# OpenVVC/OpenVVC

Measured on AMD Instinct MI355X. Metric: decoded frames/sec, full rcn back-end decode step (H2D of the recorded picture + MC incl. BDOF/DMVR/affine-PROF/GPM/CIIP + LMCS + inverse transform + ordered intra pass + deblocking + SAO + ALF/CC-ALF + D2H of refined MVs + wait + per-picture digest + publication to the device DPB), 4K 10-bit RA rec, higher is better.
Workload: dtype u16 samples / int16 coefficients / int32 accumulate

## Files before the change

### include/ovvc_hip.h

```cpp
#ifndef OVVC_HIP_H
#define OVVC_HIP_H

#include <stddef.h>
#include <stdint.h>

#ifdef __cplusplus
extern "C" {
#endif

#define OVHIP_ABI_VERSION 9

#define OVHIP_OK        0
#define OVHIP_ENODEV   (-1)
#define OVHIP_ENOMEM   (-2)
#define OVHIP_EINVAL   (-3)
#define OVHIP_ELAUNCH  (-4)
#define OVHIP_EUNSUP   (-5)
#define OVHIP_EREF     (-6)

enum { OVHIP_DST_VII = 0, OVHIP_DCT_VIII = 1, OVHIP_DCT_II = 2 };

typedef struct ovhip_pic {
    uint16_t *y, *cb, *cr;
    int32_t   w, h;
// ... 693 lines not shown
int  ovhip_dpb_create_ex(ovhip_dpb **out, int n_devices, const ovhip_dpb_ops *ops);
void ovhip_dpb_destroy(ovhip_dpb *d);
int  ovhip_dpb_n_devices(const ovhip_dpb *d);
int  ovhip_dpb_device(const ovhip_dpb *d, int dev);
int  ovhip_dpb_begin(ovhip_dpb *d, const void *key, int dev, int32_t w, int32_t h, ovhip_pic *pic);
int  ovhip_dpb_want(ovhip_dpb *d, const void *key, int dev);
int  ovhip_dpb_begin_tag(ovhip_dpb *d, const void *key, uint64_t tag, int dev, int32_t w, int32_t h, ovhip_pic *pic);
int  ovhip_dpb_want_tag(ovhip_dpb *d, const void *key, uint64_t tag, int dev);
int  ovhip_dpb_acquire_tag(ovhip_dpb *d, const void *key, uint64_t tag, int dev, ovhip_pic *pic, void **event);
int  ovhip_dpb_publish(ovhip_dpb *d, const void *key, int status);
void ovhip_dpb_set_unknown_key_timeout(ovhip_dpb *d, int ms);
int  ovhip_dpb_acquire(ovhip_dpb *d, const void *key, int dev, ovhip_pic *pic, void **event);
int  ovhip_dpb_poll_tag(ovhip_dpb *d, const void *key, uint64_t tag);
int  ovhip_dpb_post_rows(ovhip_dpb *d, const void *key, int32_t rows, void *event, const volatile uint32_t *abort_word);
int  ovhip_dpb_rows_tag(ovhip_dpb *d, const void *key, uint64_t tag, int dev, int32_t need_rows, int block, int pin, ovhip_pic *pic, void **event);
int  ovhip_dpb_wait_copy(ovhip_dpb *d, int dev, void *event);
int  ovhip_dpb_unpin(ovhip_dpb *d, const void *key);
int  ovhip_dpb_release(ovhip_dpb *d, const void *key);
int  ovhip_dpb_lookup(ovhip_dpb *d, const void *key, int *home_dev, ovhip_pic *pic);
void ovhip_dpb_shutdown(ovhip_dpb *d);
int  ovhip_dpb_get_stats(ovhip_dpb *d, ovhip_dpb_stats *out);

typedef struct ovhip_frame ovhip_frame;

enum { OVHIP_OUT_NONE = 0,
       OVHIP_OUT_DIGEST = 1,
       OVHIP_OUT_PLANES = 2,
       OVHIP_OUT_PACKED = 3 };
typedef struct ovhip_frame_output {
    int32_t  mode;
    ovhip_window window;
    uint16_t *y, *cb, *cr; int32_t stride_y, stride_c;
    void    *packed;
    uint8_t  digest[16];
} ovhip_frame_output;

enum { OVHIP_FE_BEGIN = 1, OVHIP_FE_REF, OVHIP_FE_DMVR_ROWS, OVHIP_FE_DMVR_BEGIN, OVHIP_FE_DMVR_COLLECT, OVHIP_FE_SUBMIT, OVHIP_FE_FAIL,
       OVHIP_FE_BAND  };
typedef struct ovhip_frame_event {
    uint32_t op; int32_t frame;
    uint64_t key, tag;
    int64_t  a, b, result;
} ovhip_frame_event;
void ovhip_frame_set_trace(void (*sink)(void *user, const ovhip_frame_event *ev), void *user);

int  ovhip_frame_create(ovhip_dpb *dpb, int dev, int32_t w, int32_t h, ovhip_frame **out);
void ovhip_frame_destroy(ovhip_frame *f);
ovhip_ctx      *ovhip_frame_ctx(ovhip_frame *f);
ovhip_job      *ovhip_frame_job(ovhip_frame *f);
ovhip_recorder *ovhip_frame_recorder(ovhip_frame *f);
int  ovhip_frame_begin(ovhip_frame *f, const void *key);
int  ovhip_frame_ref(ovhip_frame *f, const void *ref_key);
int  ovhip_frame_begin_tag(ovhip_frame *f, const void *key, uint64_t tag);
int  ovhip_frame_ref_tag(ovhip_frame *f, const void *ref_key, uint64_t tag);
int  ovhip_frame_ref_at(ovhip_frame *f, int slot, const void *ref_key);
int64_t ovhip_frame_dmvr_rows(ovhip_frame *f);
int  ovhip_frame_refs_ready(ovhip_frame *f);
int64_t ovhip_frame_dmvr_rows_begin(ovhip_frame *f, int32_t log2_ctu_s);
int64_t ovhip_frame_dmvr_rows_begin_upto(ovhip_frame *f, int32_t log2_ctu_s, size_t upto_units);
int64_t ovhip_frame_dmvr_rows_collect(ovhip_frame *f);
int  ovhip_frame_submit(ovhip_frame *f, ovhip_job *job, const ovhip_pic *intra, const ovhip_job_params *params, ovhip_frame_output *out);
int  ovhip_frame_set_band_mode(ovhip_frame *f, int on);
int  ovhip_frame_band(ovhip_frame *f, const ovhip_job_params *params, int32_t row_end, int32_t last, ovhip_frame_output *out);
int  ovhip_frame_band_upto(ovhip_frame *f, const ovhip_job_params *params, int32_t row_end, const ovhip_band_counts *upto, int32_t block);
int  ovhip_frame_band_stats(const ovhip_frame *f, int32_t *n_bands, int32_t *n_deferred);
int  ovhip_frame_set_output_scale(ovhip_frame *f, int32_t out_w, int32_t out_h, const ovhip_scale_info *info);
int  ovhip_frame_fail(ovhip_frame *f, int status);
const char *ovhip_frame_last_error(const ovhip_frame *f);

typedef struct ovhip_calllog ovhip_calllog;
ovhip_calllog *ovhip_calllog_create(void);
void   ovhip_calllog_destroy(ovhip_calllog *log);
void   ovhip_calllog_reset(ovhip_calllog *log);
const void *ovhip_calllog_data(const ovhip_calllog *log, size_t *bytes);
void   ovhip_rec_set_calllog(ovhip_recorder *rec, ovhip_calllog *log);
int64_t ovhip_calllog_replay(const void *data, size_t bytes, ovhip_recorder *rec);

#define OVHIP_STREAM_MAX_REFS 8
typedef struct ovhip_stream_content {
    const void *calllog; size_t calllog_bytes;
    ovhip_job_params params;
    uint32_t n_ref_slots;
} ovhip_stream_content;

typedef struct ovhip_stream_pic {
    uint32_t content;
    uint32_t job;
    int32_t  poc;
    uint16_t device;
    uint16_t n_refs;
    uint32_t refs[OVHIP_STREAM_MAX_REFS];
    int32_t  owner;
    uint32_t send_mask;
} ovhip_stream_pic;

typedef struct ovhip_stream_xfer {
    void *user;
    int (*send)(void *user, uint32_t idx, const ovhip_pic *pic, int dst_rank);
    int (*recv)(void *user, uint32_t idx, const ovhip_pic *pic, int src_rank);
} ovhip_stream_xfer;

typedef struct ovhip_rccl ovhip_rccl;
int  ovhip_rccl_unique_id(uint8_t out[128]);
int  ovhip_rccl_create(ovhip_rccl **out, const uint8_t unique_id[128], int rank, int world, int hip_device);
void ovhip_rccl_destroy(ovhip_rccl *r);
const ovhip_stream_xfer *ovhip_rccl_xfer(ovhip_rccl *r);
const char *ovhip_rccl_last_error(const ovhip_rccl *r);
int  ovhip_rccl_stats(const ovhip_rccl *r, uint64_t out[4]);
int  ovhip_rccl_self_exchange(ovhip_rccl *r, const ovhip_pic *src, const ovhip_pic *dst);

enum { OVHIP_STREAM_RECORD = 1,
       OVHIP_STREAM_DIGESTS = 2,
       OVHIP_STREAM_RESIDENT = 4,
       OVHIP_STREAM_KEEP = 8,
       OVHIP_STREAM_HOLD_ALL = 32,
       OVHIP_STREAM_FILE_MD5 = 16 };

typedef struct ovhip_stream_cfg {
    int32_t w, h;
    uint32_t flags;
    int32_t threads_per_device;
    int32_t output;
    ovhip_window window;
    uint32_t extra_stages;
    int32_t rank;
    const ovhip_stream_xfer *xfer;
    int32_t intra_lookahead;
    int32_t ahead_own_queue;
} ovhip_stream_cfg;

typedef struct ovhip_stream_result {
    double   seconds;
    uint64_t n_decoded, n_second_passes, n_received, n_sent;
    uint64_t out_frames, out_bytes;
    uint8_t  out_md5[16];
    double   record_seconds;
    double   host_seconds[5];
    int32_t  status;
    char     error[192];
    double  *trace;
} ovhip_stream_result;

typedef struct ovhip_stream ovhip_stream;
int  ovhip_stream_create(ovhip_stream **out, ovhip_dpb *dpb, const ovhip_stream_cfg *cfg, const ovhip_stream_content *contents,
                         uint32_t n_contents, ovhip_job *const *jobs, uint32_t n_jobs);
void ovhip_stream_destroy(ovhip_stream *s);
int  ovhip_stream_run(ovhip_stream *s, const ovhip_stream_pic *pics, uint32_t n_total, uint32_t first, uint32_t n, uint32_t flags,
                      uint8_t *digests, ovhip_stream_result *res);
ovhip_frame *ovhip_stream_frame(ovhip_stream *s, int dev, int thread);
int  ovhip_stream_queue_info(const ovhip_stream *s, int *moved, int *sharing);
int  ovhip_stream_set_output_scale(ovhip_stream *s, int32_t out_w, int32_t out_h, const ovhip_scale_info *info);
const void *ovhip_stream_key(const ovhip_stream *s, uint32_t idx);
int  ovhip_job_test_abort_next_flow(ovhip_job *job);

#ifdef __cplusplus
}
#endif
#endif
```

### openvvc_amd/capi.py

```python
from __future__ import annotations

import ctypes as C
import os
from pathlib import Path

import numpy as np

_PKG = Path(__file__).resolve().parent
LIB_PATH = _PKG / os.environ.get("OVVC_HIP_LIB_NAME", "libovvc_hip.so")

OVHIP_ABI_VERSION = 9
OVHIP_OK, OVHIP_ENODEV, OVHIP_ENOMEM, OVHIP_EINVAL, OVHIP_ELAUNCH, OVHIP_EUNSUP, OVHIP_EREF = 0, -1, -2, -3, -4, -5, -6
DST_VII, DCT_VIII, DCT_II = 0, 1, 2
TB_TR, TB_DC, TB_TS, TB_TS_RAW = 0, 1, 2, 3
TB_FLAG_RASTER = 0x80
RES_ADD, RES_SUB, RES_ADD_HALF, RES_SUB_HALF, RES_SCALE = 0, 1, 2, 3, 4
MC_HPEL_FILT, MC_FILT_4x4, MC_NO_LUMA, MC_NO_CHROMA, MC_LMCS, MC_BDOF, MC_DMVR = 1, 2, 4, 8, 16, 32, 64
PU_BDOF, PU_DMVR, PU_GPM = 1, 2, 4
MC_GPM = 128


class Pic(C.Structure):
    _fields_ = [("y", C.c_void_p), ("cb", C.c_void_p), ("cr", C.c_void_p),
                ("w", C.c_int32), ("h", C.c_int32), ("stride_y", C.c_int32), ("stride_c", C.c_int32)]
# ... 380 lines not shown
    global _lib
    if _lib is not None and path is None:
        return _lib
    p = Path(path) if path else LIB_PATH
    if not p.exists():
        raise RuntimeError(f"{p} not built: run `python -c 'import __graft_entry__ as g; g.build()'` "
                           "(the HIP engine has no CPU fallback)")
    try:
        import torch
    except Exception:
        pass
    lib = C.CDLL(str(p))
    vp, u32, i32 = C.c_void_p, C.c_uint32, C.c_int32
    P = C.POINTER
    sigs = {
        "ovhip_abi_version": (C.c_int, []),
        "ovhip_rec_create": (vp, [i32, i32]),
        "ovhip_rec_destroy": (None, [vp]),
        "ovhip_rec_reset": (None, [vp]),
        "ovhip_rec_tu": (C.c_int, [vp, P(TuState), P(TuDesc)]),
        "ovhip_rec_pu": (C.c_int, [vp, P(PuDesc)]),
        "ovhip_rec_set_ref_scale": (C.c_int, [vp, i32, P(RefScale)]),
        "ovhip_rec_refusal": (C.c_char_p, [vp]),
        "ovhip_rec_rpr_units": (vp, [vp, P(C.c_size_t)]),
        "ovhip_mc_rpr_launch": (C.c_int, [vp, P(Pic), P(Pic), u32, vp, u32, vp, P(Pic)]),
        "ovhip_rec_set_rpr_tools": (C.c_int, [vp, u32]),
        "ovhip_rec_aff_rpr_units": (vp, [vp, P(C.c_size_t)]),
        "ovhip_mca_rpr_launch": (C.c_int, [vp, P(Pic), P(Pic), u32, vp, u32, vp, vp]),
        "ovhip_rec_dbf_ctu": (C.c_int, [vp, vp]),
        "ovhip_rec_dbf_row": (C.c_int, [vp, vp, C.c_size_t]),
        "ovhip_rec_dbf_mv_prepass_view": (C.c_int, [vp, vp, vp, vp]),
        "ovhip_rec_cu_inter": (C.c_int, [vp, vp, vp]),
        "ovhip_rec_dbf_planes": (C.c_int, [vp, P(DbfPlanes)]),
        "ovhip_dbf_launch": (C.c_int, [vp, P(Pic), P(DbfPlanes)]),
        "ovhip_sao_launch": (C.c_int, [vp, P(Pic), P(Pic), vp, i32]),
        "ovhip_alf_launch": (C.c_int, [vp, P(Pic), P(Pic), P(AlfPic)]),
        "ovhip_rec_tb_cmds": (vp, [vp, P(C.c_size_t)]),
        "ovhip_rec_coefs": (vp, [vp, P(C.c_size_t)]),
        "ovhip_rec_mc_units": (vp, [vp, P(C.c_size_t)]),
        "ovhip_rec_mcx_units": (vp, [vp, P(C.c_size_t)]),
        "ovhip_rec_affine_cu": (C.c_int, [vp, P(AffineDesc)]),
        "ovhip_rec_transform_tree": (C.c_int, [vp, P(TuState), P(TtDesc)]),
        "ovhip_rec_lmcs_region": (C.c_int, [vp, C.c_int32, C.c_int32, u32, u32]),
        "ovhip_dbf_compact": (C.c_int64, [P(DbfPlanes), C.c_int, vp, C.c_size_t]),
        "ovhip_rec_dbf_mv_prepass": (C.c_int, [vp, P(DbfMvCtx)]),
        "ovhip_dbf_launch_edges": (C.c_int, [vp, P(Pic), vp, u32, vp, u32, C.c_int32, C.c_int32]),
        "ovhip_rec_ciip": (C.c_int, [vp, C.c_int32, C.c_int32, C.c_int32, C.c_int32, C.c_int32, C.c_int32]),
        "ovhip_rec_ciip_units": (vp, [vp, P(C.c_size_t)]),
        "ovhip_ciip_launch": (C.c_int, [vp, P(Pic), P(Pic), vp, u32]),
        "ovhip_rec_lmcs_regions": (vp, [vp, P(C.c_size_t)]),
        "ovhip_rec_tb_cmds_split": (vp, [vp, C.c_size_t * 4, P(C.c_size_t)]),
        "ovhip_itx_launch_classes": (C.c_int, [vp, P(Pic), vp, u32, u32, vp, vp]),
        "ovhip_itx_launch_chroma_lmcs": (C.c_int, [vp, P(Pic), vp, u32, u32, vp, vp, vp]),
        "ovhip_lmcs_build": (C.c_int, [P(LmcsData), P(LmcsLuts)]),
        "ovhip_lmcs_scale_launch": (C.c_int, [vp, P(Pic), vp, u32, P(LmcsLuts), vp]),
        "ovhip_lmcs_inverse_launch": (C.c_int, [vp, P(Pic), vp]),
        "ovhip_rec_aff_units": (vp, [vp, P(C.c_size_t)]),
        "ovhip_rec_aff_side": (vp, [vp, P(C.c_size_t)]),
        "ovhip_ctx_create": (C.c_int, [P(vp), C.c_int, vp]),
        "ovhip_ctx_destroy": (None, [vp]),
        "ovhip_ctx_sync": (C.c_int, [vp]),
        "ovhip_ctx_shares_queue": (C.c_int, [vp, vp]),
        "ovhip_ctx_new_stream": (C.c_int, [vp]),
        "ovhip_ctx_fork": (C.c_int, [vp, C.c_int]),
        "ovhip_ctx_join": (C.c_int, [vp]),
        "ovhip_last_error": (C.c_char_p, [vp]),
        "ovhip_ctx_stream": (vp, [vp]),
        "ovhip_malloc": (C.c_int, [vp, C.c_size_t, P(vp)]),
        "ovhip_free": (C.c_int, [vp, vp]),
        "ovhip_h2d": (C.c_int, [vp, vp, vp, C.c_size_t]),
        "ovhip_d2h": (C.c_int, [vp, vp, vp, C.c_size_t]),
        "ovhip_pic_alloc": (C.c_int, [vp, i32, i32, P(Pic)]),
        "ovhip_pic_free": (C.c_int, [vp, P(Pic)]),
        "ovhip_pic_upload": (C.c_int, [vp, P(Pic), vp, vp, vp, i32, i32]),
        "ovhip_pic_download": (C.c_int, [vp, P(Pic), vp, vp, vp, i32, i32]),
        "ovhip_itx_launch": (C.c_int, [vp, P(Pic), vp, u32, vp, vp]),
        "ovhip_mc_launch": (C.c_int, [vp, P(Pic), P(Pic), u32, vp, u32, vp, P(Pic)]),
        "ovhip_ciip_weight": (C.c_int, [C.c_int32, C.c_int32]),
        "ovhip_mcx_launch": (C.c_int, [vp, P(Pic), P(Pic), u32, vp, u32, vp, vp]),
        "ovhip_mca_launch": (C.c_int, [vp, P(Pic), P(Pic), u32, vp, u32, vp, vp]),
        "ovhip_mcxa_launch": (C.c_int, [vp, P(Pic), P(Pic), u32, vp, u32, vp, vp, u32, vp, vp]),
        "ovhip_rec_create_ex": (vp, [i32, i32, vp]),
        "ovhip_rec_set_dense_dbf_planes": (None, [vp, C.c_int]),
        "ovhip_rec_dbf_edges": (vp, [vp, C.c_int, P(C.c_size_t), P(DbfOffsets)]),
        "ovhip_dbf_launch_edges_ex": (C.c_int, [vp, P(Pic), vp, u32, vp, u32, P(DbfOffsets)]),
        "ovhip_dmvr_search_launch": (C.c_int, [vp, P(Pic), P(Pic), u32, vp, u32, vp]),
        "ovhip_rec_append_raw": (C.c_int, [vp, C.c_int, vp, C.c_size_t]),
        "ovhip_itx_launch_classes_res": (C.c_int, [vp, P(Pic), P(Pic), vp, u32, u32, vp, vp]),
        "ovhip_intra_level_launch": (C.c_int, [vp, P(Pic), P(Pic), vp, u32, vp, vp, vp, i32, u32]),
        "ovhip_intra_level_geom": (u32, [vp, C.c_size_t]),
        "ovhip_intra_sync_words": (C.c_size_t, [i32, i32, i32]),
        "ovhip_intra_flow_words": (C.c_size_t, [i32, i32]),
        "ovhip_intra_flow_items": (C.c_size_t, [vp, C.c_size_t, vp, C.c_size_t]),
        "ovhip_intra_flow_launch": (C.c_int, [vp, P(Pic), P(Pic), vp, u32, vp, u32, vp, vp, vp, i32, vp, u32, vp, i32, i32]),
        "ovhip_intra_ctu_launch": (C.c_int, [vp, P(Pic), P(Pic), vp, vp, u32, vp, vp, vp, i32, vp, u32, vp]),
        "ovhip_rec_itask_levels": (u32, [vp]),
        "ovhip_rec_isp_cu": (C.c_int, [vp, vp, vp]),
        "ovhip_isp_geometry": (None, [i32, i32, i32, P(i32), P(i32), P(i32), P(i32)]),
        "ovhip_job_bind": (C.c_int, [vp, vp]),
        "ovhip_rec_set_ctu_size": (C.c_int, [vp, i32]),
        "ovhip_rec_itasks_by_ctu": (vp, [vp, i32, P(C.c_size_t), P(vp), P(C.c_size_t)]),
        "ovhip_rec_tu_intra": (C.c_int, [vp, P(TuState), P(TuDesc), P(ITask), P(ITask)]),
        "ovhip_rec_itasks": (vp, [vp, P(C.c_size_t)]),
        "ovhip_rec_itasks_sorted": (vp, [vp, P(C.c_size_t), P(P(C.c_uint32)), P(C.c_uint32)]),
        "ovhip_rec_set_dbf_offsets": (C.c_int, [vp, P(DbfOffsets), C.c_int]),
        "ovhip_job_create": (C.c_int, [vp, i32, i32, P(vp)]),
        "ovhip_job_destroy": (None, [vp]),
        "ovhip_job_recorder": (vp, [vp]),
        "ovhip_job_begin": (C.c_int, [vp]),
        "ovhip_job_flush": (C.c_int, [vp, P(Pic), P(Pic), u32, P(Pic), P(JobParams)]),
        "ovhip_frame_band": (C.c_int, [vp, P(JobParams), i32, i32, P(FrameOutput)]),
        "ovhip_frame_set_band_mode": (C.c_int, [vp, C.c_int]),
        "ovhip_frame_band_upto": (C.c_int, [vp, P(JobParams), i32, P(BandCounts), i32]),
        "ovhip_frame_dmvr_rows_begin_upto": (C.c_int64, [vp, i32, C.c_size_t]),
        "ovhip_job_dmvr_rows_begin_upto": (C.c_int64, [vp, P(Pic), u32, i32, C.c_size_t]),
        "ovhip_frame_band_stats": (C.c_int, [vp, P(i32), P(i32)]),
        "ovhip_dpb_post_rows": (C.c_int, [vp, vp, i32, vp, vp]),
        "ovhip_dpb_rows_tag": (C.c_int, [vp, vp, C.c_uint64, C.c_int, i32, C.c_int, C.c_int, P(Pic), P(vp)]),
        "ovhip_job_band": (C.c_int, [vp, P(Pic), P(Pic), u32, P(JobParams), P(BandCounts), i32, i32]),
        "ovhip_job_band_active": (C.c_int, [vp]),
        "ovhip_job_band_busy": (C.c_int, [vp]),
        "ovhip_job_band_progress": (C.c_int, [vp, P(i32), P(vp), P(vp)]),
        "ovhip_rec_counts": (None, [vp, P(BandCounts)]),
        "ovhip_sao_launch_rows": (C.c_int, [vp, P(Pic), P(Pic), vp, i32, i32, i32]),
        "ovhip_alf_launch_rows": (C.c_int, [vp, P(Pic), P(Pic), P(AlfPic), i32, i32]),
        "ovhip_job_wait": (C.c_int, [vp]),
        "ovhip_job_refined_mvs": (vp, [vp, P(C.c_size_t)]),
        "ovhip_job_dmvr_rows": (C.c_int64, [vp, P(Pic), u32]),
        "ovhip_job_dmvr_rows_begin": (C.c_int64, [vp, P(Pic), u32, i32]),
        "ovhip_job_dmvr_rows_collect": (C.c_int64, [vp]),
        "ovhip_job_last_stats": (C.c_int, [vp, P(JobStats)]),
        "ovhip_job_time_stage": (C.c_int, [vp, C.c_int]),
        "ovhip_job_stage_time": (C.c_int, [vp, P(C.c_double), P(C.c_uint64)]),
        "ovhip_lmcs_scale_prepare_launch": (C.c_int, [vp, P(Pic), vp, u32, vp, vp, vp, u32, vp, u32]),
        "ovhip_lmcs_inverse_untag_launch": (C.c_int, [vp, P(Pic), vp, vp, u32]),
        "ovhip_intra_flow_untag_launch": (C.c_int, [vp, P(Pic), vp, u32, i32]),
        "ovhip_tmvp_cells_launch": (C.c_int, [vp, vp, u32, vp, i32, i32, vp]),
        "ovhip_job_tmvp_cells": (vp, [vp, P(C.c_size_t)]),
        "ovhip_output_bytes": (C.c_size_t, [i32, i32, P(Window)]),
        "ovhip_output_rows": (C.c_size_t, [i32, i32, P(Window)]),
        "ovhip_output_pack_launch": (C.c_int, [vp, P(Pic), P(Window), vp]),
        "ovhip_output_row_md5_launch": (C.c_int, [vp, P(Pic), P(Window), vp]),
        "ovhip_output_bands": (C.c_size_t, [i32, i32, P(Window)]),
        "ovhip_output_tree_md5_launch": (C.c_int, [vp, P(Pic), P(Window), vp]),
        "ovhip_pic_output": (C.c_int, [vp, P(Pic), P(Window), vp]),
        "ovhip_pic_digest": (C.c_int, [vp, P(Pic), P(Window), vp]),
        "ovhip_md5_init": (None, [P(Md5State)]),
        "ovhip_md5_update": (None, [P(Md5State), vp, C.c_size_t]),
        "ovhip_md5_final": (None, [P(Md5State), vp]),
        "ovhip_d2d": (C.c_int, [vp, vp, vp, C.c_size_t]),
        "ovhip_host_alloc": (vp, [C.c_size_t]),
        "ovhip_host_free": (None, [vp]),
        "ovhip_job_test_abort_next_flow": (C.c_int, [vp]),
        "ovhip_dpb_create": (C.c_int, [P(vp), P(C.c_int), C.c_int]),
        "ovhip_dpb_create_ex": (C.c_int, [P(vp), C.c_int, P(DpbOps)]),
        "ovhip_dpb_destroy": (None, [vp]),
        "ovhip_dpb_n_devices": (C.c_int, [vp]),
        "ovhip_dpb_device": (C.c_int, [vp, C.c_int]),
        "ovhip_dpb_begin": (C.c_int, [vp, vp, C.c_int, i32, i32, P(Pic)]),
        "ovhip_dpb_want": (C.c_int, [vp, vp, C.c_int]),
        "ovhip_dpb_begin_tag": (C.c_int, [vp, vp, C.c_uint64, C.c_int, i32, i32, P(Pic)]),
        "ovhip_dpb_want_tag": (C.c_int, [vp, vp, C.c_uint64, C.c_int]),
        "ovhip_dpb_acquire_tag": (C.c_int, [vp, vp, C.c_uint64, C.c_int, P(Pic), P(vp)]),
        "ovhip_dpb_publish": (C.c_int, [vp, vp, C.c_int]),
        "ovhip_dpb_acquire": (C.c_int, [vp, vp, C.c_int, P(Pic), P(vp)]),
        "ovhip_dpb_wait_copy": (C.c_int, [vp, C.c_int, vp]),
        "ovhip_dpb_poll_tag": (C.c_int, [vp, vp, C.c_uint64]),
        "ovhip_frame_refs_ready": (C.c_int, [vp]),
        "ovhip_dpb_set_unknown_key_timeout": (None, [vp, C.c_int]),
        "ovhip_dpb_unpin": (C.c_int, [vp, vp]),
        "ovhip_dpb_release": (C.c_int, [vp, vp]),
        "ovhip_dpb_lookup": (C.c_int, [vp, vp, P(C.c_int), P(Pic)]),
        "ovhip_dpb_shutdown": (None, [vp]),
        "ovhip_dpb_get_stats": (C.c_int, [vp, P(DpbStats)]),
        "ovhip_frame_create": (C.c_int, [vp, C.c_int, i32, i32, P(vp)]),
        "ovhip_frame_destroy": (None, [vp]),
        "ovhip_frame_ctx": (vp, [vp]),
        "ovhip_frame_job": (vp, [vp]),
        "ovhip_frame_recorder": (vp, [vp]),
        "ovhip_frame_begin": (C.c_int, [vp, vp]),
        "ovhip_frame_ref": (C.c_int, [vp, vp]),
        "ovhip_frame_set_trace": (None, [vp, vp]),
        "ovhip_rccl_unique_id": (C.c_int, [vp]),
        "ovhip_rccl_create": (C.c_int, [P(vp), vp, C.c_int, C.c_int, C.c_int]),
        "ovhip_rccl_destroy": (None, [vp]),
        "ovhip_rccl_xfer": (vp, [vp]),
        "ovhip_rccl_last_error": (C.c_char_p, [vp]),
        "ovhip_rccl_stats": (C.c_int, [vp, P(C.c_uint64)]),
        "ovhip_rccl_self_exchange": (C.c_int, [vp, P(Pic), P(Pic)]),
        "ovhip_frame_begin_tag": (C.c_int, [vp, vp, C.c_uint64]),
        "ovhip_frame_ref_tag": (C.c_int, [vp, vp, C.c_uint64]),
        "ovhip_frame_ref_at": (C.c_int, [vp, C.c_int, vp]),
        "ovhip_frame_dmvr_rows": (C.c_int64, [vp]),
        "ovhip_frame_dmvr_rows_begin": (C.c_int64, [vp, i32]),
        "ovhip_frame_dmvr_rows_collect": (C.c_int64, [vp]),
        "ovhip_frame_submit": (C.c_int, [vp, vp, P(Pic), P(JobParams), P(FrameOutput)]),
        "ovhip_frame_fail": (C.c_int, [vp, C.c_int]),
        "ovhip_frame_last_error": (C.c_char_p, [vp]),
        "ovhip_calllog_create": (vp, []),
        "ovhip_calllog_destroy": (None, [vp]),
        "ovhip_calllog_reset": (None, [vp]),
        "ovhip_calllog_data": (vp, [vp, P(C.c_size_t)]),
        "ovhip_rec_set_calllog": (None, [vp, vp]),
        "ovhip_calllog_replay": (C.c_int64, [vp, C.c_size_t, vp]),
        "ovhip_stream_create": (C.c_int, [P(vp), vp, P(StreamCfg), P(StreamContent), u32, P(vp), u32]),
        "ovhip_stream_destroy": (None, [vp]),
        "ovhip_stream_run": (C.c_int, [vp, P(StreamPic), u32, u32, u32, u32, vp, P(StreamResult)]),
        "ovhip_stream_frame": (vp, [vp, C.c_int, C.c_int]),
        "ovhip_stream_queue_info": (C.c_int, [vp, P(C.c_int), P(C.c_int)]),
        "ovhip_stream_key": (vp, [vp, u32]),
        "ovhip_output_scale_check": (C.c_int, [i32, i32, P(ScaleInfo), i32, i32, P(i32 * 4)]),
        "ovhip_output_scale_launch": (C.c_int, [vp, P(Pic), P(ScaleInfo), P(Pic)]),
        "ovhip_pic_output_scaled": (C.c_int, [vp, P(Pic), P(ScaleInfo), i32, i32, P(Window), vp]),
        "ovhip_pic_digest_scaled": (C.c_int, [vp, P(Pic), P(ScaleInfo), i32, i32, P(Window), vp]),
        "ovhip_ctx_scratch_bytes": (C.c_size_t, [vp]),
        "ovhip_frame_set_output_scale": (C.c_int, [vp, i32, i32, P(ScaleInfo)]),
        "ovhip_stream_set_output_scale": (C.c_int, [vp, i32, i32, P(ScaleInfo)]),
    }
    ab_build = "OVVC_HIP_LIB_NAME" in os.environ
    for name, (res, args) in sigs.items():
        if ab_build and not hasattr(lib, name):
            continue
        fn = getattr(lib, name)
        fn.restype, fn.argtypes = res, args
    if lib.ovhip_abi_version() != OVHIP_ABI_VERSION and not ab_build:
        raise RuntimeError("libovvc_hip.so ABI version mismatch")
    if path is None:
        _lib = lib
    return lib


EXPORTED_SYMBOLS = [
    "ovhip_abi_version", "ovhip_rec_create", "ovhip_rec_destroy", "ovhip_rec_reset", "ovhip_rec_tu",
    "ovhip_rec_pu", "ovhip_rec_cu_inter", "ovhip_rec_dbf_row", "ovhip_rec_dbf_mv_prepass_view", "ovhip_rec_dbf_ctu", "ovhip_rec_dbf_planes", "ovhip_dbf_launch", "ovhip_sao_launch", "ovhip_alf_launch", "ovhip_rec_tb_cmds", "ovhip_rec_coefs", "ovhip_rec_mc_units", "ovhip_rec_mcx_units", "ovhip_mcx_launch", "ovhip_rec_affine_cu", "ovhip_rec_transform_tree", "ovhip_rec_lmcs_region", "ovhip_dbf_compact", "ovhip_rec_dbf_mv_prepass", "ovhip_dbf_launch_edges", "ovhip_rec_ciip", "ovhip_ciip_weight", "ovhip_rec_ciip_units", "ovhip_ciip_launch", "ovhip_rec_lmcs_regions", "ovhip_rec_tb_cmds_split", "ovhip_itx_launch_classes", "ovhip_itx_launch_chroma_lmcs", "ovhip_lmcs_build", "ovhip_lmcs_scale_launch", "ovhip_lmcs_inverse_launch", "ovhip_rec_aff_units", "ovhip_rec_aff_side", "ovhip_mca_launch", "ovhip_mcxa_launch", "ovhip_ctx_create",
    "ovhip_ctx_destroy", "ovhip_ctx_sync", "ovhip_ctx_shares_queue", "ovhip_ctx_new_stream", "ovhip_ctx_fork", "ovhip_ctx_join", "ovhip_last_error", "ovhip_ctx_stream", "ovhip_malloc",
    "ovhip_free", "ovhip_h2d", "ovhip_d2h", "ovhip_pic_alloc", "ovhip_pic_free", "ovhip_pic_upload",
    "ovhip_pic_download", "ovhip_itx_launch", "ovhip_mc_launch",
    "ovhip_rec_set_ref_scale", "ovhip_rec_refusal", "ovhip_rec_rpr_units", "ovhip_mc_rpr_launch",
    "ovhip_rec_set_rpr_tools", "ovhip_rec_aff_rpr_units", "ovhip_mca_rpr_launch",
    "ovhip_rec_create_ex", "ovhip_rec_set_dense_dbf_planes", "ovhip_rec_dbf_edges", "ovhip_dbf_launch_edges_ex",
    "ovhip_dmvr_search_launch", "ovhip_rec_append_raw", "ovhip_rec_set_dbf_offsets", "ovhip_rec_tu_intra", "ovhip_rec_itasks", "ovhip_rec_itasks_sorted", "ovhip_itx_launch_classes_res", "ovhip_intra_level_launch", "ovhip_intra_level_geom", "ovhip_intra_sync_words", "ovhip_intra_ctu_launch", "ovhip_intra_flow_words", "ovhip_intra_flow_items", "ovhip_intra_flow_launch",
    "ovhip_rec_itask_levels", "ovhip_rec_isp_cu", "ovhip_isp_geometry", "ovhip_rec_itasks_by_ctu", "ovhip_rec_set_ctu_size", "ovhip_job_bind", "ovhip_job_create", "ovhip_job_destroy", "ovhip_job_recorder", "ovhip_job_begin",
    "ovhip_frame_band", "ovhip_frame_band_upto", "ovhip_frame_dmvr_rows_begin_upto", "ovhip_job_dmvr_rows_begin_upto", "ovhip_frame_set_band_mode", "ovhip_frame_band_stats", "ovhip_dpb_post_rows", "ovhip_dpb_rows_tag",
    "ovhip_job_band", "ovhip_job_band_active", "ovhip_job_band_busy", "ovhip_job_band_reserve", "ovhip_job_reserve_for_picture", "ovhip_rec_reserve_for_picture", "ovhip_job_band_progress", "ovhip_rec_counts", "ovhip_sao_launch_rows", "ovhip_alf_launch_rows",
    "ovhip_job_flush", "ovhip_job_wait", "ovhip_job_refined_mvs", "ovhip_job_dmvr_rows", "ovhip_job_dmvr_rows_begin", "ovhip_job_dmvr_rows_collect", "ovhip_job_last_stats", "ovhip_job_time_stage", "ovhip_job_stage_time",
    "ovhip_output_bytes", "ovhip_output_rows", "ovhip_output_pack_launch", "ovhip_output_row_md5_launch", "ovhip_output_bands", "ovhip_output_tree_md5_launch", "ovhip_pic_output", "ovhip_pic_digest",
    "ovhip_md5_init", "ovhip_md5_update", "ovhip_md5_final", "ovhip_tmvp_cells_launch", "ovhip_job_tmvp_cells", "ovhip_intra_flow_untag_launch", "ovhip_lmcs_inverse_untag_launch", "ovhip_lmcs_scale_prepare_launch",
    "ovhip_host_alloc", "ovhip_host_free", "ovhip_d2d", "ovhip_job_test_abort_next_flow",
    "ovhip_dpb_create", "ovhip_dpb_create_ex", "ovhip_dpb_destroy", "ovhip_dpb_n_devices", "ovhip_dpb_device", "ovhip_dpb_begin", "ovhip_dpb_want",
    "ovhip_dpb_publish", "ovhip_dpb_acquire", "ovhip_dpb_wait_copy", "ovhip_dpb_poll_tag", "ovhip_frame_refs_ready", "ovhip_dpb_set_unknown_key_timeout", "ovhip_dpb_unpin", "ovhip_dpb_release", "ovhip_dpb_lookup", "ovhip_dpb_shutdown",
    "ovhip_dpb_get_stats", "ovhip_dpb_begin_tag", "ovhip_dpb_want_tag", "ovhip_dpb_acquire_tag", "ovhip_frame_begin_tag", "ovhip_frame_ref_tag", "ovhip_frame_set_trace",
    "ovhip_rccl_unique_id", "ovhip_rccl_create", "ovhip_rccl_destroy", "ovhip_rccl_xfer", "ovhip_rccl_last_error", "ovhip_rccl_stats", "ovhip_rccl_self_exchange",
    "ovhip_frame_create", "ovhip_frame_destroy", "ovhip_frame_ctx", "ovhip_frame_job", "ovhip_frame_recorder", "ovhip_frame_begin", "ovhip_frame_ref",
    "ovhip_frame_ref_at", "ovhip_frame_dmvr_rows", "ovhip_frame_dmvr_rows_begin", "ovhip_frame_dmvr_rows_collect", "ovhip_frame_submit", "ovhip_frame_fail", "ovhip_frame_last_error",
    "ovhip_calllog_create", "ovhip_calllog_destroy", "ovhip_calllog_reset", "ovhip_calllog_data", "ovhip_rec_set_calllog", "ovhip_calllog_replay",
    "ovhip_stream_create", "ovhip_stream_destroy", "ovhip_stream_run", "ovhip_stream_frame", "ovhip_stream_key", "ovhip_stream_queue_info",
    "ovhip_output_scale_check", "ovhip_output_scale_launch", "ovhip_pic_output_scaled", "ovhip_pic_digest_scaled",
    "ovhip_frame_set_output_scale", "ovhip_stream_set_output_scale", "ovhip_ctx_scratch_bytes",
]


def rpr_units(lib, rec) -> list:
    n = C.c_size_t(0)
    ptr = lib.ovhip_rec_rpr_units(rec, C.byref(n))
    if not ptr or not n.value:
        return []
    raw = C.string_at(ptr, n.value * C.sizeof(RprUnit))
    return [RprUnit.from_buffer_copy(raw, i * C.sizeof(RprUnit)) for i in range(n.value)]


def aff_rpr_units(lib, rec) -> list:
    n = C.c_size_t(0)
    ptr = lib.ovhip_rec_aff_rpr_units(rec, C.byref(n))
    if not ptr or not n.value:
        return []
    raw = C.string_at(ptr, n.value * C.sizeof(AffRprUnit))
    return [AffRprUnit.from_buffer_copy(raw, i * C.sizeof(AffRprUnit)) for i in range(n.value)]


def set_ref_scale(lib, rec, slot: int, scale_hor: int | None = None, scale_ver: int | None = None, ref_w: int = 0, ref_h: int = 0,
                  col_hor: int = 0, col_ver: int = 0) -> int:
    if scale_hor is None:
        return lib.ovhip_rec_set_ref_scale(rec, slot, None)
    sc = RefScale(scale_hor, scale_ver if scale_ver is not None else scale_hor, ref_w, ref_h, col_hor, col_ver)
    return lib.ovhip_rec_set_ref_scale(rec, slot, C.byref(sc))


class Recorder:

    def __init__(self, pic_w: int, pic_h: int):
        self.lib = load()
        self.h = self.lib.ovhip_rec_create(pic_w, pic_h)
        if not self.h:
            raise MemoryError("ovhip_rec_create")
        self._keep = []

    def close(self):
        if self.h:
            self.lib.ovhip_rec_destroy(self.h)
            self.h = None

    def __del__(self):
        try:
            self.close()
        except Exception:
            pass

    def reset(self):
        self.lib.ovhip_rec_reset(self.h)

    def start_calllog(self):
        self._log = self.lib.ovhip_calllog_create()
        self.lib.ovhip_rec_set_calllog(self.h, self._log)

    def take_calllog(self) -> np.ndarray:
        n = C.c_size_t()
        p = self.lib.ovhip_calllog_data(self._log, C.byref(n))
        if not p and n.value:
            raise MemoryError("call log")
        out = np.frombuffer((C.c_char * n.value).from_address(p), dtype=np.uint8).copy() if n.value else np.zeros(0, np.uint8)
        self.lib.ovhip_rec_set_calllog(self.h, None)
        self.lib.ovhip_calllog_destroy(self._log)
        self._log = None
        return out

    def replay(self, log: np.ndarray) -> int:
        n = self.lib.ovhip_calllog_replay(log.ctypes.data, log.nbytes, self.h)
        if n < 0:
            raise ValueError(f"ovhip_calllog_replay -> {n}")
        return int(n)

    def tu(self, st: TuState, d: TuDesc) -> int:
        r = self.lib.ovhip_rec_tu(self.h, C.byref(st), C.byref(d))
        if r < 0:
            raise ValueError(f"ovhip_rec_tu -> {r}")
        return r

    def tu_intra(self, st: TuState, d: TuDesc, task_l: "ITask | None", task_c: "ITask | None") -> int:
        r = self.lib.ovhip_rec_tu_intra(self.h, C.byref(st), C.byref(d), C.byref(task_l) if task_l is not None else None,
                                        C.byref(task_c) if task_c is not None else None)
        if r < 0:
            raise ValueError(f"ovhip_rec_tu_intra -> {r}")
        return r

    def itasks(self) -> np.ndarray:
        return self._arr(self.lib.ovhip_rec_itasks, ITASK_DTYPE)

    def itasks_sorted(self):
        n, nl, ls = C.c_size_t(), C.c_uint32(), C.POINTER(C.c_uint32)()
        p = self.lib.ovhip_rec_itasks_sorted(self.h, C.byref(n), C.byref(ls), C.byref(nl))
        if not n.value:
            return np.zeros(0, ITASK_DTYPE), np.zeros(1, np.uint32)
        t = np.frombuffer((C.c_char * (n.value * 32)).from_address(p), dtype=ITASK_DTYPE).copy()
        return t, np.array([ls[i] for i in range(nl.value + 1)], np.uint32)

    def itasks_by_ctu(self, log2_ctu: int = 7):
        n, nc, cp = C.c_size_t(), C.c_size_t(), C.c_void_p()
        p = self.lib.ovhip_rec_itasks_by_ctu(self.h, log2_ctu, C.byref(n), C.byref(cp), C.byref(nc))
        if not n.value:
            return np.zeros(0, ITASK_DTYPE), np.zeros(0, ICTU_DTYPE)
        t = np.frombuffer((C.c_char * (n.value * 32)).from_address(p), dtype=ITASK_DTYPE).copy()
        c = np.frombuffer((C.c_char * (nc.value * 16)).from_address(cp.value), dtype=ICTU_DTYPE).copy()
        return t, c

    def transform_tree(self, st: "TuState", d: TtDesc, infos: bytes, res_cb: np.ndarray, res_cr: np.ndarray, res_y: np.ndarray) -> int:
        ib = (C.c_char * len(infos)).from_buffer_copy(infos)
        keep = [np.ascontiguousarray(a, dtype=np.int16) for a in (res_cb, res_cr, res_y)]
        d.tu_info = C.addressof(ib)
        for k in range(3):
            d.residual[k] = keep[k].ctypes.data
        r = self.lib.ovhip_rec_transform_tree(self.h, C.byref(st), C.byref(d))
        d.tu_info = None
        if r < 0:
            raise ValueError(f"ovhip_rec_transform_tree -> {r}")
        return r

    def isp_cu(self, st: TuState, d: IspDesc) -> int:
        r = self.lib.ovhip_rec_isp_cu(self.h, C.byref(st), C.byref(d))
        if r < 0:
            raise ValueError(f"ovhip_rec_isp_cu -> {r}")
        return r

    def isp_geometry(self, log2_w: int, log2_h: int, vertical: int):
        a, b, c, d = C.c_int32(), C.c_int32(), C.c_int32(), C.c_int32()
        self.lib.ovhip_isp_geometry(log2_w, log2_h, vertical, C.byref(a), C.byref(b), C.byref(c), C.byref(d))
        return a.value, b.value, c.value, d.value

    def pu(self, d: PuDesc) -> int:
        r = self.lib.ovhip_rec_pu(self.h, C.byref(d))
        if r < 0:
            raise ValueError(f"ovhip_rec_pu -> {r}")
        return r

    def affine_cu(self, d: AffineDesc, mv0: np.ndarray, mv1: np.ndarray) -> int:
        mv0 = np.ascontiguousarray(mv0, dtype=np.int32)
        mv1 = np.ascontiguousarray(mv1, dtype=np.int32)
        d.mv0, d.mv1 = mv0.ctypes.data, mv1.ctypes.data
        r = self.lib.ovhip_rec_affine_cu(self.h, C.byref(d))
        d.mv0 = d.mv1 = None
        if r < 0:
            raise ValueError(f"ovhip_rec_affine_cu -> {r}")
# ... 99 lines not shown
```

### openvvc_amd/csrc/kernels_dbf.hip

```cpp
#include "ovvc_common.hip.h"
#define OVT_ATTR __device__
#include "vvc_dbf_tables.h"

#ifndef OV_WPE_DBF
#define OV_WPE_DBF 0
#endif
#if OV_WPE_DBF > 0
#define OV_OCC_DBF __attribute__((amdgpu_waves_per_eu(OV_WPE_DBF)))
#else
#define OV_OCC_DBF
#endif

namespace {

struct Lim { int tc, beta; };

__device__ __forceinline__ Lim dbf_limits(int qp, int bs, int tc_off, int beta_off)
{
    Lim l;
    l.tc = ovt_dbf_tc[ov_clip3(qp + 2 * (bs - 1) + tc_off, 0, 66)];
    l.beta = (int)ovt_dbf_beta[ov_clip3(qp + beta_off, 0, 64)] << 2;
    return l;
}

struct Line16 { int s[16]; };

template <int NP, int NQ>
__device__ __forceinline__ void load_line(const uint16_t *pix, int step, int *s)
{
#pragma unroll
    for (int i = 0; i < NP; ++i) s[7 - i] = pix[(-1 - i) * step];
#pragma unroll
    for (int i = 0; i < NQ; ++i) s[8 + i] = pix[i * step];
}
#define P(i) s[7 - (i)]
#define Q(i) s[8 + (i)]

__device__ __forceinline__ int dp_of(const int *s, int o) { return abs(P(2 + o) - 2 * P(1 + o) + P(0 + o)); }
__device__ __forceinline__ int dq_of(const int *s, int o) { return abs(Q(0 + o) - 2 * Q(1 + o) + Q(2 + o)); }

__device__ __forceinline__ bool strong_large(const int *s, int beta, int tc, int lp, int lq)
{
    int sp3 = abs(P(3) - P(0)), sq3 = abs(Q(3) - Q(0));
    if (lp == 7)      { sp3 += abs((P(4) - P(5)) - P(6) + P(7)); sp3 += abs(P(3) - P(7)) + 1; sp3 >>= 1; }
    else if (lp == 5) { sp3 += abs(P(3) - P(5)) + 1; sp3 >>= 1; }
    if (lq == 7)      { sq3 += abs((Q(4) - Q(5)) - Q(6) + Q(7)); sq3 += abs(Q(7) - Q(3)) + 1; sq3 >>= 1; }
    else if (lq == 5) { sq3 += abs(Q(5) - Q(3)) + 1; sq3 >>= 1; }
    return ((sp3 + sq3) < (beta * 3 >> 5)) && (abs(P(0) - Q(0)) < ((tc * 5 + 1) >> 1));
}

__device__ __forceinline__ bool strong_small(const int *s, int beta, int tc)
{
    return ((abs(P(3) - P(0)) + abs(Q(3) - Q(0))) < (beta >> 3)) && (abs(P(0) - Q(0)) < ((tc * 5 + 1) >> 1));
}

__device__ __forceinline__ void long_regs(const int *s, uint16_t *pix, int step, int tc, int lp, int lq)
{
    const int f7[7] = { 59, 50, 41, 32, 23, 14, 5 }, f5[5] = { 58, 45, 32, 19, 6 }, f3[3] = { 53, 32, 11 };
    const int t7[7] = { 6, 5, 4, 3, 2, 1, 1 }, t3[3] = { 6, 4, 2 };
    const int ref_p = (P(lp - 1) + P(lp) + 1) >> 1, ref_q = (Q(lq - 1) + Q(lq) + 1) >> 1;
    int mid;
    if (lp == lq && lp == 7)
        mid = (2 * (P(0) + Q(0)) + P(1) + P(2) + P(3) + P(4) + P(5) + P(6) + Q(1) + Q(2) + Q(3) + Q(4) + Q(5) + Q(6) + 8) >> 4;
    else if (lp == lq)
        mid = (2 * (P(0) + P(1) + P(2) + Q(0) + Q(1) + Q(2)) + P(3) + P(4) + Q(3) + Q(4) + 8) >> 4;
    else if (lp + lq == 12)
        mid = (2 * (P(0) + P(1) + Q(0) + Q(1)) + P(2) + P(3) + P(4) + P(5) + Q(2) + Q(3) + Q(4) + Q(5) + 8) >> 4;
    else if (lp + lq == 8)
        mid = (P(0) + P(1) + P(2) + P(3) + Q(0) + Q(1) + Q(2) + Q(3) + 4) >> 3;
    else if (lp == 7)
        mid = (2 * (P(0) + Q(0)) + P(1) + P(2) + P(3) + P(4) + P(5) + P(6) + Q(0) + 3 * Q(1) + 2 * Q(2) + 8) >> 4;
    else
        mid = (2 * (P(0) + Q(0)) + Q(1) + Q(2) + Q(3) + Q(4) + Q(5) + Q(6) + P(0) + 3 * P(1) + 2 * P(2) + 8) >> 4;
#pragma unroll
    for (int i = 0; i < 7; ++i) {
        if (i < lp) {
            const int f = lp == 7 ? f7[i] : (lp == 5 ? f5[i < 5 ? i : 0] : f3[i < 3 ? i : 0]);
            const int cv = (tc * (lp == 3 ? t3[i < 3 ? i : 0] : t7[i])) >> 1;
            pix[(-1 - i) * step] = (uint16_t)ov_clip3((mid * f + ref_p * (64 - f) + 32) >> 6, P(i) - cv, P(i) + cv);
        }
        if (i < lq) {
            const int f = lq == 7 ? f7[i] : (lq == 5 ? f5[i < 5 ? i : 0] : f3[i < 3 ? i : 0]);
            const int cv = (tc * (lq == 3 ? t3[i < 3 ? i : 0] : t7[i])) >> 1;
            pix[i * step] = (uint16_t)ov_clip3((mid * f + ref_q * (64 - f) + 32) >> 6, Q(i) - cv, Q(i) + cv);
        }
    }
}

__device__ __forceinline__ void long_line(uint16_t *pix, int step, int tc, int lp, int lq)
{
    int s[16];
    load_line<8, 8>(pix, step, s);
    long_regs(s, pix, step, tc, lp, lq);
}

__device__ __forceinline__ void strong_regs(const int *s, uint16_t *pix, int step, int tc)
{
    const int p3 = P(3), p2 = P(2), p1 = P(1), p0 = P(0), q0 = Q(0), q1 = Q(1), q2 = Q(2), q3 = Q(3);
    pix[-3 * step] = (uint16_t)ov_clip3((2 * p3 + 3 * p2 + p1 + p0 + q0 + 4) >> 3, p2 - tc, p2 + tc);
    pix[-2 * step] = (uint16_t)ov_clip3((p2 + p1 + p0 + q0 + 2) >> 2, p1 - 2 * tc, p1 + 2 * tc);
    pix[-1 * step] = (uint16_t)ov_clip3((p2 + 2 * p1 + 2 * p0 + 2 * q0 + q1 + 4) >> 3, p0 - 3 * tc, p0 + 3 * tc);
    pix[0]         = (uint16_t)ov_clip3((p1 + 2 * p0 + 2 * q0 + 2 * q1 + q2 + 4) >> 3, q0 - 3 * tc, q0 + 3 * tc);
    pix[1 * step]  = (uint16_t)ov_clip3((p0 + q0 + q1 + q2 + 2) >> 2, q1 - 2 * tc, q1 + 2 * tc);
    pix[2 * step]  = (uint16_t)ov_clip3((p0 + q0 + q1 + 3 * q2 + 2 * q3 + 4) >> 3, q2 - tc, q2 + tc);
}

__device__ __forceinline__ void strong_line(uint16_t *pix, int step, int tc)
{
    int s[16];
    load_line<4, 4>(pix, step, s);
    strong_regs(s, pix, step, tc);
}

__device__ __forceinline__ void weak_regs(const int *s, uint16_t *pix, int step, int tc, bool ext_p, bool ext_q)
{
    const int p2 = P(2), p1 = P(1), p0 = P(0), q0 = Q(0), q1 = Q(1), q2 = Q(2);
    const int tc2p = ext_p ? tc >> 1 : 0, tc2q = ext_q ? tc >> 1 : 0;
    int delta = (9 * (q0 - p0) - 3 * (q1 - p1) + 8) >> 4;
    if (abs(delta) < tc * 10) {
        delta = ov_clip3(delta, -tc, tc);
        const int d1 = ov_clip3((((p2 + p0 + 1) >> 1) - p1 + delta) >> 1, -tc2p, tc2p);
        const int d2 = ov_clip3((((q2 + q0 + 1) >> 1) - q1 - delta) >> 1, -tc2q, tc2q);
        pix[-2 * step] = (uint16_t)ov_clip_bd(p1 + d1);
        pix[-1 * step] = (uint16_t)ov_clip_bd(p0 + delta);
        pix[0]         = (uint16_t)ov_clip_bd(q0 - delta);
        pix[1 * step]  = (uint16_t)ov_clip_bd(q1 + d2);
    }
}

__device__ __forceinline__ void weak_line(uint16_t *pix, int step, int tc, bool ext_p, bool ext_q)
{
    int s[16];
    load_line<3, 3>(pix, step, s);
    weak_regs(s, pix, step, tc, ext_p, ext_q);
}

template <int SEL> __device__ __forceinline__ int quad_bcast(int v)
{
    return __builtin_amdgcn_mov_dpp(v, SEL * 0x55, 0xf, 0xf, true);
}

template <int DIR, int NS>
__device__ __forceinline__ void load_line_q(const uint16_t *pix, int step, int *s)
{
    if (DIR == 0 && !(reinterpret_cast<uintptr_t>(pix) & 7)) {
#pragma unroll
        for (int g = 0; g < NS / 4; ++g) {
            const uint2 a = *reinterpret_cast<const uint2 *>(pix - 4 * (g + 1));
            const uint2 b = *reinterpret_cast<const uint2 *>(pix + 4 * g);
            s[7 - (4 * g + 3)] = a.x & 0xffff; s[7 - (4 * g + 2)] = a.x >> 16; s[7 - (4 * g + 1)] = a.y & 0xffff; s[7 - 4 * g] = a.y >> 16;
            s[8 + 4 * g] = b.x & 0xffff; s[8 + 4 * g + 1] = b.x >> 16; s[8 + 4 * g + 2] = b.y & 0xffff; s[8 + 4 * g + 3] = b.y >> 16;
        }
    } else {
#pragma unroll
        for (int i = 0; i < NS; ++i) { s[7 - i] = pix[(-1 - i) * step]; s[8 + i] = pix[i * step]; }
    }
}

template <int DIR>
__device__ __forceinline__ void luma_quad(uint16_t *pix, int step, Lim lim, int lp, int lq)
{
    const int beta = lim.beta, tc = lim.tc;
    const bool big = lp > 3 || lq > 3;
    int s[16];
    if (big) load_line_q<DIR, 8>(pix, step, s);
    else     load_line_q<DIR, 4>(pix, step, s);
    const int dp = dp_of(s, 0), dq = dq_of(s, 0);
    const int dp0 = quad_bcast<0>(dp), dq0 = quad_bcast<0>(dq), dp3 = quad_bcast<3>(dp), dq3 = quad_bcast<3>(dq);
    const int d0 = dp0 + dq0, d3 = dp3 + dq3;
    if (d0 + d3 >= beta) return;
    if (big) {
        int dpL = dp, dqL = dq;
        if (lp > 3) dpL = (dpL + dp_of(s, 3) + 1) >> 1;
        if (lq > 3) dqL = (dqL + dq_of(s, 3) + 1) >> 1;
        const int dL = dpL + dqL;
        const int ok = (dL < ((beta + 0x10) >> 5)) && strong_large(s, beta, tc, lp, lq);
        const int d0L = quad_bcast<0>(dL), d3L = quad_bcast<3>(dL);
        if ((d0L + d3L < beta) && quad_bcast<0>(ok) && quad_bcast<3>(ok)) { long_regs(s, pix, step, tc, lp, lq); return; }
    }
    const int oks = strong_small(s, beta, tc);
    const bool sw = lp > 2 && (d0 < ((beta + 4) >> 3)) && (d3 < ((beta + 4) >> 3)) && quad_bcast<0>(oks) && quad_bcast<3>(oks);
    if (sw) {
        strong_regs(s, pix, step, tc);
    } else {
        const int side = (beta + (beta >> 1)) >> 3;
        const bool ext_p = (dp0 + dp3) < side && lp > 1;
        const bool ext_q = (dq0 + dq3) < side && lp > 1;
        weak_regs(s, pix, step, tc, ext_p, ext_q);
    }
}

template <int DIR>
__device__ __forceinline__ void chroma_quad(uint16_t *pix, int step, Lim lim, bool large, bool ctb_b, bool store)
{
    const int tc = lim.tc, beta = lim.beta;
    if (tc == 0 || beta == 0) return;
    int s[16];
    load_line_q<DIR, 4>(pix, step, s);
    bool strong = false;
    if (large) {
        const int p3 = ctb_b ? P(1) : P(3);
        const int dpv = abs((ctb_b ? P(1) : P(2)) - 2 * P(1) + P(0));
        const int d = dpv + dq_of(s, 0);
        const int ok = ((abs(p3 - P(0)) + abs(Q(3) - Q(0))) < (beta >> 3)) && (abs(P(0) - Q(0)) < ((tc * 5 + 1) >> 1))
                       && (2 * d < (beta >> 2));
        const int da = quad_bcast<0>(d), db = quad_bcast<1>(d);
        strong = quad_bcast<0>(ok) && quad_bcast<1>(ok) && (da + db < beta);
    }
    if (!store) return;
    const int p3 = P(3), p2 = P(2), p1 = P(1), p0 = P(0), q0 = Q(0), q1 = Q(1), q2 = Q(2), q3 = Q(3);
    if (strong) {
        if (ctb_b) {
            pix[-1 * step] = (uint16_t)ov_clip3((3 * p1 + 2 * p0 + q0 + q1 + q2 + 4) >> 3, p0 - tc, p0 + tc);
            pix[0]         = (uint16_t)ov_clip3((2 * p1 + p0 + 2 * q0 + q1 + q2 + q3 + 4) >> 3, q0 - tc, q0 + tc);
        } else {
            pix[-3 * step] = (uint16_t)ov_clip3((3 * p3 + 2 * p2 + p1 + p0 + q0 + 4) >> 3, p2 - tc, p2 + tc);
            pix[-2 * step] = (uint16_t)ov_clip3((2 * p3 + p2 + 2 * p1 + p0 + q0 + q1 + 4) >> 3, p1 - tc, p1 + tc);
            pix[-1 * step] = (uint16_t)ov_clip3((p3 + p2 + p1 + 2 * p0 + q0 + q1 + q2 + 4) >> 3, p0 - tc, p0 + tc);
            pix[0]         = (uint16_t)ov_clip3((p2 + p1 + p0 + 2 * q0 + q1 + q2 + q3 + 4) >> 3, q0 - tc, q0 + tc);
        }
        pix[1 * step] = (uint16_t)ov_clip3((p1 + p0 + q0 + 2 * q1 + q2 + 2 * q3 + 4) >> 3, q1 - tc, q1 + tc);
        pix[2 * step] = (uint16_t)ov_clip3((p0 + q0 + q1 + 2 * q2 + 3 * q3 + 4) >> 3, q2 - tc, q2 + tc);
    } else {
        const int delta = ov_clip3(((q0 << 2) - (p0 << 2) + p1 - q1 + 4) >> 3, -tc, tc);
        pix[-1 * step] = (uint16_t)ov_clip_bd(p0 + delta);
        pix[0]         = (uint16_t)ov_clip_bd(q0 - delta);
    }
}

__device__ __forceinline__ void luma_segment(uint16_t *pix0, int step, int lstep, Lim lim, int lp, int lq)
{
    const int beta = lim.beta, tc = lim.tc;
    int a[16], b[16];
    if (lp > 3 || lq > 3) { load_line<8, 8>(pix0, step, a); load_line<8, 8>(pix0 + 3 * lstep, step, b); }
    else                  { load_line<4, 4>(pix0, step, a); load_line<4, 4>(pix0 + 3 * lstep, step, b); }
    const int dp0 = dp_of(a, 0), dq0 = dq_of(a, 0), dp3 = dp_of(b, 0), dq3 = dq_of(b, 0);
    const int d0 = dp0 + dq0, d3 = dp3 + dq3;
    if (d0 + d3 >= beta) return;
    bool sl = false;
    if (lp > 3 || lq > 3) {
        int dp0L = dp0, dq0L = dq0, dp3L = dp3, dq3L = dq3;
        if (lp > 3) { dp0L = (dp0L + dp_of(a, 3) + 1) >> 1; dp3L = (dp3L + dp_of(b, 3) + 1) >> 1; }
        if (lq > 3) { dq0L = (dq0L + dq_of(a, 3) + 1) >> 1; dq3L = (dq3L + dq_of(b, 3) + 1) >> 1; }
        const int d0L = dp0L + dq0L, d3L = dp3L + dq3L;
        sl = (d0L + d3L < beta) && (d0L < ((beta + 0x10) >> 5)) && (d3L < ((beta + 0x10) >> 5))
             && strong_large(a, beta, tc, lp, lq) && strong_large(b, beta, tc, lp, lq);
    }
    if (sl) {
#pragma unroll 1
        for (int l = 0; l < 4; ++l) long_line(pix0 + l * lstep, step, tc, lp, lq);
        return;
    }
    const bool sw = lp > 2 && (d0 < ((beta + 4) >> 3)) && (d3 < ((beta + 4) >> 3))
                    && strong_small(a, beta, tc) && strong_small(b, beta, tc);
    if (sw) {
#pragma unroll 1
        for (int l = 0; l < 4; ++l) strong_line(pix0 + l * lstep, step, tc);
    } else {
        const int side = (beta + (beta >> 1)) >> 3;
        const bool ext_p = (dp0 + dp3) < side && lp > 1;
        const bool ext_q = (dq0 + dq3) < side && lp > 1;
#pragma unroll 1
        for (int l = 0; l < 4; ++l) weak_line(pix0 + l * lstep, step, tc, ext_p, ext_q);
    }
}

__device__ __forceinline__ void chroma_segment(uint16_t *pix0, int step, int lstep, Lim lim, bool large, bool ctb_b)
{
    const int tc = lim.tc, beta = lim.beta;
    if (tc == 0 || beta == 0) return;
    int s0[16], s1[16];
    load_line<4, 4>(pix0, step, s0);
    load_line<4, 4>(pix0 + lstep, step, s1);
    bool strong = false;
    if (large) {
        int d[2];
        bool ok = true;
#pragma unroll
        for (int l = 0; l < 2; ++l) {
            const int *s = l ? s1 : s0;
            const int p3 = ctb_b ? P(1) : P(3);
            const int dp = abs((ctb_b ? P(1) : P(2)) - 2 * P(1) + P(0));
            d[l] = dp + dq_of(s, 0);
            ok = ok && ((abs(p3 - P(0)) + abs(Q(3) - Q(0))) < (beta >> 3)) && (abs(P(0) - Q(0)) < ((tc * 5 + 1) >> 1));
        }
        strong = ok && (d[0] + d[1] < beta) && (2 * d[0] < (beta >> 2)) && (2 * d[1] < (beta >> 2));
    }
#pragma unroll
    for (int l = 0; l < 2; ++l) {
        const int *s = l ? s1 : s0;
        uint16_t *pix = pix0 + l * lstep;
        const int p3 = P(3), p2 = P(2), p1 = P(1), p0 = P(0), q0 = Q(0), q1 = Q(1), q2 = Q(2), q3 = Q(3);
        if (strong) {
            if (ctb_b) {
                pix[-1 * step] = (uint16_t)ov_clip3((3 * p1 + 2 * p0 + q0 + q1 + q2 + 4) >> 3, p0 - tc, p0 + tc);
                pix[0]         = (uint16_t)ov_clip3((2 * p1 + p0 + 2 * q0 + q1 + q2 + q3 + 4) >> 3, q0 - tc, q0 + tc);
            } else {
                pix[-3 * step] = (uint16_t)ov_clip3((3 * p3 + 2 * p2 + p1 + p0 + q0 + 4) >> 3, p2 - tc, p2 + tc);
                pix[-2 * step] = (uint16_t)ov_clip3((2 * p3 + p2 + 2 * p1 + p0 + q0 + q1 + 4) >> 3, p1 - tc, p1 + tc);
                pix[-1 * step] = (uint16_t)ov_clip3((p3 + p2 + p1 + 2 * p0 + q0 + q1 + q2 + 4) >> 3, p0 - tc, p0 + tc);
                pix[0]         = (uint16_t)ov_clip3((p2 + p1 + p0 + 2 * q0 + q1 + q2 + q3 + 4) >> 3, q0 - tc, q0 + tc);
            }
            pix[1 * step] = (uint16_t)ov_clip3((p1 + p0 + q0 + 2 * q1 + q2 + 2 * q3 + 4) >> 3, q1 - tc, q1 + tc);
            pix[2 * step] = (uint16_t)ov_clip3((p0 + q0 + q1 + 2 * q2 + 3 * q3 + 4) >> 3, q2 - tc, q2 + tc);
        } else {
            const int delta = ov_clip3(((q0 << 2) - (p0 << 2) + p1 - q1 + 4) >> 3, -tc, tc);
            pix[-1 * step] = (uint16_t)ov_clip_bd(p0 + delta);
            pix[0]         = (uint16_t)ov_clip_bd(q0 - delta);
        }
    }
}
#undef P
#undef Q

template <int DIR>
__global__ __launch_bounds__(256) void k_dbf(ovhip_pic pic, ovhip_dbf_planes pl)
{
    const int comp = blockIdx.y;
    const int w4 = pl.w4, h4 = pl.h4;
    const int nthreads = gridDim.x * 256;
    if (comp == 0) {
        for (int tid = blockIdx.x * 256 + threadIdx.x; tid < w4 * h4; tid += nthreads) {
            const int ux = tid % w4, uy = tid / w4;
            const int v = (DIR ? pl.luma_h : pl.luma_v)[tid];
            if (!(v & 3)) continue;
            if ((DIR ? uy : ux) == 0) continue;
            const Lim lim = dbf_limits(v >> 8, v & 3, pl.tc_offset, pl.beta_offset);
            if (!(lim.tc || lim.beta)) continue;
            uint16_t *p = pic.y + (uy * 4) * pic.stride_y + ux * 4;
            luma_segment(p, DIR ? pic.stride_y : 1, DIR ? 1 : pic.stride_y, lim, (v >> 2) & 7, (v >> 5) & 7);
        }
    } else {
        const int cw = DIR ? w4 : (w4 + 1) >> 1, chh = DIR ? (h4 + 1) >> 1 : h4;
        const uint16_t *plane = DIR ? (comp == 1 ? pl.cb_h : pl.cr_h) : (comp == 1 ? pl.cb_v : pl.cr_v);
        for (int tid = blockIdx.x * 256 + threadIdx.x; tid < cw * chh; tid += nthreads) {
            const int cx = tid % cw, cy = tid / cw;
            const int v = plane[tid];
            if (!(v & OVHIP_DBF_C_ON)) continue;
            const int ux = DIR ? cx : cx * 2, uy = DIR ? cy * 2 : cy;
            if ((DIR ? uy : ux) == 0) continue;
            const Lim lim = dbf_limits(v >> 8, 1 + !!(v & OVHIP_DBF_C_BS2), pl.tc_offset, pl.beta_offset);
            uint16_t *p = (comp == 1 ? pic.cb : pic.cr) + (uy * 2) * pic.stride_c + ux * 2;
            chroma_segment(p, DIR ? pic.stride_c : 1, DIR ? 1 : pic.stride_c, lim, v & OVHIP_DBF_C_LARGE, v & OVHIP_DBF_C_CTB_B);
        }
    }
}

template <int DIR>
__global__ __launch_bounds__(256) OV_OCC_DBF void k_dbf_list(ovhip_pic pic, const ovhip_dbf_edge *__restrict__ edges, uint32_t n,
                                                  uint64_t tc_pack, uint64_t beta_pack)
{
    const uint32_t tid = ov_xcd_slot(blockIdx.x, gridDim.x) * 256 + threadIdx.x;
    const uint32_t ei = tid >> 2;
    const int l = tid & 3;
    if (ei >= n) return;
    const ovhip_dbf_edge e = edges[ei];
    const int v = e.word;
    const int osh = (e.pad & 7) * 8;
    const int tc_offset = (int8_t)(tc_pack >> osh), beta_offset = (int8_t)(beta_pack >> osh);
    if (e.comp == 0) {
        const Lim lim = dbf_limits(v >> 8, v & 3, tc_offset, beta_offset);
        if (!(lim.tc || lim.beta)) return;
        uint16_t *p = pic.y + (e.uy * 4) * pic.stride_y + e.ux * 4 + l * (DIR ? 1 : pic.stride_y);
        luma_quad<DIR>(p, DIR ? pic.stride_y : 1, lim, (v >> 2) & 7, (v >> 5) & 7);
    } else {
        const Lim lim = dbf_limits(v >> 8, 1 + !!(v & OVHIP_DBF_C_BS2), tc_offset, beta_offset);
        uint16_t *p = (e.comp == 1 ? pic.cb : pic.cr) + (e.uy * 2) * pic.stride_c + e.ux * 2 + (l & 1) * (DIR ? 1 : pic.stride_c);
        chroma_quad<DIR>(p, DIR ? pic.stride_c : 1, lim, v & OVHIP_DBF_C_LARGE, v & OVHIP_DBF_C_CTB_B, l < 2);
    }
}

}

extern "C" int ovhip_dbf_launch_edges_ex(ovhip_ctx *ctx, const ovhip_pic *pic, const ovhip_dbf_edge *d_edges_v, uint32_t n_v,
                                         const ovhip_dbf_edge *d_edges_h, uint32_t n_h, const ovhip_dbf_offsets *offsets)
{
    if (!ctx || !pic || !offsets) return OVHIP_EINVAL;
    OV_DEVICE(ctx);
    if ((n_v && !d_edges_v) || (n_h && !d_edges_h))
        return ov_fail(ctx, OVHIP_EINVAL, "ovhip_dbf_launch_edges: null edge list", hipSuccess);
    uint64_t tc_pack, beta_pack;
    memcpy(&tc_pack, offsets->tc, 8); memcpy(&beta_pack, offsets->beta, 8);
    if (n_v) {
        hipLaunchKernelGGL(k_dbf_list<0>, dim3((n_v + 63) / 64), dim3(256), 0, ctx->stream, *pic, d_edges_v, n_v, tc_pack, beta_pack);
        OV_LAUNCH_CHECK(ctx, "k_dbf_list<v>");
    }
    if (n_h) {
        hipLaunchKernelGGL(k_dbf_list<1>, dim3((n_h + 63) / 64), dim3(256), 0, ctx->stream, *pic, d_edges_h, n_h, tc_pack, beta_pack);
        OV_LAUNCH_CHECK(ctx, "k_dbf_list<h>");
    }
    return OVHIP_OK;
}

extern "C" int ovhip_dbf_launch_edges(ovhip_ctx *ctx, const ovhip_pic *pic, const ovhip_dbf_edge *d_edges_v, uint32_t n_v,
                                      const ovhip_dbf_edge *d_edges_h, uint32_t n_h, int32_t beta_offset, int32_t tc_offset)
{
    if (beta_offset < -128 || beta_offset > 127 || tc_offset < -128 || tc_offset > 127) return OVHIP_EINVAL;
    ovhip_dbf_offsets o;
    for (int i = 0; i < OVHIP_DBF_MAX_OFFSETS; ++i) { o.beta[i] = (int8_t)beta_offset; o.tc[i] = (int8_t)tc_offset; }
    return ovhip_dbf_launch_edges_ex(ctx, pic, d_edges_v, n_v, d_edges_h, n_h, &o);
}

extern "C" int ovhip_dbf_launch(ovhip_ctx *ctx, const ovhip_pic *pic, const ovhip_dbf_planes *pl)
{
    if (!ctx || !pic || !pl) return OVHIP_EINVAL;
    OV_DEVICE(ctx);
    if (!pl->luma_v || !pl->luma_h || !pl->cb_v || !pl->cr_v || !pl->cb_h || !pl->cr_h)
        return ov_fail(ctx, OVHIP_EINVAL, "ovhip_dbf_launch: null edge plane", hipSuccess);
    if (pl->w4 != (pic->w + 3) / 4 || pl->h4 != (pic->h + 3) / 4)
        return ov_fail(ctx, OVHIP_EINVAL, "ovhip_dbf_launch: edge planes do not match the picture", hipSuccess);
    const int n = pl->w4 * pl->h4;
    const int nb = (n + 255) / 256;
    dim3 grid(nb, 3);
    hipLaunchKernelGGL(k_dbf<0>, grid, dim3(256), 0, ctx->stream, *pic, *pl);
    OV_LAUNCH_CHECK(ctx, "k_dbf<v>");
    hipLaunchKernelGGL(k_dbf<1>, grid, dim3(256), 0, ctx->stream, *pic, *pl);
    OV_LAUNCH_CHECK(ctx, "k_dbf<h>");
    return OVHIP_OK;
}
```

### openvvc_amd/csrc/kernels_sao.hip

```cpp
#include "ovvc_common.hip.h"
#include <stdlib.h>

namespace {

#define SAO_TW 64
#define SAO_TH 32

struct Vec8 { int v[8]; };

__device__ __forceinline__ void load8(const uint16_t *p, bool vec, int n, int v[8])
{
    if (vec) {
        const uint4 q = *reinterpret_cast<const uint4 *>(p);
        v[0] = q.x & 0xffff; v[1] = q.x >> 16; v[2] = q.y & 0xffff; v[3] = q.y >> 16;
        v[4] = q.z & 0xffff; v[5] = q.z >> 16; v[6] = q.w & 0xffff; v[7] = q.w >> 16;
    } else {
#pragma unroll
        for (int i = 0; i < 8; ++i) v[i] = i < n ? p[i] : 0;
    }
}

__global__ __launch_bounds__(256) void k_sao(ovhip_pic dst, ovhip_pic src, const ovhip_sao_ctu *__restrict__ prm,
                                              int log2_ctu, int nb_ctu_w, int tiles_y, int tiles_c, int ty0_y, int ty0_c, int row0, int row1)
{
    const int tx = threadIdx.x & 7, ty = threadIdx.x >> 3;
    for (int t = blockIdx.x; t < tiles_y + 2 * tiles_c; t = tiles_y + 2 * tiles_c) {
        const int c = t < tiles_y ? 0 : (t < tiles_y + tiles_c ? 1 : 2);
        const int tt = (int)ov_xcd_slot_at(t, c == 0 ? 0 : (c == 1 ? tiles_y : tiles_y + tiles_c), c == 0 ? tiles_y : tiles_c);
        const int sh = c ? 1 : 0;
        const int w = src.w >> sh, h = src.h >> sh, l2 = log2_ctu - sh;
        const int ntx = (w + SAO_TW - 1) / SAO_TW;
        const int x0 = (tt % ntx) * SAO_TW + tx * 8, y = (tt / ntx + (c ? ty0_c : ty0_y)) * SAO_TH + ty;
        if (x0 >= w || y >= h || y < (row0 >> sh) || y >= (row1 >> sh)) continue;
        int ss, ds;
        const uint16_t *s = ov_plane(src, c, ss) + y * ss;
        uint16_t *d = ov_plane(dst, c, ds) + y * ds;
        const ovhip_sao_ctu *p = &prm[(y >> l2) * nb_ctu_w + (x0 >> l2)];
        const int type = p->type[c];
        const int n = min(8, w - x0);
        const bool vec = n == 8 && !((ss | ds) & 7) && !(((uintptr_t)s | (uintptr_t)d) & 15);
        int v[8], o[8];
        load8(s + x0, vec, n, v);
#pragma unroll
        for (int i = 0; i < 8; ++i) o[i] = v[i];
        if (type == OVHIP_SAO_BAND) {
            const int bp = p->band_position[c];
            const int o0 = p->offset_val[c][0], o1 = p->offset_val[c][1], o2 = p->offset_val[c][2], o3 = p->offset_val[c][3];
#pragma unroll
            for (int i = 0; i < 8; ++i) {
                const int k = ((v[i] >> (OV_BD - 5)) - bp) & 31;
                const int off = k == 0 ? o0 : k == 1 ? o1 : k == 2 ? o2 : k == 3 ? o3 : 0;
                o[i] = ov_clip_bd(v[i] + off);
            }
        } else if (type == OVHIP_SAO_EDGE) {
            const int eo = p->eo_class[c];
            const int dxa = eo == 1 ? 0 : (eo == 3 ? 1 : -1), dya = eo == 0 ? 0 : -1;
            const int bd = p->border, cs = 1 << l2;
            const int cy0 = y & ~(cs - 1), cx0 = x0 & ~(cs - 1);
            const int cx1 = min(cx0 + cs, w) - 1;
            const bool rowskip = eo != 0 && (y == 0 || y == h - 1 || (src.h <= (1 << log2_ctu) && y == (6 >> sh) - 1) ||
                                             ((bd & OVHIP_BORDER_UPPER) && y == cy0) || ((bd & OVHIP_BORDER_BOTTOM) && y == min(cy0 + cs, h) - 1) ||
                                             ((bd & OVHIP_BORDER_ONE_ROW) && y == cy0 + (6 >> sh) - 1));
            const int skip_l = (bd & OVHIP_BORDER_LEFT) ? cx0 : -1, skip_r = (bd & OVHIP_BORDER_RIGHT) ? cx1 : -1;
            if (!rowskip) {
                const int of0 = p->offset_val[c][0], of1 = p->offset_val[c][1], of2 = p->offset_val[c][2],
                          of3 = p->offset_val[c][3], of4 = p->offset_val[c][4];
                int ra[10], rb[10];
                const uint16_t *sa = s + dya * ss, *sb = s - dya * ss;
                load8(sa + x0, vec, n, ra + 1);
                load8(sb + x0, vec, n, rb + 1);
                ra[0] = x0 > 0 ? sa[x0 - 1] : 0; rb[0] = x0 > 0 ? sb[x0 - 1] : 0;
                ra[9] = x0 + 8 < w ? sa[x0 + 8] : 0; rb[9] = x0 + 8 < w ? sb[x0 + 8] : 0;
#pragma unroll
                for (int i = 0; i < 8; ++i) {
                    const int x = x0 + i;
                    if (i < n && !(eo != 1 && (x == 0 || x == w - 1 || x == skip_l || x == skip_r))) {
                        const int a = ra[1 + i + dxa], b = rb[1 + i - dxa];
                        const int idx = 2 + (v[i] > a) - (v[i] < a) + (v[i] > b) - (v[i] < b);
                        const int off = idx == 0 ? of0 : idx == 1 ? of1 : idx == 2 ? of2 : idx == 3 ? of3 : of4;
                        o[i] = ov_clip_bd(v[i] + off);
                    }
                }
            }
        }
        if (vec) {
            uint4 q;
            q.x = o[0] | (o[1] << 16); q.y = o[2] | (o[3] << 16); q.z = o[4] | (o[5] << 16); q.w = o[6] | (o[7] << 16);
            *reinterpret_cast<uint4 *>(d + x0) = q;
        } else {
#pragma unroll
            for (int i = 0; i < 8; ++i) if (i < n) d[x0 + i] = (uint16_t)o[i];
        }
    }
}

}

extern "C" int ovhip_sao_launch_rows(ovhip_ctx *ctx, const ovhip_pic *dst, const ovhip_pic *src,
                                     const ovhip_sao_ctu *d_params, int32_t log2_ctu_s, int32_t row0, int32_t row1)
{
    if (!ctx || !dst || !src || !d_params) return OVHIP_EINVAL;
    OV_DEVICE(ctx);
    if (dst->w != src->w || dst->h != src->h || dst->y == src->y || log2_ctu_s < 5 || log2_ctu_s > 7)
        return ov_fail(ctx, OVHIP_EINVAL, "ovhip_sao_launch: bad pictures / CTU size", hipSuccess);
    if (row0 < 0 || row1 > src->h || row0 > row1 || (row0 & 7) || ((row1 & 7) && row1 != src->h))
        return ov_fail(ctx, OVHIP_EINVAL, "ovhip_sao_launch_rows: row window", hipSuccess);
    if (row0 == row1) return OVHIP_OK;
    const int nb_ctu_w = (src->w + (1 << log2_ctu_s) - 1) >> log2_ctu_s;
    const int ty0_y = row0 / SAO_TH, ty1_y = (row1 + SAO_TH - 1) / SAO_TH;
    const int ty0_c = (row0 / 2) / SAO_TH, ty1_c = (row1 / 2 + SAO_TH - 1) / SAO_TH;
    const int tiles_y = ((src->w + SAO_TW - 1) / SAO_TW) * (ty1_y - ty0_y);
    const int tiles_c = ((src->w / 2 + SAO_TW - 1) / SAO_TW) * (ty1_c - ty0_c);
    const int total = tiles_y + 2 * tiles_c;
    hipLaunchKernelGGL(k_sao, dim3(total), dim3(256), 0, ctx->stream, *dst, *src, d_params,
                       log2_ctu_s, nb_ctu_w, tiles_y, tiles_c, ty0_y, ty0_c, row0, row1);
    OV_LAUNCH_CHECK(ctx, "k_sao");
    return OVHIP_OK;
}

extern "C" int ovhip_sao_launch(ovhip_ctx *ctx, const ovhip_pic *dst, const ovhip_pic *src,
                                const ovhip_sao_ctu *d_params, int32_t log2_ctu_s)
{
    if (!src) return OVHIP_EINVAL;
    return ovhip_sao_launch_rows(ctx, dst, src, d_params, log2_ctu_s, 0, src->h);
}
```

### openvvc_amd/csrc/ovvc_common.hip.h

```cpp
#pragma once
#include <hip/hip_runtime.h>
#include <stdint.h>
#include <stdio.h>
#include <string.h>
#include "ovvc_hip.h"


#define OV_BD 10
#define OV_PIX_MAX ((1 << OV_BD) - 1)

#define OV_MAX_LANES 4
struct ovhip_ctx {
    int device;
    int num_cus;
    hipStream_t stream;
    int owns_stream;
    hipStream_t main_stream;
    hipStream_t lane[OV_MAX_LANES];
    hipEvent_t ev_fork, ev_lane[OV_MAX_LANES];
    int lane_used[OV_MAX_LANES];
    int have_events;
    void *scratch_d; size_t scratch_d_cap;
    void *scratch_h; size_t scratch_h_cap;
    void *scale_d; size_t scale_d_cap;
    hipEvent_t ev_sync;
    char err[256];
};

static inline int ov_fail(ovhip_ctx *ctx, int code, const char *what, hipError_t e)
{
    if (ctx) snprintf(ctx->err, sizeof(ctx->err), "%s: %s", what, e == hipSuccess ? "invalid argument" : hipGetErrorString(e));
    return code;
}

#define OV_HIP(ctx, call)                                                     \
    do {                                                                      \
        hipError_t e__ = (call);                                              \
        if (e__ != hipSuccess) return ov_fail((ctx), OVHIP_ENODEV, #call, e__); \
    } while (0)

#define OV_DEVICE(ctx)                                                        \
    do {                                                                      \
        hipError_t e__ = hipSetDevice((ctx)->device);                         \
        if (e__ != hipSuccess) return ov_fail((ctx), OVHIP_ENODEV, "hipSetDevice", e__); \
        (void)hipGetLastError();    \
    } while (0)

static inline hipError_t ov_sync_stream(ovhip_ctx *ctx)
{
    hipError_t e = hipSuccess;
    if (!ctx->ev_sync) e = hipEventCreateWithFlags(&ctx->ev_sync, hipEventDisableTiming);
    if (e == hipSuccess) e = hipEventRecord(ctx->ev_sync, ctx->stream);
    if (e == hipSuccess) e = hipEventSynchronize(ctx->ev_sync);
    return e;
}

static inline int ov_scratch(ovhip_ctx *ctx, size_t dev_bytes, size_t host_bytes)
{
    if (dev_bytes > ctx->scratch_d_cap) {
        if (ctx->scratch_d) (void)hipFree(ctx->scratch_d);
        ctx->scratch_d = nullptr; ctx->scratch_d_cap = 0;
        hipError_t e = hipMalloc(&ctx->scratch_d, dev_bytes);
        if (e != hipSuccess) return ov_fail(ctx, OVHIP_ENOMEM, "hipMalloc(scratch)", e);
        ctx->scratch_d_cap = dev_bytes;
    }
    if (host_bytes > ctx->scratch_h_cap) {
        if (ctx->scratch_h) (void)hipHostFree(ctx->scratch_h);
        ctx->scratch_h = nullptr; ctx->scratch_h_cap = 0;
        hipError_t e = hipHostMalloc(&ctx->scratch_h, host_bytes, hipHostMallocDefault);
        if (e != hipSuccess) return ov_fail(ctx, OVHIP_ENOMEM, "hipHostMalloc(scratch)", e);
        ctx->scratch_h_cap = host_bytes;
    }
    return OVHIP_OK;
}

#define OV_LAUNCH_CHECK(ctx, name)                                            \
    do {                                                                      \
        hipError_t e__ = hipGetLastError();                                   \
        if (e__ != hipSuccess) return ov_fail((ctx), OVHIP_ELAUNCH, name, e__); \
    } while (0)

#define OV_NUM_XCD 8
__device__ __forceinline__ uint32_t ov_xcd_slot(uint32_t i, uint32_t n)
{
    const uint32_t k = i % OV_NUM_XCD, j = i / OV_NUM_XCD;
    const uint32_t base = n / OV_NUM_XCD, rem = n % OV_NUM_XCD;
    return k * base + (k < rem ? k : rem) + j;
}

__device__ __forceinline__ uint32_t ov_xcd_slot_at(uint32_t b, uint32_t first, uint32_t n)
{
    const uint32_t i = b - first, k = b % OV_NUM_XCD, f = first % OV_NUM_XCD;
    uint32_t start = 0;
#pragma unroll
    for (uint32_t q = 0; q < OV_NUM_XCD; ++q) {
        const uint32_t r = (q + OV_NUM_XCD - f) % OV_NUM_XCD;
        if (q < k) start += (n + OV_NUM_XCD - 1 - r) / OV_NUM_XCD;
    }
    return start + i / OV_NUM_XCD;
}

__device__ __forceinline__ int ov_rowoff(int row, int stride) { return __mul24(row, stride); }

__device__ __forceinline__ int ov_clip3(int v, int lo, int hi) { return min(max(v, lo), hi); }
__device__ __forceinline__ int ov_clip16(int v) { return ov_clip3(v, -32768, 32767); }
__device__ __forceinline__ int ov_clip_bd(int v) { return ov_clip3(v, 0, OV_PIX_MAX); }

__device__ __forceinline__ uint16_t *ov_plane(const ovhip_pic &p, int plane, int &stride)
{
    stride = plane ? p.stride_c : p.stride_y;
    return plane == 0 ? p.y : (plane == 1 ? p.cb : p.cr);
}
```

### openvvc_amd/csrc/ovvc_picture.hip

```cpp
#include "ovvc_common.hip.h"
#include "flow_state.hip.h"
#include <stdlib.h>

extern "C" int ovhip_dmvr_search_launch(ovhip_ctx *ctx, const ovhip_pic *geom, const ovhip_pic *refs, uint32_t n_refs,
                                        const ovhip_mc_unit *d_units, uint32_t n_units, int32_t *d_mv_out);

struct BandState;
namespace {

struct DevBuf { void *p; size_t cap; };

enum { B_TB, B_COEF, B_MC, B_MCX, B_MV, B_AFF, B_SIDE, B_REG, B_SCALE, B_EV, B_EH, B_PARAM, B_CLASS, B_CIIP, B_ITASK, B_ICTU, B_IITEM, B_TMVP, B_RPR, B_AFFR, B_COUNT };

static const ovhip_pic *same_size_refs(const ovhip_pic *geom, const ovhip_pic *refs, uint32_t n_refs, ovhip_pic *out)
{
    if (!refs || n_refs > 16) return refs;
    bool any = false;
    for (uint32_t i = 0; i < n_refs; ++i) {
        const bool same = refs[i].w == geom->w && refs[i].h == geom->h && refs[i].stride_y == geom->stride_y && refs[i].stride_c == geom->stride_c;
        out[i] = same ? refs[i] : *geom;
        any |= !same;
    }
    return any ? out : refs;
}

}

struct ovhip_job {
    ovhip_ctx *ctx;
    ovhip_ctx *home;
    int32_t w, h;
    ovhip_recorder *rec;
    DevBuf dev[B_COUNT];
    ovhip_pic tmp;
    ovhip_pic res;
    uint32_t *d_sync; uint32_t epoch;
    uint32_t *d_flow;
    uint32_t *items_host; size_t items_cap;
    uint32_t *abort_host;
    char *param_host; size_t param_cap;
    int32_t *mv_host; size_t mv_cap;
    struct { int valid, has_intra; ovhip_pic dst, refs[16], intra; uint32_t n_refs; ovhip_job_params pr; } again;
    uint32_t n_retries;
    int flow_launched;
    int test_abort, test_abort_seen;
    ovhip_tmvp_cell *tmvp_host; size_t tmvp_cap, n_tmvp;
    size_t n_mv;
    size_t dmvr_first;
    size_t rows_end; int rows_pending;
    hipEvent_t ev_rows;
    hipEvent_t ev_h2d, ev_done;
    int flow_on_device;
    int flushed;
    const void *packed_prev[24];
    int resident;
    ovhip_job_stats st;
    struct BandState *bs;
    int t_stage;
    hipEvent_t t_ev[32][2]; uint8_t t_pending[32]; int t_next;
    double t_sum_ms; uint64_t t_count;
};

static void band_free(ovhip_job *j);
static int  band_reset(ovhip_job *j);
static int  band_active(const ovhip_job *j);
static int  band_wait_done(ovhip_job *j);

enum { FLOW_DEVS = 64, FLOW_DECAY = 512 };
static int g_flow_shift[FLOW_DEVS], g_flow_clean[FLOW_DEVS];
static inline int flow_shift_of(int device)
{
    const int s = __atomic_load_n(&g_flow_shift[device & (FLOW_DEVS - 1)], __ATOMIC_RELAXED);
    return s < 0 ? 0 : s > 4 ? 4 : s;
}

namespace {

__global__ __launch_bounds__(256) void k_store_host(uint4 *__restrict__ dst, const uint4 *__restrict__ src, size_t n)
{
    const size_t i = (size_t)blockIdx.x * 256 + threadIdx.x;
    if (i < n) dst[i] = src[i];
}

int store_host(ovhip_ctx *ctx, void *dst_host, const void *src_dev, size_t bytes)
{
    const size_t n = (bytes + 15) / 16;
    if (!n) return OVHIP_OK;
    hipLaunchKernelGGL(k_store_host, dim3((unsigned)((n + 255) / 256)), dim3(256), 0, ctx->stream, (uint4 *)dst_host, (const uint4 *)src_dev, n);
    OV_LAUNCH_CHECK(ctx, "k_store_host");
    return OVHIP_OK;
}

double host_now_us();
int grow_trace() { static int on = -1; if (on < 0) on = getenv("OVVC_HIP_GROW_TRACE") != nullptr; return on; }

void *pinned_alloc(void *user, size_t bytes)
{
    (void)user;
    void *p = nullptr;
    const double t0 = grow_trace() ? host_now_us() : 0.0;
    const bool ok = hipHostMalloc(&p, bytes ? bytes : 16, hipHostMallocDefault) == hipSuccess;
    if (grow_trace()) fprintf(stderr, "grow: pinned %zu bytes at %.3f ms, took %.3f ms\n", bytes, 1e-3 * t0, 1e-3 * (host_now_us() - t0));
    return ok ? p : nullptr;
}
void pinned_free(void *user, void *p) { (void)user; if (p) (void)hipHostFree(p); }

int dev_reserve(ovhip_job *j, int k, size_t bytes)
{
    DevBuf &b = j->dev[k];
    if (bytes <= b.cap) return OVHIP_OK;
    size_t nc = b.cap ? b.cap : (size_t)1 << 16;
    while (nc < bytes) nc *= 2;
    const double t0 = grow_trace() ? host_now_us() : 0.0;
    if (b.p) OV_HIP(j->ctx, hipFree(b.p));
    b.p = nullptr; b.cap = 0;
    hipError_t e = hipMalloc(&b.p, nc);
    if (grow_trace()) fprintf(stderr, "grow: device buffer %d to %zu bytes at %.3f ms, took %.3f ms\n", k, nc, 1e-3 * t0, 1e-3 * (host_now_us() - t0));
    if (e != hipSuccess) return ov_fail(j->ctx, OVHIP_ENOMEM, "hipMalloc(job buffer)", e);
    b.cap = nc;
    return OVHIP_OK;
}

enum { UP_DEVS = 64, UP_MAX = 8 };
static pthread_mutex_t g_up_mtx = PTHREAD_MUTEX_INITIALIZER;
static hipStream_t g_up[UP_DEVS][UP_MAX];
static unsigned g_up_next[UP_DEVS];
static int g_up_n = -1;
static int upload_stream_count();
static hipStream_t upload_stream_for(ovhip_job *j)
{
    const int n = upload_stream_count(), dev = j->ctx->device;
    if (n <= 0 || dev < 0 || dev >= UP_DEVS || j->t_stage >= 0) return nullptr;
    pthread_mutex_lock(&g_up_mtx);
    const unsigned k = g_up_next[dev]++ % (unsigned)n;
    if (!g_up[dev][k] && hipStreamCreateWithFlags(&g_up[dev][k], hipStreamNonBlocking) != hipSuccess) g_up[dev][k] = nullptr;
    hipStream_t st = g_up[dev][k];
    pthread_mutex_unlock(&g_up_mtx);
    return st;
}

static int upload_stream_count()
{
    if (__atomic_load_n(&g_up_n, __ATOMIC_RELAXED) < 0) {
        const char *e = getenv("OVVC_HIP_UPLOAD_STREAMS"); const int n = e ? atoi(e) : 2;
        __atomic_store_n(&g_up_n, n < 0 ? 0 : n > UP_MAX ? UP_MAX : n, __ATOMIC_RELAXED);
    }
    return __atomic_load_n(&g_up_n, __ATOMIC_RELAXED);
}

int h2d(ovhip_job *j, hipStream_t st, int k, const void *host, size_t bytes)
{
    if (!bytes) return OVHIP_OK;
    if (j->resident) return j->dev[k].cap >= bytes ? OVHIP_OK : ov_fail(j->ctx, OVHIP_EINVAL, "resident flush before a full one", hipSuccess);
    int r = dev_reserve(j, k, bytes);
    if (r) return r;
    OV_HIP(j->ctx, hipMemcpyAsync(j->dev[k].p, host, bytes, hipMemcpyHostToDevice, st));
    j->st.h2d_bytes += bytes; j->st.n_h2d++;
    return OVHIP_OK;
}

int pinned_reserve(ovhip_job *j, void **p, size_t *cap, size_t bytes)
{
    if (bytes <= *cap) return OVHIP_OK;
    size_t nc = *cap ? *cap : 4096;
    while (nc < bytes) nc *= 2;
    void *q = pinned_alloc(nullptr, nc);
    if (!q) return ov_fail(j->ctx, OVHIP_ENOMEM, "hipHostMalloc", hipSuccess);
    if (*p) { memcpy(q, *p, *cap); pinned_free(nullptr, *p); }
    *p = q; *cap = nc;
    return OVHIP_OK;
}

extern "C" const ovhip_tb_cmd *ovhip_rec_tb_cmds_split_tiny_(ovhip_recorder *r, size_t counts[4], size_t tiny[4][4], size_t *n);
extern "C" int ovhip_itx_launch_ex_(ovhip_ctx *ctx, const ovhip_pic *dst, const ovhip_pic *res, const ovhip_tb_cmd *d_cmds, uint32_t n_large,
                                    uint32_t n_small, const uint32_t tiny3[4], const int16_t *d_coefs, const int16_t *d_lmcs_scales, const uint16_t *d_bwd_lut);

extern "C" int ovhip_sao_launch_rows(ovhip_ctx *ctx, const ovhip_pic *dst, const ovhip_pic *src, const ovhip_sao_ctu *d_params, int32_t log2_ctu_s, int32_t row0, int32_t row1);
extern "C" int ovhip_alf_launch_rows(ovhip_ctx *ctx, const ovhip_pic *dst, const ovhip_pic *src, const ovhip_alf_pic *alf, int32_t row0, int32_t row1);

#define CHK(x) do { int r__ = (x); if (r__ != OVHIP_OK) return r__; } while (0)

#ifndef OVHIP_PACK_LIMIT
#define OVHIP_PACK_LIMIT (1 << 20)
#endif

double host_now_us()
{
    timespec t;
    clock_gettime(CLOCK_MONOTONIC, &t);
    return 1e6 * (double)t.tv_sec + 1e-3 * (double)t.tv_nsec;
}

int t_collect(ovhip_job *j, int k)
{
    if (!j->t_pending[k]) return OVHIP_OK;
    float ms = 0.f;
    OV_HIP(j->ctx, hipEventSynchronize(j->t_ev[k][1]));
    OV_HIP(j->ctx, hipEventElapsedTime(&ms, j->t_ev[k][0], j->t_ev[k][1]));
    j->t_sum_ms += ms; j->t_count++;
    j->t_pending[k] = 0;
    return OVHIP_OK;
}

struct StageTimer {
    ovhip_job *j; int k;
    StageTimer(ovhip_job *job, int stage) : j(job), k(-1)
    {
        if (!j || j->t_stage != stage) return;
        k = j->t_next; j->t_next = (j->t_next + 1) % 32;
        if (t_collect(j, k) != OVHIP_OK || hipEventRecord(j->t_ev[k][0], j->ctx->stream) != hipSuccess) k = -1;
    }
    ~StageTimer()
    {
        if (k >= 0 && hipEventRecord(j->t_ev[k][1], j->ctx->stream) == hipSuccess) j->t_pending[k] = 1;
    }
};

int copy_rows(ovhip_ctx *ctx, const ovhip_pic *d, const ovhip_pic *s, int32_t r0, int32_t r1)
{
    uint16_t *dp[3] = { d->y, d->cb, d->cr };
    uint16_t *sp[3] = { s->y, s->cb, s->cr };
    for (int p = 0; p < 3; ++p) {
        const size_t ds = p ? d->stride_c : d->stride_y, ss = p ? s->stride_c : s->stride_y;
        const int32_t a = p ? r0 / 2 : r0, b = p ? r1 / 2 : r1;
        OV_HIP(ctx, hipMemcpy2DAsync(dp[p] + a * ds, ds * 2, sp[p] + a * ss, ss * 2, (size_t)(p ? d->w / 2 : d->w) * 2, b - a,
                                     hipMemcpyDeviceToDevice, ctx->stream));
    }
    return OVHIP_OK;
}

int state_words(ovhip_job *j, uint32_t **words, size_t n)
{
    if (*words) return OVHIP_OK;
    OV_HIP(j->ctx, hipMalloc((void **)words, n * sizeof(uint32_t)));
    OV_HIP(j->ctx, hipMemsetAsync(*words, 0, n * sizeof(uint32_t), j->ctx->stream));
    return OVHIP_OK;
}

int ordered_arm(ovhip_job *j, uint32_t **words, size_t n)
{
    CHK(state_words(j, words, n));
    if (!j->abort_host) {
        j->abort_host = (uint32_t *)pinned_alloc(nullptr, 64);
        if (!j->abort_host) return ov_fail(j->ctx, OVHIP_ENOMEM, "pinned abort word", hipSuccess);
        *j->abort_host = 0;
    }
    if (++j->epoch >= 0x7ffffff0u) j->epoch = 1;
    return OVHIP_OK;
}

int flow_widest(const ovhip_itask *sorted, const uint32_t *items, size_t n_items)
{
    size_t widest = 0, run = 0;
    for (size_t q = 0; q < n_items; ++q) {
        run = (q && sorted[flow_item_unpack(items[q]).task].level == sorted[flow_item_unpack(items[q - 1]).task].level) ? run + 1 : 1;
        if (run > widest) widest = run;
    }
    return (int)((2 * widest + 63) & ~(size_t)63);
}

int tmvp_cells(ovhip_job *j, const ovhip_mc_unit *d_units, const int32_t *d_mv, size_t first, size_t n, int log2_ctu)
{
    ovhip_tmvp_cell *d_cells = (ovhip_tmvp_cell *)j->dev[B_TMVP].p + 4 * first;
    CHK(ovhip_tmvp_cells_launch(j->ctx, d_units, (uint32_t)(n - first), d_mv, log2_ctu, (j->w + (1 << log2_ctu) - 1) >> log2_ctu, d_cells));
    CHK(store_host(j->ctx, j->tmvp_host + 4 * first, d_cells, 4 * (n - first) * sizeof(ovhip_tmvp_cell)));
    j->n_tmvp = 4 * n;
    return OVHIP_OK;
}

struct Layout {
    size_t o = 0;
    size_t put(size_t bytes) { const size_t at = o; o += (bytes + 255) & ~(size_t)255; return at; }
};

enum { T_LCOEF, T_LCLIP, T_CCOEF, T_CCLIP, T_CC, T_FWD, T_BWD, T_COUNT };
struct Tables { size_t at[T_COUNT]; };
static const size_t TABLE_BYTES[T_COUNT] = { 24 * OVHIP_ALF_LUMA_SET_SIZE * 2, 24 * OVHIP_ALF_LUMA_SET_SIZE * 2, 8 * 7 * 2, 8 * 7 * 2, 2 * 4 * 8 * 2, 2048, 2048 };

Tables tables_put(Layout &L, bool alf, bool lmcs)
{
    Tables t;
    for (int k = 0; k < T_COUNT; ++k) t.at[k] = L.put((k < T_FWD ? alf : lmcs) ? TABLE_BYTES[k] : 0);
    return t;
}

void tables_fill(char *h, const Tables &t, const ovhip_job_params *pr, bool alf, bool lmcs)
{
    const void *src[T_COUNT] = { pr->alf_luma_coeff, pr->alf_luma_clip, pr->alf_chroma_coeff, pr->alf_chroma_clip, pr->alf_cc_coeff,
                                 lmcs ? pr->lmcs->fwd_lut : nullptr, lmcs ? pr->lmcs->bwd_lut : nullptr };
    for (int k = 0; k < T_COUNT; ++k) if (k < T_FWD ? alf : lmcs) memcpy(h + t.at[k], src[k], TABLE_BYTES[k]);
}

ovhip_alf_pic alf_pic_at(const char *d, const Tables &t, const ovhip_alf_ctu *ctus, uint8_t *class_scratch, int log2_ctu)
{
    auto tab = [&](int k) { return (const int16_t *)(d + t.at[k]); };
    return ovhip_alf_pic{ ctus, tab(T_LCOEF), tab(T_LCLIP), tab(T_CCOEF), tab(T_CCLIP), tab(T_CC), class_scratch, log2_ctu };
}

struct Chain {
    ovhip_job *j;
    ovhip_job *timer;
    const ovhip_pic *dst, *res;
    int log2_ctu;
    const ovhip_lmcs_luts *luts; const uint16_t *d_fwd; int16_t *d_scales;
    const ovhip_mc_unit *d_mc, *d_mcx; uint32_t n_mc, n_mcx;
    const ovhip_aff_unit *d_aff; uint32_t n_aff; const int32_t *d_side;
    const ovhip_rpr_unit *d_rpr; uint32_t n_rpr;
    const ovhip_aff_rpr_unit *d_affr; uint32_t n_affr;
    const ovhip_tb_cmd *d_tb; size_t cls[4], tiny[4][4]; const int16_t *d_coef;
    const ovhip_lmcs_region *d_reg; uint32_t reg0, n_reg;
    const ovhip_itask *d_it, *h_it; uint32_t n_it;
    const uint32_t *lv_start; uint32_t n_lv;
    const uint32_t *d_items; uint32_t n_items;
    int prepared;
};

int chain_predict(const Chain &c, const ovhip_pic *refs_same, const ovhip_pic *refs, uint32_t n_refs, const ovhip_pic *intra, int32_t *d_mv)
{
    ovhip_job *j = c.j;
    {
        StageTimer t_(c.timer, OVHIP_TIME_MC);
        CHK(ovhip_mc_launch(j->ctx, c.dst, refs_same, n_refs, c.d_mc, c.n_mc, c.d_fwd, intra));
        if (c.n_rpr) CHK(ovhip_mc_rpr_launch(j->ctx, c.dst, refs, n_refs, c.d_rpr, c.n_rpr, c.d_fwd, intra));
    }
    j->st.n_launches += (c.n_mc != 0) + (c.n_rpr != 0);
    if (c.n_mcx || c.n_aff) {
        StageTimer t_(c.timer, OVHIP_TIME_MCXA);
        CHK(ovhip_mcxa_launch(j->ctx, c.dst, refs_same, n_refs, c.d_mcx, c.n_mcx, d_mv, c.d_aff, c.n_aff, c.d_side, c.d_fwd));
        j->st.n_launches++;
    }
    if (c.n_affr) {
        StageTimer t_(c.timer, OVHIP_TIME_MCXA);
        CHK(ovhip_mca_rpr_launch(j->ctx, c.dst, refs, n_refs, c.d_affr, c.n_affr, c.d_side, c.d_fwd));
        j->st.n_launches++;
    }
    return OVHIP_OK;
}

int chain_residual(Chain &c, const uint16_t *d_bwd)
{
    ovhip_job *j = c.j;
    ovhip_ctx *ctx = j->ctx;
    const uint32_t t_luma[4] = { (uint32_t)c.tiny[1][0], (uint32_t)c.tiny[1][1], (uint32_t)c.tiny[1][2], (uint32_t)c.tiny[1][3] };
    const uint32_t t_chroma[4] = { (uint32_t)c.tiny[3][0], (uint32_t)c.tiny[3][1], (uint32_t)c.tiny[3][2], (uint32_t)c.tiny[3][3] };
    if (c.cls[0] + c.cls[1]) {
        StageTimer t_(c.timer, OVHIP_TIME_ITX_LUMA);
        CHK(ovhip_itx_launch_ex_(ctx, c.dst, c.res, c.d_tb, (uint32_t)c.cls[0], (uint32_t)c.cls[1], t_luma, c.d_coef, nullptr, nullptr));
        j->st.n_launches++;
    }
    if (c.n_reg) {
        if (!c.luts) return ov_fail(ctx, OVHIP_EINVAL, "chroma-scale regions recorded without LMCS tables", hipSuccess);
        StageTimer t_(c.timer, OVHIP_TIME_LMCS_SCALE);
        if (c.n_items) {
            CHK(ovhip_lmcs_scale_prepare_launch(ctx, c.dst, c.d_reg + c.reg0, c.n_reg, c.luts, c.d_scales + c.reg0, c.d_it, c.n_it, j->d_flow, j->epoch));
            c.prepared = 1;
        } else CHK(ovhip_lmcs_scale_launch(ctx, c.dst, c.d_reg + c.reg0, c.n_reg, c.luts, c.d_scales + c.reg0));
        j->st.n_launches++;
    }
    const ovhip_tb_cmd *d_tbc = c.d_tb + c.cls[0] + c.cls[1];
    StageTimer t_(c.timer, OVHIP_TIME_ITX_CHROMA);
    if (d_bwd && c.cls[3]) {
        CHK(ovhip_itx_launch_ex_(ctx, c.dst, nullptr, d_tbc, (uint32_t)c.cls[2], (uint32_t)c.cls[3], t_chroma, c.d_coef, c.d_scales, d_bwd));
        j->st.n_launches++;
        return OVHIP_OK;
    }
    if (c.cls[2] + c.cls[3]) {
        CHK(ovhip_itx_launch_ex_(ctx, c.dst, c.res, d_tbc, (uint32_t)c.cls[2], (uint32_t)c.cls[3], t_chroma, c.d_coef, c.d_scales, nullptr));
        j->st.n_launches++;
    }
    if (d_bwd) { CHK(ovhip_lmcs_inverse_launch(ctx, c.dst, d_bwd)); j->st.n_launches++; }
    return OVHIP_OK;
}

int chain_ordered(const Chain &c, int n_workers)
{
    ovhip_job *j = c.j;
    if (c.n_items) {
        CHK(ovhip_intra_flow_launch(j->ctx, c.dst, c.res, c.d_it, c.n_it, c.d_items, c.n_items, c.d_reg, c.luts, c.d_scales, c.log2_ctu,
                                    j->d_flow, j->epoch, j->abort_host, !c.prepared, n_workers));
        j->st.n_launches += 1 + !c.prepared;
        return OVHIP_OK;
    }
    for (uint32_t l = 0; l < c.n_lv; ++l) {
        const uint32_t a = c.lv_start[l], b = c.lv_start[l + 1];
        if (b > a) {
            CHK(ovhip_intra_level_launch(j->ctx, c.dst, c.res, c.d_it + a, b - a, c.d_reg, c.luts, c.d_scales, c.log2_ctu,
                                         ovhip_intra_level_geom(c.h_it + a, b - a)));
            j->st.n_launches++;
        }
    }
    return OVHIP_OK;
}

int chain_unmap(ovhip_job *j, const ovhip_pic *dst, int32_t row0, int32_t row1, const uint16_t *d_bwd, const ovhip_itask *d_it, uint32_t n_tagged)
{
    if (d_bwd) {
        ovhip_pic view = *dst;
        view.y = dst->y + (size_t)row0 * dst->stride_y; view.h = row1 - row0;
        CHK(ovhip_lmcs_inverse_untag_launch(j->ctx, &view, d_bwd, d_it, n_tagged));
    } else if (n_tagged) CHK(ovhip_intra_flow_untag_launch(j->ctx, dst, d_it, n_tagged, 1));
    else return OVHIP_OK;
    j->st.n_launches++;
    return OVHIP_OK;
}

int chain_deblock(const Chain &c, const ovhip_dbf_edge *d_ev, uint32_t n_ev, const ovhip_dbf_edge *d_eh, uint32_t n_eh, const ovhip_dbf_offsets *offs)
{
    StageTimer t_(c.timer, OVHIP_TIME_DBF);
    CHK(ovhip_dbf_launch_edges_ex(c.j->ctx, c.dst, d_ev, n_ev, d_eh, n_eh, offs));
    c.j->st.n_launches += (n_ev != 0) + (n_eh != 0);
    return OVHIP_OK;
}

int chain_filters(const Chain &c, const ovhip_sao_ctu *d_sao, const ovhip_alf_pic *alf, int32_t s0, int32_t s1, int32_t a0, int32_t a1)
{
    ovhip_job *j = c.j;
    if (s1 > s0) {
        if (d_sao) {
            StageTimer t_(c.timer, OVHIP_TIME_SAO);
            CHK(ovhip_sao_launch_rows(j->ctx, &j->tmp, c.dst, d_sao, c.log2_ctu, s0, s1));
            j->st.n_launches++;
        } else if (alf) CHK(copy_rows(j->ctx, &j->tmp, c.dst, s0, s1));
    }
    if (a1 > a0) {
        if (alf) {
            StageTimer t_(c.timer, OVHIP_TIME_ALF);
            CHK(ovhip_alf_launch_rows(j->ctx, c.dst, &j->tmp, alf, a0, a1));
            j->st.n_launches++;
        } else if (d_sao) CHK(copy_rows(j->ctx, c.dst, &j->tmp, a0, a1));
    }
    return OVHIP_OK;
}

}

extern "C" {

int ovhip_job_create(ovhip_ctx *ctx, int32_t w, int32_t h, ovhip_job **out)
{
    if (!ctx || !out || w <= 0 || h <= 0 || (w & 1) || (h & 1)) return OVHIP_EINVAL;
    OV_DEVICE(ctx);
    *out = nullptr;
    ovhip_job *j = (ovhip_job *)calloc(1, sizeof(*j));
    if (!j) return OVHIP_ENOMEM;
    j->ctx = ctx; j->home = ctx; j->w = w; j->h = h; j->t_stage = -1;
    const ovhip_allocator al = { pinned_alloc, pinned_free, nullptr };
    j->rec = ovhip_rec_create_ex(w, h, &al);
    if (!j->rec) { free(j); return OVHIP_ENOMEM; }
    ovhip_rec_set_dense_dbf_planes(j->rec, 0);
    int r = ovhip_pic_alloc(ctx, w, h, &j->tmp);
    if (r == OVHIP_OK && hipEventCreateWithFlags(&j->ev_h2d, hipEventDisableTiming) != hipSuccess) r = OVHIP_ENODEV;
    if (r == OVHIP_OK && hipEventCreateWithFlags(&j->ev_done, hipEventDisableTiming) != hipSuccess) r = OVHIP_ENODEV;
    if (r == OVHIP_OK && hipEventCreateWithFlags(&j->ev_rows, hipEventDisableTiming) != hipSuccess) r = OVHIP_ENODEV;
    if (r != OVHIP_OK) { ovhip_job_destroy(j); return r; }
    *out = j;
    return OVHIP_OK;
}

void ovhip_job_destroy(ovhip_job *j)
{
    if (!j) return;
    (void)hipSetDevice(j->ctx->device);
    if (j->flushed) (void)hipEventSynchronize(j->ev_done);
    for (int k = 0; k < B_COUNT; ++k) if (j->dev[k].p) (void)hipFree(j->dev[k].p);
    if (j->tmp.y) (void)ovhip_pic_free(j->ctx, &j->tmp);
    if (j->res.y) (void)ovhip_pic_free(j->ctx, &j->res);
    if (j->d_sync) (void)hipFree(j->d_sync);
    if (j->d_flow) (void)hipFree(j->d_flow);
    pinned_free(nullptr, j->items_host);
    pinned_free(nullptr, j->abort_host);
    pinned_free(nullptr, j->param_host); pinned_free(nullptr, j->mv_host); pinned_free(nullptr, j->tmvp_host);
    for (int k = 0; k < 32; ++k) for (int q = 0; q < 2; ++q) if (j->t_ev[k][q]) (void)hipEventDestroy(j->t_ev[k][q]);
    if (j->ev_h2d) (void)hipEventDestroy(j->ev_h2d);
    if (j->ev_done) (void)hipEventDestroy(j->ev_done);
    if (j->ev_rows) { if (j->rows_pending) (void)hipEventSynchronize(j->ev_rows); (void)hipEventDestroy(j->ev_rows); }
    band_free(j);
    ovhip_rec_destroy(j->rec);
    free(j);
}

ovhip_recorder *ovhip_job_recorder(ovhip_job *j) { return j ? j->rec : nullptr; }

int ovhip_job_reserve_for_picture(ovhip_job *j)
{
    if (!j) return OVHIP_EINVAL;
    OV_DEVICE(j->ctx);
    if (ovhip_rec_reserve_for_picture(j->rec) != OVHIP_OK) return ov_fail(j->ctx, OVHIP_ENOMEM, "ovhip_rec_reserve_for_picture", hipSuccess);
    const size_t P = (size_t)j->w * j->h;
    const struct { int k; size_t bytes; } want[] = {
        { B_TB, (P / 64 + 1024) * sizeof(ovhip_tb_cmd) }, { B_COEF, (P / 2 + 1024) * 2 }, { B_MC, (P / 128 + 1024) * sizeof(ovhip_mc_unit) },
        { B_MCX, (P / 256 + 1024) * sizeof(ovhip_mc_unit) }, { B_MV, (P / 256 + 1024) * 16 }, { B_AFF, (P / 1024 + 256) * sizeof(ovhip_aff_unit) },
        { B_SIDE, (P / 6 + 1024) * 4 }, { B_REG, (P / 4096 + 64) * sizeof(ovhip_lmcs_region) }, { B_SCALE, 65536 },
        { B_EV, (P / 32 + 2048) * sizeof(ovhip_dbf_edge) }, { B_EH, (P / 32 + 2048) * sizeof(ovhip_dbf_edge) }, { B_PARAM, P / 2 + ((size_t)2 << 20) },
        { B_CLASS, (size_t)((j->w + 3) / 4) * ((j->h + 3) / 4) }, { B_ITASK, (P / 64 + 1024) * sizeof(ovhip_itask) }, { B_IITEM, (P / 32 + 1024) * 4 },
        { B_TMVP, 4 * (P / 256 + 1024) * sizeof(ovhip_tmvp_cell) },
    };
    for (const auto &q : want) CHK(dev_reserve(j, q.k, q.bytes));
    CHK(pinned_reserve(j, (void **)&j->param_host, &j->param_cap, P / 2 + ((size_t)2 << 20)));
    CHK(pinned_reserve(j, (void **)&j->mv_host, &j->mv_cap, (P / 256 + 1024) * 16));
    CHK(pinned_reserve(j, (void **)&j->tmvp_host, &j->tmvp_cap, 4 * (P / 256 + 1024) * sizeof(ovhip_tmvp_cell)));
    CHK(pinned_reserve(j, (void **)&j->items_host, &j->items_cap, (P / 32 + 1024) * sizeof(uint32_t)));
    if (!j->res.y) CHK(ovhip_pic_alloc(j->ctx, j->w, j->h, &j->res));
    return OVHIP_OK;
}

int ovhip_job_begin(ovhip_job *j)
{
    if (!j) return OVHIP_EINVAL;
    OV_DEVICE(j->ctx);
    if (j->flushed) OV_HIP(j->ctx, hipEventSynchronize(j->ev_h2d));
    if (j->rows_pending) { OV_HIP(j->ctx, hipEventSynchronize(j->ev_rows)); j->rows_pending = 0; }
    { const int rb = band_reset(j); if (rb != OVHIP_OK) return rb; }
    ovhip_rec_reset(j->rec);
    j->dmvr_first = 0; j->n_mv = 0; j->n_tmvp = 0; j->rows_end = 0;
    return OVHIP_OK;
}

int ovhip_job_bind(ovhip_job *j, ovhip_ctx *ctx)
{
    if (!j) return OVHIP_EINVAL;
    if (!ctx) ctx = j->home;
    if (ctx->device != j->ctx->device) return ov_fail(ctx, OVHIP_EINVAL, "ovhip_job_bind: context of another device", hipSuccess);
    OV_DEVICE(ctx);
    if (j->flushed) {
        hipError_t e = hipEventSynchronize(j->ev_done);
        if (e != hipSuccess) return ov_fail(ctx, OVHIP_ELAUNCH, "ovhip_job_bind: hipEventSynchronize(previous flush)", e);
    }
    j->ctx = ctx;
    return OVHIP_OK;
}

static int job_flush_impl(ovhip_job *j, const ovhip_pic *dst, const ovhip_pic *refs, uint32_t n_refs, const ovhip_pic *intra,
                          const ovhip_job_params *pr);

int ovhip_job_wait(ovhip_job *j)
{
    if (!j) return OVHIP_EINVAL;
    OV_DEVICE(j->ctx);
    if (!j->flushed) return OVHIP_OK;
    hipError_t e = hipEventSynchronize(j->ev_done);
    if (e != hipSuccess) return ov_fail(j->ctx, OVHIP_ELAUNCH, "hipEventSynchronize(job)", e);
    if (band_active(j)) return band_wait_done(j);
    if (j->abort_host && *(volatile uint32_t *)j->abort_host) {
        *(volatile uint32_t *)j->abort_host = 0;
        const int fd = j->ctx->device & (FLOW_DEVS - 1);
        if (!j->test_abort_seen) {
            if (__atomic_load_n(&g_flow_shift[fd], __ATOMIC_RELAXED) < 4) __atomic_fetch_add(&g_flow_shift[fd], 1, __ATOMIC_RELAXED);
            __atomic_store_n(&g_flow_clean[fd], 0, __ATOMIC_RELAXED);
        }
        j->test_abort_seen = 0;
        if (j->d_sync) (void)hipMemset(j->d_sync, 0, sizeof(uint32_t));
        if (j->d_flow) (void)hipMemset(j->d_flow, 0, sizeof(uint32_t));
        j->flow_launched = 0;
        if (j->again.valid && j->n_retries == 0) {
            j->n_retries = 1;
            ovhip_job_params pr = j->again.pr;
            pr.stages = ((pr.stages ? pr.stages : (uint32_t)(OVHIP_STAGE_MC | OVHIP_STAGE_ITX | OVHIP_STAGE_DBF | OVHIP_STAGE_SAO | OVHIP_STAGE_ALF | OVHIP_STAGE_INTRA)) | OVHIP_STAGE_INTRA_LEVELS) & ~(uint32_t)OVHIP_STAGE_INTRA_CTU;
            pr.wait_events = nullptr; pr.n_wait_events = 0; pr.before_launch = nullptr;
            int r = job_flush_impl(j, &j->again.dst, j->again.refs, j->again.n_refs, j->again.has_intra ? &j->again.intra : nullptr, &pr);
            if (r) return r;
            e = hipEventSynchronize(j->ev_done);
            if (e != hipSuccess) return ov_fail(j->ctx, OVHIP_ELAUNCH, "hipEventSynchronize(job, second pass)", e);
            return OVHIP_OK;
        }
        return ov_fail(j->ctx, OVHIP_ELAUNCH, "ordered pass: a CTU's bounded wait for its neighbours expired (picture incomplete)", hipSuccess);
    }
    if (j->flow_launched) {
        const int fd = j->ctx->device & (FLOW_DEVS - 1);
        j->flow_launched = 0;
        if (__atomic_load_n(&g_flow_shift[fd], __ATOMIC_RELAXED) > 0 && __atomic_add_fetch(&g_flow_clean[fd], 1, __ATOMIC_RELAXED) == FLOW_DECAY) {
            __atomic_store_n(&g_flow_clean[fd], 0, __ATOMIC_RELAXED);
            int cur = __atomic_load_n(&g_flow_shift[fd], __ATOMIC_RELAXED);
            while (cur > 0 && !__atomic_compare_exchange_n(&g_flow_shift[fd], &cur, cur - 1, true, __ATOMIC_RELAXED, __ATOMIC_RELAXED)) {}
        }
    }
    return OVHIP_OK;
}

const int32_t *ovhip_job_refined_mvs(ovhip_job *j, size_t *n_units)
{
    if (!j || !n_units) return nullptr;
    *n_units = j->n_mv;
    return j->mv_host;
}

const ovhip_tmvp_cell *ovhip_job_tmvp_cells(ovhip_job *j, size_t *n_entries)
{
    if (!j || !n_entries) return nullptr;
    *n_entries = j->n_tmvp;
    return j->tmvp_host;
}

int ovhip_job_last_stats(const ovhip_job *j, ovhip_job_stats *out)
{
    if (!j || !out) return OVHIP_EINVAL;
    *out = j->st;
    return OVHIP_OK;
}

int ovhip_job_time_stage(ovhip_job *j, int stage)
{
    if (!j || stage < -1 || stage >= OVHIP_TIME_COUNT) return OVHIP_EINVAL;
    OV_DEVICE(j->ctx);
    for (int k = 0; k < 32; ++k) {
        CHK(t_collect(j, k));
        for (int q = 0; q < 2 && stage >= 0; ++q)
            if (!j->t_ev[k][q]) OV_HIP(j->ctx, hipEventCreate(&j->t_ev[k][q]));
    }
    j->t_stage = stage; j->t_sum_ms = 0.0; j->t_count = 0;
    return OVHIP_OK;
}

int ovhip_job_stage_time(ovhip_job *j, double *sum_ms, uint64_t *count)
{
    if (!j || !sum_ms || !count) return OVHIP_EINVAL;
    OV_DEVICE(j->ctx);
    for (int k = 0; k < 32; ++k) CHK(t_collect(j, k));
    *sum_ms = j->t_sum_ms; *count = j->t_count;
    return OVHIP_OK;
}

int64_t ovhip_job_dmvr_rows_collect(ovhip_job *j)
{
    if (!j) return OVHIP_EINVAL;
    if (j->rows_pending) {
        ovhip_ctx *ctx = j->ctx;
        OV_DEVICE(ctx);
        hipError_t e = hipEventSynchronize(j->ev_rows);
        j->rows_pending = 0;
        if (e != hipSuccess) return ov_fail(ctx, OVHIP_ELAUNCH, "hipEventSynchronize(dmvr rows)", e);
        if (j->rows_end > j->n_mv) j->n_mv = j->rows_end;
    }
    return (int64_t)j->rows_end;
}

int64_t ovhip_job_dmvr_rows_begin_upto(ovhip_job *j, const ovhip_pic *refs, uint32_t n_refs, int32_t log2_ctu_s, size_t upto);
int64_t ovhip_job_dmvr_rows_begin(ovhip_job *j, const ovhip_pic *refs, uint32_t n_refs, int32_t log2_ctu_s)
{
    return ovhip_job_dmvr_rows_begin_upto(j, refs, n_refs, log2_ctu_s, (size_t)-1);
}

int64_t ovhip_job_dmvr_rows_begin_upto(ovhip_job *j, const ovhip_pic *refs, uint32_t n_refs, int32_t log2_ctu_s, size_t upto)
{
    if (!j) return OVHIP_EINVAL;
    const int64_t c = ovhip_job_dmvr_rows_collect(j);
    if (c < 0) return c;
    ovhip_ctx *ctx = j->ctx;
    OV_DEVICE(ctx);
    size_t n = 0;
    const ovhip_mc_unit *u = ovhip_rec_mcx_units(j->rec, &n);
    if (n > upto) n = upto;
    const size_t first = j->dmvr_first;
    if (n <= first) return (int64_t)first;
    int any = 0;
    for (size_t i = first; i < n && !any; ++i) any = (u[i].flags & OVHIP_MC_DMVR) != 0;
    if (any) {
        CHK(pinned_reserve(j, (void **)&j->mv_host, &j->mv_cap, n * 16));
        if (log2_ctu_s) CHK(pinned_reserve(j, (void **)&j->tmvp_host, &j->tmvp_cap, 4 * n * sizeof(ovhip_tmvp_cell)));
        if (j->dev[B_MCX].cap < n * sizeof(ovhip_mc_unit) || j->dev[B_MV].cap < n * 16 ||
            (log2_ctu_s && j->dev[B_TMVP].cap < 4 * n * sizeof(ovhip_tmvp_cell))) {
            const size_t ub = (size_t)((j->w + 7) / 8) * ((j->h + 7) / 8);
            CHK(dev_reserve(j, B_MCX, (ub > n ? ub : n) * sizeof(ovhip_mc_unit)));
            CHK(dev_reserve(j, B_MV, (ub > n ? ub : n) * 16));
            if (log2_ctu_s) CHK(dev_reserve(j, B_TMVP, 4 * (ub > n ? ub : n) * sizeof(ovhip_tmvp_cell)));
        }
        char *d_units = (char *)j->dev[B_MCX].p + first * sizeof(ovhip_mc_unit);
        int32_t *d_mv = (int32_t *)j->dev[B_MV].p + 4 * first;
        OV_HIP(ctx, hipMemcpyAsync(d_units, u + first, (n - first) * sizeof(ovhip_mc_unit), hipMemcpyHostToDevice, ctx->stream));
        ovhip_pic geom = j->tmp, same[16];
        CHK(ovhip_dmvr_search_launch(ctx, &geom, same_size_refs(&geom, refs, n_refs, same), n_refs, (const ovhip_mc_unit *)d_units,
                                     (uint32_t)(n - first), d_mv));
        CHK(store_host(ctx, j->mv_host + 4 * first, d_mv, (n - first) * 16));
        if (log2_ctu_s) CHK(tmvp_cells(j, (const ovhip_mc_unit *)d_units, d_mv, first, n, log2_ctu_s));
        OV_HIP(ctx, hipEventRecord(j->ev_rows, ctx->stream));
        j->rows_pending = 1;
    }
    else if (log2_ctu_s) {
        CHK(pinned_reserve(j, (void **)&j->tmvp_host, &j->tmvp_cap, 4 * n * sizeof(ovhip_tmvp_cell)));
        for (size_t i = 4 * first; i < 4 * n; ++i) { j->tmvp_host[i] = ovhip_tmvp_cell{}; j->tmvp_host[i].cell = OVHIP_TMVP_NONE; }
        j->n_tmvp = 4 * n;
    }
    j->dmvr_first = n;
    j->rows_end = n;
    return (int64_t)n;
}

int64_t ovhip_job_dmvr_rows(ovhip_job *j, const ovhip_pic *refs, uint32_t n_refs)
{
    const int64_t n = ovhip_job_dmvr_rows_begin(j, refs, n_refs, 0);
    return n < 0 ? n : ovhip_job_dmvr_rows_collect(j);
}

int ovhip_job_flush(ovhip_job *j, const ovhip_pic *dst, const ovhip_pic *refs, uint32_t n_refs, const ovhip_pic *intra,
                    const ovhip_job_params *pr)
{
    if (!j || !dst || !pr) return OVHIP_EINVAL;
    j->again.valid = 0;
    j->n_retries = 0;
    const int r = job_flush_impl(j, dst, refs, n_refs, intra, pr);
    j->again.valid = r == OVHIP_OK && n_refs <= 16;
    j->again.dst = *dst;
    for (uint32_t i = 0; i < n_refs && i < 16; ++i) j->again.refs[i] = refs[i];
    j->again.n_refs = n_refs;
    j->again.has_intra = intra != nullptr;
    if (intra) j->again.intra = *intra;
    j->again.pr = *pr;
    return r;
}

int ovhip_job_test_abort_next_flow(ovhip_job *j)
{
    if (!j) return OVHIP_EINVAL;
    j->test_abort = 1;
    return OVHIP_OK;
}

static int job_flush_impl(ovhip_job *j, const ovhip_pic *dst, const ovhip_pic *refs, uint32_t n_refs, const ovhip_pic *intra,
                          const ovhip_job_params *pr)
{
    ovhip_ctx *ctx = j->ctx;
    OV_DEVICE(ctx);
    if ((dst->w != j->w || dst->h != j->h)) return ov_fail(ctx, OVHIP_EINVAL, "ovhip_job_flush: picture size differs from the job's", hipSuccess);
    { const int64_t c_ = ovhip_job_dmvr_rows_collect(j); if (c_ < 0) return (int)c_; }
    const uint32_t stages = pr->stages ? pr->stages : UINT32_MAX;
    const int log2_ctu = pr->log2_ctu_s ? pr->log2_ctu_s : 7;
    if (log2_ctu < 5 || log2_ctu > 7) return ov_fail(ctx, OVHIP_EINVAL, "ovhip_job_flush: log2_ctu_s", hipSuccess);
    const size_t n_ctu = (size_t)((j->w + (1 << log2_ctu) - 1) >> log2_ctu) * ((j->h + (1 << log2_ctu) - 1) >> log2_ctu);
    memset(&j->st, 0, sizeof(j->st));
    j->st.n_ordered_retries = j->n_retries;
    const double t_flush0 = host_now_us();
    j->resident = (stages & OVHIP_STAGE_RESIDENT) && pr->stages;
    ovhip_recorder *rec = j->rec;
    const bool no_upload = j->resident;

    size_t cls[4] = { 0, 0, 0, 0 }, n_tb = 0, n_coef = 0, n_mc = 0, n_mcx = 0, n_aff = 0, n_side = 0, n_reg = 0, n_ev = 0, n_eh = 0;
    const ovhip_tb_cmd *tb;
    size_t tiny[4][4] = { { 0, 0, 0, 0 }, { 0, 0, 0, 0 }, { 0, 0, 0, 0 }, { 0, 0, 0, 0 } };
    tb = ovhip_rec_tb_cmds_split_tiny_(rec, cls, tiny, &n_tb);
    if (!tb && n_tb) return ov_fail(ctx, OVHIP_ENOMEM, "ovhip_rec_tb_cmds_split", hipSuccess);
    const int16_t *coef = ovhip_rec_coefs(rec, &n_coef);
    const ovhip_mc_unit *mc = ovhip_rec_mc_units(rec, &n_mc);
    const ovhip_mc_unit *mcx = ovhip_rec_mcx_units(rec, &n_mcx);
    const ovhip_aff_unit *aff = ovhip_rec_aff_units(rec, &n_aff);
    const int32_t *side = ovhip_rec_aff_side(rec, &n_side);
    const ovhip_lmcs_region *reg = ovhip_rec_lmcs_regions(rec, &n_reg);
    size_t n_ciip = 0;
    const ovhip_ciip_unit *ciip = ovhip_rec_ciip_units(rec, &n_ciip);
    if (n_ciip && !intra)
        return ov_fail(ctx, OVHIP_EUNSUP, "ovhip_job_flush: CIIP blend units recorded but no picture with their intra prediction", hipSuccess);
    size_t n_rpr = 0;
    const ovhip_rpr_unit *rpr = ovhip_rec_rpr_units(rec, &n_rpr);
    size_t n_affr = 0;
    const ovhip_aff_rpr_unit *affr = ovhip_rec_aff_rpr_units(rec, &n_affr);
    size_t n_it = 0, n_ictu = 0; uint32_t n_lv = 0; const uint32_t *lv_start = nullptr; const ovhip_ictu *ictu = nullptr;
    const int by_ctu = pr->stages && (stages & OVHIP_STAGE_INTRA_CTU);
    int by_flow = !by_ctu && !(pr->stages && (stages & OVHIP_STAGE_INTRA_LEVELS));
    if (j->resident && by_flow && !j->flow_on_device) by_flow = 0;
    const int by_level = !by_ctu;
    const ovhip_itask *it;
    it = by_level ? ovhip_rec_itasks_sorted(rec, &n_it, &lv_start, &n_lv)
                       : ovhip_rec_itasks_by_ctu(rec, pr->log2_ctu_s ? pr->log2_ctu_s : 7, &n_it, &ictu, &n_ictu);
    size_t n_items = 0;
    if (by_flow && n_it) {
        n_items = ovhip_intra_flow_items_(it, n_it, j->items_host, j->items_cap / sizeof(uint32_t));
        if (n_items > j->items_cap / sizeof(uint32_t)) {
            CHK(pinned_reserve(j, (void **)&j->items_host, &j->items_cap, n_items * sizeof(uint32_t)));
            n_items = ovhip_intra_flow_items_(it, n_it, j->items_host, n_items);
        }
        if (!n_items) by_flow = 0;
    }
    if (!it && ovhip_rec_itask_levels(rec)) return ov_fail(ctx, OVHIP_ENOMEM, "ovhip_job_flush: sorting the ordered tasks", hipSuccess);
    if (!by_level) n_lv = ovhip_rec_itask_levels(rec);
    if (!(stages & OVHIP_STAGE_INTRA)) { n_it = 0; n_lv = 0; n_ictu = 0; }
    const int ordered = n_it != 0;
    const bool flow = (stages & OVHIP_STAGE_INTRA) && by_flow && n_items;
    if (ordered && !j->res.y) CHK(ovhip_pic_alloc(ctx, j->w, j->h, &j->res));
    if (ordered && (dst->stride_y != j->res.stride_y || dst->stride_c != j->res.stride_c))
        return ov_fail(ctx, OVHIP_EUNSUP, "ovhip_job_flush: pictures with ordered tasks need tight planes (stride = width)", hipSuccess);
    j->st.n_itasks = (uint32_t)n_it; j->st.n_ilevels = n_lv;
    ovhip_dbf_offsets offs;
    const ovhip_dbf_edge *ev = ovhip_rec_dbf_edges(rec, 0, &n_ev, &offs);
    const ovhip_dbf_edge *eh = ovhip_rec_dbf_edges(rec, 1, &n_eh, nullptr);
    j->st.n_tb = (uint32_t)n_tb; j->st.n_mc = (uint32_t)n_mc; j->st.n_mcx = (uint32_t)n_mcx; j->st.n_aff = (uint32_t)n_aff;
    j->st.n_edges_v = (uint32_t)n_ev; j->st.n_edges_h = (uint32_t)n_eh; j->st.n_regions = (uint32_t)n_reg;

    const int sao_on = pr->sao && (stages & OVHIP_STAGE_SAO), alf_on = pr->alf_ctus && (stages & OVHIP_STAGE_ALF);
    if (alf_on && (!pr->alf_luma_coeff || !pr->alf_luma_clip || !pr->alf_chroma_coeff || !pr->alf_chroma_clip || !pr->alf_cc_coeff))
        return ov_fail(ctx, OVHIP_EINVAL, "ovhip_job_flush: ALF tables missing", hipSuccess);
    Layout L;
    const size_t o_sao = L.put(sao_on ? n_ctu * sizeof(ovhip_sao_ctu) : 0), o_alf = L.put(alf_on ? n_ctu * sizeof(ovhip_alf_ctu) : 0);
    const Tables tabs = tables_put(L, alf_on, pr->lmcs != nullptr);
#ifdef OVHIP_TUNING
    static const size_t PACK_LIMIT = getenv("OVHIP_X_PACK_LIMIT") ? (size_t)atol(getenv("OVHIP_X_PACK_LIMIT")) : (size_t)OVHIP_PACK_LIMIT;
#else
    const size_t PACK_LIMIT = OVHIP_PACK_LIMIT;
#endif
    struct Small { const void *host; size_t bytes; int buf; size_t at; } small[] = {
        { mc, n_mc * sizeof(*mc), B_MC, 0 }, { tb, n_tb * sizeof(*tb), B_TB, 0 }, { coef, n_coef * sizeof(*coef), B_COEF, 0 },
        { it, n_it * sizeof(*it), B_ITASK, 0 }, { ictu, n_ictu * sizeof(*ictu), B_ICTU, 0 },
        { j->items_host, by_flow ? n_items * sizeof(uint32_t) : 0, B_IITEM, 0 },
        { mcx, n_mcx * sizeof(*mcx), B_MCX, 0 }, { ciip, n_ciip * sizeof(*ciip), B_CIIP, 0 }, { aff, n_aff * sizeof(*aff), B_AFF, 0 },
        { side, n_side * sizeof(*side), B_SIDE, 0 }, { reg, n_reg * sizeof(*reg), B_REG, 0 },
        { rpr, n_rpr * sizeof(*rpr), B_RPR, 0 }, { affr, n_affr * sizeof(*affr), B_AFFR, 0 },
        { ev, (stages & OVHIP_STAGE_DBF) ? n_ev * sizeof(*ev) : 0, B_EV, 0 }, { eh, (stages & OVHIP_STAGE_DBF) ? n_eh * sizeof(*eh) : 0, B_EH, 0 },
    };
    static_assert(B_COUNT <= 24, "packed_prev");
    const void *packed[24] = { nullptr };
    for (auto &sm : small) if (sm.bytes && sm.bytes <= PACK_LIMIT && !j->resident) sm.at = L.put(sm.bytes) + 1;
    if (L.o) {
        CHK(pinned_reserve(j, (void **)&j->param_host, &j->param_cap, L.o));
        char *ph = j->param_host;
        for (auto &sm : small) if (sm.at) memcpy(ph + sm.at - 1, sm.host, sm.bytes);
        if (sao_on) memcpy(ph + o_sao, pr->sao, n_ctu * sizeof(ovhip_sao_ctu));
        if (alf_on) memcpy(ph + o_alf, pr->alf_ctus, n_ctu * sizeof(ovhip_alf_ctu));
        tables_fill(ph, tabs, pr, alf_on, pr->lmcs != nullptr);
    }

    const double t_flush1 = host_now_us();
    const hipStream_t up = no_upload ? nullptr : upload_stream_for(j), ust = up ? up : ctx->stream;
    if (up) {
        hipError_t e0 = hipSuccess;
        if (j->flushed) e0 = hipStreamWaitEvent(up, j->ev_done, 0);
        if (e0 == hipSuccess && j->rows_pending) e0 = hipStreamWaitEvent(up, j->ev_rows, 0);
        if (e0 != hipSuccess) return ov_fail(ctx, OVHIP_ENODEV, "ovhip_job_flush: upload stream", e0);
    }
    auto upload = [&]() -> int {
        StageTimer t_(j, OVHIP_TIME_H2D);
        CHK(h2d(j, ust, B_PARAM, j->param_host, L.o));
        if (n_mcx) {
            CHK(dev_reserve(j, B_MV, n_mcx * 16));
            CHK(pinned_reserve(j, (void **)&j->mv_host, &j->mv_cap, n_mcx * 16));
        }
        if (n_reg) CHK(dev_reserve(j, B_SCALE, n_reg * 2));
        for (auto &sm : small) {
            if (j->resident) continue;
            if (sm.at) packed[sm.buf] = (const char *)j->dev[B_PARAM].p + sm.at - 1;
            else CHK(h2d(j, ust, sm.buf, sm.host, sm.bytes));
        }
        return OVHIP_OK;
    };
    const int r_up = upload();
    OV_HIP(ctx, hipEventRecord(j->ev_h2d, ust));
    j->flushed = 1;
    if (r_up != OVHIP_OK) return r_up;
    if (up) OV_HIP(ctx, hipStreamWaitEvent(ctx->stream, j->ev_h2d, 0));
    if (no_upload) memcpy(packed, j->packed_prev, sizeof(packed)); else { memcpy(j->packed_prev, packed, sizeof(packed)); j->flow_on_device = by_flow && n_items; }
    auto DEV = [&](int k) -> const void * { return packed[k] ? packed[k] : j->dev[k].p; };
    const double t_flush2 = host_now_us();
    for (uint32_t i = 0; i < pr->n_wait_events; ++i)
        if (pr->wait_events && pr->wait_events[i]) {
            if (pr->wait_on_host) OV_HIP(ctx, hipEventSynchronize((hipEvent_t)pr->wait_events[i]));
            else OV_HIP(ctx, hipStreamWaitEvent(ctx->stream, (hipEvent_t)pr->wait_events[i], 0));
        }
    if (pr->before_launch && pr->before_launch(pr->before_launch_user))
        return ov_fail(ctx, OVHIP_EINVAL, "ovhip_job_flush: before_launch callback failed", hipSuccess);
#ifdef OVHIP_TUNING
    static const int X_H2D_HOSTWAIT = getenv("OVHIP_X_H2D_HOSTWAIT") ? atoi(getenv("OVHIP_X_H2D_HOSTWAIT")) : 0;
    static const int X_MV_D2H = getenv("OVHIP_X_MV_D2H") ? atoi(getenv("OVHIP_X_MV_D2H")) : 3;
    if (X_H2D_HOSTWAIT && !j->resident) OV_HIP(ctx, hipEventSynchronize(j->ev_h2d));
#else
    const int X_MV_D2H = 3;
#endif
    const double t_flush3 = host_now_us();
    j->st.host_us_prepare = (uint32_t)(t_flush1 - t_flush0); j->st.host_us_upload = (uint32_t)(t_flush2 - t_flush1);
    j->st.host_us_wait = (uint32_t)(t_flush3 - t_flush2);

    const char *dp = (const char *)j->dev[B_PARAM].p;
    const uint16_t *d_bwd = pr->lmcs ? (const uint16_t *)(dp + tabs.at[T_BWD]) : nullptr;
    Chain c = {};
    c.j = j; c.timer = j; c.dst = dst; c.res = ordered ? &j->res : nullptr; c.log2_ctu = log2_ctu;
    c.luts = pr->lmcs; c.d_fwd = pr->lmcs ? (const uint16_t *)(dp + tabs.at[T_FWD]) : nullptr; c.d_scales = (int16_t *)j->dev[B_SCALE].p;
    c.d_mc = (const ovhip_mc_unit *)DEV(B_MC); c.n_mc = (uint32_t)n_mc; c.d_mcx = (const ovhip_mc_unit *)DEV(B_MCX); c.n_mcx = (uint32_t)n_mcx;
    c.d_aff = (const ovhip_aff_unit *)DEV(B_AFF); c.n_aff = (uint32_t)n_aff; c.d_side = (const int32_t *)DEV(B_SIDE);
    c.d_rpr = (const ovhip_rpr_unit *)DEV(B_RPR); c.n_rpr = (uint32_t)n_rpr;
    c.d_affr = (const ovhip_aff_rpr_unit *)DEV(B_AFFR); c.n_affr = (uint32_t)n_affr;
    c.d_tb = (const ovhip_tb_cmd *)DEV(B_TB); memcpy(c.cls, cls, sizeof(cls)); memcpy(c.tiny, tiny, sizeof(tiny)); c.d_coef = (const int16_t *)DEV(B_COEF);
    c.d_reg = (const ovhip_lmcs_region *)DEV(B_REG); c.n_reg = (uint32_t)n_reg;
    c.d_it = (const ovhip_itask *)DEV(B_ITASK); c.h_it = it; c.n_it = (uint32_t)n_it; c.lv_start = lv_start; c.n_lv = n_lv;
    c.d_items = (const uint32_t *)DEV(B_IITEM); c.n_items = flow ? (uint32_t)n_items : 0;

    if (stages & OVHIP_STAGE_MC) {
        const bool mv_direct = n_mcx && !pr->tmvp_cells && !j->resident && X_MV_D2H == 3;
        ovhip_pic same[16];
        CHK(chain_predict(c, same_size_refs(dst, refs, n_refs, same), refs, n_refs, intra, mv_direct ? j->mv_host : (int32_t *)j->dev[B_MV].p));
        if (mv_direct) j->st.d2h_bytes += n_mcx * 16;
        else if (n_mcx && !j->resident && X_MV_D2H) {
            if (X_MV_D2H == 3) CHK(store_host(ctx, j->mv_host, j->dev[B_MV].p, n_mcx * 16));
            else OV_HIP(ctx, hipMemcpyAsync(j->mv_host, j->dev[B_MV].p, n_mcx * 16, hipMemcpyDeviceToHost, ctx->stream));
            j->st.d2h_bytes += n_mcx * 16;
        }
        j->n_mv = n_mcx;
        j->n_tmvp = 0;
        if (n_mcx && pr->tmvp_cells) {
            const size_t bytes = 4 * n_mcx * sizeof(ovhip_tmvp_cell);
            CHK(dev_reserve(j, B_TMVP, bytes));
            CHK(pinned_reserve(j, (void **)&j->tmvp_host, &j->tmvp_cap, bytes));
            CHK(tmvp_cells(j, c.d_mcx, (const int32_t *)j->dev[B_MV].p, 0, n_mcx, log2_ctu));
            j->st.n_launches++; j->st.d2h_bytes += bytes;
        }
        if (n_ciip) { CHK(ovhip_ciip_launch(ctx, dst, intra, (const ovhip_ciip_unit *)DEV(B_CIIP), (uint32_t)n_ciip)); j->st.n_launches++; }
    }
    if (flow) {
        CHK(ordered_arm(j, &j->d_flow, ovhip_intra_flow_words(j->w, j->h)));
        if (j->test_abort && j->n_retries == 0) {
            j->test_abort = 0; j->test_abort_seen = 1;
            OV_HIP(ctx, hipMemsetAsync(j->d_flow, 0xff, sizeof(uint32_t), ctx->stream));
            *(volatile uint32_t *)j->abort_host = 1;
        }
    }
    if (stages & OVHIP_STAGE_ITX) CHK(chain_residual(c, ordered ? nullptr : d_bwd));
    if (ordered) {
        StageTimer t_(j, OVHIP_TIME_INTRA);
        if (!by_level) {
            CHK(ordered_arm(j, &j->d_sync, ovhip_intra_sync_words(j->w, j->h, 5)));
            CHK(ovhip_intra_ctu_launch(ctx, dst, &j->res, c.d_it, (const ovhip_ictu *)DEV(B_ICTU), (uint32_t)n_ictu, c.d_reg, pr->lmcs, c.d_scales,
                                       log2_ctu, j->d_sync, j->epoch, j->abort_host));
            j->st.n_launches++;
        } else {
#ifdef OVHIP_TUNING
            static const long WORKERS = getenv("OVHIP_FLOW_WORKERS") ? atol(getenv("OVHIP_FLOW_WORKERS")) : -1;
#else
            static const long WORKERS = -1;
#endif
            int n_workers = pr->flow_workers ? (int)pr->flow_workers : (WORKERS >= 0 ? (int)WORKERS : (6 * ctx->num_cus) >> flow_shift_of(ctx->device));
            if (flow && !pr->flow_workers && WORKERS < 0) {
                const int want = flow_widest(it, j->items_host, n_items);
                if (want < n_workers) n_workers = want < 64 ? 64 : want;
            }
            if (n_workers < 1) n_workers = 1;
            CHK(chain_ordered(c, n_workers));
            if (flow) { j->flow_launched = 1; j->st.flow_shift = (uint32_t)flow_shift_of(ctx->device); }
        }
        CHK(chain_unmap(j, dst, 0, j->h, (pr->lmcs && (stages & OVHIP_STAGE_ITX)) ? d_bwd : nullptr, c.d_it, c.n_items ? c.n_it : 0u));
    }
    if (stages & OVHIP_STAGE_DBF)
        CHK(chain_deblock(c, (const ovhip_dbf_edge *)DEV(B_EV), (uint32_t)n_ev, (const ovhip_dbf_edge *)DEV(B_EH), (uint32_t)n_eh, &offs));
    ovhip_alf_pic ap;
    if (alf_on) {
        CHK(dev_reserve(j, B_CLASS, (size_t)((j->w + 3) / 4) * ((j->h + 3) / 4)));
        ap = alf_pic_at(dp, tabs, (const ovhip_alf_ctu *)(dp + o_alf), (uint8_t *)j->dev[B_CLASS].p, log2_ctu);
    }
    CHK(chain_filters(c, sao_on ? (const ovhip_sao_ctu *)(dp + o_sao) : nullptr, alf_on ? &ap : nullptr, 0, j->h, 0, j->h));
    OV_HIP(ctx, hipEventRecord(j->ev_done, ctx->stream));
    j->st.host_us_launch = (uint32_t)(host_now_us() - t_flush3);
    return OVHIP_OK;
}

}

extern "C" void ovhip_rec_tb_split_range_(const ovhip_recorder *r, size_t first, size_t n, ovhip_tb_cmd *out, size_t counts[4], size_t tiny[4][4]);
extern "C" int  ovhip_rec_itasks_sorted_range_(const ovhip_recorder *r, size_t first, size_t n, ovhip_itask *out, uint32_t *level_start, size_t cap, uint32_t *n_levels);

enum { MAX_BANDS = 96, ARENA_CHUNKS = 16, BAND_LEVELS = 4096 };
struct ArenaChunk { char *host, *dev; size_t cap, used; };
struct BandRec {
    int32_t row0, row1;
    ovhip_band_counts c0, c1;
    const ovhip_itask *d_it; uint32_t n_it; int tagged;
    const ovhip_dbf_edge *d_ev, *d_eh; uint32_t n_ev, n_eh;
    int flow_charge;
    int32_t rows_final;
};
struct BandState {
    int active, n, tails, closed, failed;
    ovhip_pic dst;
    ovhip_band_counts cur;
    int32_t row_prev, dbf_rows, sao_rows, alf_rows, rows_final;
    int log2_ctu, sao_on, alf_on, filters_latched;
    uint32_t stages;
    const uint16_t *d_fwd, *d_bwd; int lmcs_up;
    ovhip_alf_pic d_alf; int alf_up;
    ovhip_lmcs_luts luts; int have_luts;
    ovhip_dbf_offsets offs;
    ArenaChunk chunk[ARENA_CHUNKS]; int n_chunks, cur_chunk;
    BandRec band[MAX_BANDS];
    hipEvent_t ev_recon[MAX_BANDS], ev_tail[MAX_BANDS];
    uint32_t level_start[BAND_LEVELS + 2];
    void *last_event; int32_t last_rows;
    uint16_t *keep; int keep_valid;
};

__global__ __launch_bounds__(256) void k_band_row(ovhip_pic pic, uint16_t *keep, int row_y, int mode, unsigned mask)
{
    const int i = blockIdx.x * 256 + threadIdx.x, w = pic.w, wc = w >> 1;
    if (i >= 2 * w) return;
    uint16_t *p = i < w ? pic.y + (size_t)row_y * pic.stride_y + i
                        : (i < w + wc ? pic.cb + (size_t)(row_y >> 1) * pic.stride_c + (i - w) : pic.cr + (size_t)(row_y >> 1) * pic.stride_c + (i - w - wc));
    uint16_t *unf = keep + i, *fil = keep + 2 * w + i;
    if (mode == 0) *unf = *p;
    else if (mode == 1) { *fil = *p; *p = (uint16_t)(*unf & mask); }
    else *p = *fil;
}
static int band_row(ovhip_job *j, const ovhip_pic *pic, int row_y, int mode, unsigned mask)
{
    hipLaunchKernelGGL(k_band_row, dim3((2 * pic->w + 255) / 256), dim3(256), 0, j->ctx->stream, *pic, j->bs->keep, row_y, mode, mask);
    OV_LAUNCH_CHECK(j->ctx, "k_band_row");
    j->st.n_launches++;
    return OVHIP_OK;
}


static int g_band_flow_inflight[FLOW_DEVS];
static int band_flow_take(ovhip_ctx *ctx, int want)
{
    const int fd = ctx->device & (FLOW_DEVS - 1), cap = 12 * ctx->num_cus;
    int cur = __atomic_load_n(&g_band_flow_inflight[fd], __ATOMIC_RELAXED);
    for (;;) {
        int give = cap - cur < want ? cap - cur : want;
        give &= ~63;
        if (give < 64) return 0;
        if (__atomic_compare_exchange_n(&g_band_flow_inflight[fd], &cur, cur + give, true, __ATOMIC_RELAXED, __ATOMIC_RELAXED)) return give;
    }
}
static void band_flow_give(ovhip_ctx *ctx, int n) { if (n) __atomic_fetch_sub(&g_band_flow_inflight[ctx->device & (FLOW_DEVS - 1)], n, __ATOMIC_RELAXED); }

static void band_flow_reclaim(ovhip_job *j, int wait)
{
    BandState *bs = j->bs;
    for (int b = 0; bs && b <= bs->n && b < MAX_BANDS; ++b) {
        BandRec &B = bs->band[b];
        if (!B.flow_charge) continue;
        if (wait) (void)hipEventSynchronize(bs->ev_recon[b]);
        else if (hipEventQuery(bs->ev_recon[b]) != hipSuccess) { (void)hipGetLastError(); break; }
        band_flow_give(j->ctx, B.flow_charge);
        B.flow_charge = 0;
    }
}

static int band_active(const ovhip_job *j) { return j->bs && j->bs->active; }

static void band_free(ovhip_job *j)
{
    BandState *bs = j->bs;
    if (!bs) return;
    band_flow_reclaim(j, 1);
    for (int i = 0; i < bs->n_chunks; ++i) { pinned_free(nullptr, bs->chunk[i].host); if (bs->chunk[i].dev) (void)hipFree(bs->chunk[i].dev); }
    for (int i = 0; i < MAX_BANDS; ++i) { if (bs->ev_recon[i]) (void)hipEventDestroy(bs->ev_recon[i]); if (bs->ev_tail[i]) (void)hipEventDestroy(bs->ev_tail[i]); }
    if (bs->keep) (void)hipFree(bs->keep);
    free(bs);
    j->bs = nullptr;
}

static int band_reset(ovhip_job *j)
{
    BandState *bs = j->bs;
    if (!bs) return OVHIP_OK;
    band_flow_reclaim(j, 1);
    if (bs->n_chunks > 1) {
        size_t total = 0;
        if (j->flushed) OV_HIP(j->ctx, hipEventSynchronize(j->ev_done));
        for (int i = 0; i < bs->n_chunks; ++i) { total += bs->chunk[i].cap; pinned_free(nullptr, bs->chunk[i].host); if (bs->chunk[i].dev) (void)hipFree(bs->chunk[i].dev); }
        memset(bs->chunk, 0, sizeof(bs->chunk));
        bs->n_chunks = 0;
        total += total / 4;
        bs->chunk[0].host = (char *)pinned_alloc(nullptr, total);
        if (!bs->chunk[0].host) return ov_fail(j->ctx, OVHIP_ENOMEM, "band arena (pinned)", hipSuccess);
        if (hipMalloc((void **)&bs->chunk[0].dev, total) != hipSuccess) { pinned_free(nullptr, bs->chunk[0].host); bs->chunk[0].host = nullptr; return ov_fail(j->ctx, OVHIP_ENOMEM, "band arena (device)", hipSuccess); }
        bs->chunk[0].cap = total; bs->n_chunks = 1;
    }
    for (int i = 0; i < bs->n_chunks; ++i) bs->chunk[i].used = 0;
    bs->cur_chunk = 0;
    bs->active = 0; bs->n = 0; bs->tails = 0; bs->closed = 0; bs->failed = 0;
    return OVHIP_OK;
}

static int arena_take(ovhip_job *j, size_t bytes, char **host, char **dev)
{
    BandState *bs = j->bs;
    bytes = (bytes + 255) & ~(size_t)255;
    for (;;) {
        if (bs->cur_chunk < bs->n_chunks) {
            ArenaChunk &c = bs->chunk[bs->cur_chunk];
            if (c.cap - c.used >= bytes) { *host = c.host + c.used; *dev = c.dev + c.used; c.used += bytes; return OVHIP_OK; }
            bs->cur_chunk++;
            continue;
        }
        if (bs->n_chunks == ARENA_CHUNKS) return ov_fail(j->ctx, OVHIP_ENOMEM, "band arena: too many chunks", hipSuccess);
        size_t cap = bs->n_chunks ? 2 * bs->chunk[bs->n_chunks - 1].cap : ((size_t)j->w * j->h * 3 / 2 < ((size_t)4 << 20) ? (size_t)4 << 20 : (size_t)j->w * j->h * 3 / 2);
        while (cap < bytes) cap *= 2;
        ArenaChunk &c = bs->chunk[bs->n_chunks];
        c.host = (char *)pinned_alloc(nullptr, cap);
        if (!c.host) return ov_fail(j->ctx, OVHIP_ENOMEM, "band arena (pinned)", hipSuccess);
        if (hipMalloc((void **)&c.dev, cap) != hipSuccess) { pinned_free(nullptr, c.host); c.host = nullptr; return ov_fail(j->ctx, OVHIP_ENOMEM, "band arena (device)", hipSuccess); }
        c.cap = cap; c.used = 0;
        bs->n_chunks++;
    }
// ... 300 lines not shown
```

### openvvc_amd/engine.py

```python
from __future__ import annotations

import ctypes as C

import numpy as np

from . import capi


class EngineError(RuntimeError):
    pass


class Context:
    def __init__(self, device: int = 0, stream: int | None = None):
        self.lib = capi.load()
        h = C.c_void_p()
        r = self.lib.ovhip_ctx_create(C.byref(h), device, C.c_void_p(stream) if stream else None)
        if r != 0:
            raise EngineError(f"ovhip_ctx_create(device={device}) failed: {r} (no HIP device? the engine has no CPU fallback)")
        self.h = h
        self._bufs = []

    def _chk(self, r, what):
        if r != 0:
# ... 367 lines not shown
            k = self.wl.tb_classes
            if self.lmcs is not None and k[3]:
                c.itx_chroma_lmcs(self.dst, self.tb_cmds, self.coefs, k[0] + k[1], k[2], k[3], self.lmcs_scales, self.lmcs_bwd)
            elif k[2] + k[3]:
                c.itx_classes(self.dst, self.tb_cmds, self.coefs, k[0] + k[1], k[2], k[3], self.lmcs_scales)
        elif name == "lmcs_inv":
            if self.lmcs is not None and not self.wl.tb_classes[3]:
                c.lmcs_inverse(self.dst, self.lmcs_bwd)
        elif name == "dbf":
            c.dbf_edges(self.dst, self.dbf_v, self.dbf_h, self.wl.dbf_planes["beta_offset"], self.wl.dbf_planes["tc_offset"])
        elif name == "sao":
            c.sao(self.tmp, self.dst, self.sao_params, self.log2_ctu)
        elif name == "alf":
            c.alf(self.dst, self.tmp, self.alf)
        else:
            raise ValueError(name)

    def decode(self, stages=STAGES):
        for s in stages:
            self.run_stage(s)

    def result(self):
        self.ctx.sync()
        return self.dst.download()

    def refined_mvs(self) -> np.ndarray:
        self.ctx.sync()
        return self.mv_out.download(np.int32).reshape(-1, 4) if self.mv_out else np.zeros((0, 4), np.int32)

    def free(self):
        for b in self.bufs + [self.dbf_planes, self.alf]:
            b.free()
        for p in self.refs + [self.dst, self.tmp] + ([self.intra] if self.intra else []):
            p.free()


class Job:

    def __init__(self, ctx: Context, w: int, h: int):
        self.ctx, self.lib, self.w, self.h = ctx, ctx.lib, w, h
        j = C.c_void_p()
        ctx._chk(self.lib.ovhip_job_create(ctx.h, w, h, C.byref(j)), "job_create")
        self.j = j
        self.rec = capi.Recorder.__new__(capi.Recorder)
        self.rec.lib, self.rec.h, self.rec._keep = self.lib, self.lib.ovhip_job_recorder(j), []
        self._keep = {}

    def close(self):
        if self.j:
            self.rec.h = None
            self.lib.ovhip_job_destroy(self.j)
            self.j = None

    def begin(self):
        self.ctx._chk(self.lib.ovhip_job_begin(self.j), "job_begin")

    def load_workload(self, wl):
        self.begin()
        r = self.rec
        for which, arr in ((capi.REC_COEF, wl.coefs), (capi.REC_TB, wl.tb_cmds), (capi.REC_MC, wl.mc_units),
                           (capi.REC_MCX, wl.mcx_units), (capi.REC_AFF, wl.aff_units), (capi.REC_SIDE, wl.aff_side),
                           (capi.REC_REGION, wl.lmcs_regions), (capi.REC_CIIP, wl.ciip_units), (capi.REC_ITASK, wl.itasks),
                           (capi.REC_EDGE_V, wl.dbf_edges[0]), (capi.REC_EDGE_H, wl.dbf_edges[1])):
            if arr is not None and len(arr):
                r.append_raw(which, arr)
        offs = capi.DbfOffsets()
        for i in range(8):
            offs.beta[i], offs.tc[i] = wl.dbf_planes["beta_offset"], wl.dbf_planes["tc_offset"]
        self.ctx._chk(self.lib.ovhip_rec_set_dbf_offsets(r.h, C.byref(offs), 1), "set_dbf_offsets")
        self.params = self.make_params(wl)

    def make_params(self, wl, log2_ctu: int = 7, stages: int = 0) -> "capi.JobParams":
        keep = self._keep
        keep["sao"] = np.ascontiguousarray(wl.sao_params)
        keep["alf"] = {k: np.ascontiguousarray(wl.alf[k], dtype=dt) for k, dt in capi.ALF_TABLES}
        keep["lmcs"] = wl.lmcs
        a = keep["alf"]
        p = capi.JobParams()
        p.lmcs = C.addressof(wl.lmcs) if wl.lmcs is not None else None
        p.sao = keep["sao"].ctypes.data
        p.alf_ctus = a["ctus"].ctypes.data
        p.alf_luma_coeff, p.alf_luma_clip = a["luma_coeff"].ctypes.data, a["luma_clip"].ctypes.data
        p.alf_chroma_coeff, p.alf_chroma_clip = a["chroma_coeff"].ctypes.data, a["chroma_clip"].ctypes.data
        p.alf_cc_coeff = a["cc_coeff"].ctypes.data
        p.log2_ctu_s, p.stages = log2_ctu, stages
        return p

    def flush(self, dst: "DevPic", refs: list, intra: "DevPic | None" = None, params=None):
        arr = (capi.Pic * max(len(refs), 1))(*[r.s for r in refs])
        self.ctx._chk(self.lib.ovhip_job_flush(self.j, C.byref(dst.s), arr, len(refs), C.byref(intra.s) if intra else None,
                                               C.byref(params if params is not None else self.params)), "job_flush")

    def wait(self):
        self.ctx._chk(self.lib.ovhip_job_wait(self.j), "job_wait")

    def band(self, dst: "DevPic", refs: list, row_end: int, last: bool = False, upto: "capi.BandCounts | None" = None, params=None):
        arr = (capi.Pic * max(len(refs), 1))(*[r.s for r in refs])
        self.ctx._chk(self.lib.ovhip_job_band(self.j, C.byref(dst.s), arr, len(refs), C.byref(params if params is not None else self.params),
                                              C.byref(upto) if upto is not None else None, row_end, int(last)), "job_band")

    def band_progress(self) -> int:
        rows = C.c_int32()
        self.ctx._chk(self.lib.ovhip_job_band_progress(self.j, C.byref(rows), None, None), "job_band_progress")
        return rows.value

    def flush_in_bands(self, wl, dst: "DevPic", refs: list, ctu_rows_per_band: int = 1, log2_ctu: int = 7, params=None):
        rows = list(range(ctu_rows_per_band << log2_ctu, self.h, ctu_rows_per_band << log2_ctu))
        cuts = band_counts(wl, rows, log2_ctu)
        for r, c in zip(rows, cuts):
            self.band(dst, refs, r, False, c, params)
        self.band(dst, refs, self.h, True, None, params)

    def bind(self, ctx: "Context"):
        self.ctx._chk(self.lib.ovhip_job_bind(self.j, ctx.h), "job_bind")
        self.ctx = ctx

    def dmvr_rows(self, refs: list) -> int:
        arr = (capi.Pic * max(len(refs), 1))(*[r.s for r in refs])
        n = self.lib.ovhip_job_dmvr_rows(self.j, arr, len(refs))
        if n < 0:
            self.ctx._chk(int(n), "job_dmvr_rows")
        return int(n)

    def dmvr_rows_begin(self, refs: list, log2_ctu: int = 0) -> int:
        arr = (capi.Pic * max(len(refs), 1))(*[r.s for r in refs])
        n = self.lib.ovhip_job_dmvr_rows_begin(self.j, arr, len(refs), log2_ctu)
        if n < 0:
            self.ctx._chk(int(n), "job_dmvr_rows_begin")
        return int(n)

    def dmvr_rows_collect(self) -> int:
        n = self.lib.ovhip_job_dmvr_rows_collect(self.j)
        if n < 0:
            self.ctx._chk(int(n), "job_dmvr_rows_collect")
        return int(n)

    def refined_mvs(self) -> np.ndarray:
        n = C.c_size_t()
        p = self.lib.ovhip_job_refined_mvs(self.j, C.byref(n))
        if not n.value:
            return np.zeros((0, 4), np.int32)
        return np.frombuffer((C.c_int32 * (4 * n.value)).from_address(p), dtype=np.int32).reshape(-1, 4).copy()

    def tmvp_cells(self) -> np.ndarray:
        n = C.c_size_t()
        p = self.lib.ovhip_job_tmvp_cells(self.j, C.byref(n))
        if not n.value:
            return np.zeros(0, capi.TMVP_CELL_DTYPE)
        return np.ctypeslib.as_array(C.cast(p, C.POINTER(C.c_uint8)), (n.value * capi.TMVP_CELL_DTYPE.itemsize,)).view(capi.TMVP_CELL_DTYPE).copy()

    def test_abort_next_flow(self):
        self.ctx._chk(self.lib.ovhip_job_test_abort_next_flow(self.j), "job_test_abort_next_flow")

    def stats(self) -> "capi.JobStats":
        s = capi.JobStats()
        self.lib.ovhip_job_last_stats(self.j, C.byref(s))
        return s

    def time_stage(self, name: "str | None"):
        self.ctx._chk(self.lib.ovhip_job_time_stage(self.j, capi.TIME_STAGES.index(name) if name else -1), "job_time_stage")

    def stage_time(self):
        s, n = C.c_double(), C.c_uint64()
        self.ctx._chk(self.lib.ovhip_job_stage_time(self.j, C.byref(s), C.byref(n)), "job_stage_time")
        return s.value * 1e-3, n.value


def band_counts(wl, rows, log2_ctu: int = 7) -> list:
    def cut(ctu_row, what):
        ctu_row = np.asarray(ctu_row, np.int64)
        if len(ctu_row) > 1 and (np.diff(ctu_row) < 0).any():
            raise EngineError(f"band_counts: {what} are not in CTU-row order")
        return [int(np.searchsorted(ctu_row, r >> log2_ctu, side="left")) for r in rows]

    def arr(a, dt):
        return np.zeros(0, dt) if a is None or not len(a) else np.asarray(a).view(dt).reshape(-1)

    tb, mc, mcx = arr(wl.tb_cmds, capi.TB_CMD_DTYPE), arr(wl.mc_units, capi.MC_UNIT_DTYPE), arr(wl.mcx_units, capi.MC_UNIT_DTYPE)
    aff, reg, it = arr(wl.aff_units, capi.AFF_UNIT_DTYPE), arr(wl.lmcs_regions, capi.LMCS_REGION_DTYPE), arr(wl.itasks, capi.ITASK_DTYPE)
    ev, eh = arr(wl.dbf_edges[0], capi.DBF_EDGE_DTYPE), arr(wl.dbf_edges[1], capi.DBF_EDGE_DTYPE)
    n_coef = 0 if wl.coefs is None else len(wl.coefs)
    n_side = 0 if wl.aff_side is None else len(wl.aff_side)
    tb_row = (tb["y"].astype(np.int64) << (tb["plane"] != 0)) >> log2_ctu
    it_chroma = (it["kind"] == capi.IT_CHROMA) | (it["kind"] == capi.IT_RES_C)
    it_row = (it["y"].astype(np.int64) << it_chroma) >> log2_ctu
    k_tb, k_mc, k_mcx = cut(tb_row, "transform blocks"), cut(mc["y"] >> log2_ctu, "MC units"), cut(mcx["y"] >> log2_ctu, "refined units")
    k_aff, k_reg, k_it = cut(aff["y"] >> log2_ctu, "affine units"), cut(reg["y"] >> log2_ctu, "regions"), cut(it_row, "ordered tasks")
    k_ev = cut((ev["uy"].astype(np.int64) << 2) >> log2_ctu, "vertical edges")
    k_eh = cut((eh["uy"].astype(np.int64) << 2) >> log2_ctu, "horizontal edges")
    out = []
    for i in range(len(rows)):
        c = capi.BandCounts()
        c.n_tb, c.n_mc, c.n_mcx, c.n_aff, c.n_reg, c.n_itask, c.n_edge_v, c.n_edge_h = k_tb[i], k_mc[i], k_mcx[i], k_aff[i], k_reg[i], k_it[i], k_ev[i], k_eh[i]
        later = tb["coef_off"][k_tb[i]:]
        c.n_coef = int(later.min()) if len(later) else n_coef
        la = aff[k_aff[i]:]
        c.n_side = int(min(la["side_off"].min(), la["prof_off"][(la["flags"] & 1) != 0].min(initial=0xffffffff))) if len(la) else n_side
        out.append(c)
    return out


class Dpb:

    def __init__(self, devices=(0,), ops: "capi.DpbOps | None" = None, n_devices: int | None = None):
        self.lib = capi.load()
        h = C.c_void_p()
        if ops is not None:
            self._ops = ops
            r = self.lib.ovhip_dpb_create_ex(C.byref(h), n_devices or 1, C.byref(ops))
        else:
            arr = (C.c_int * len(devices))(*devices)
            r = self.lib.ovhip_dpb_create(C.byref(h), arr, len(devices))
        if r != 0:
            raise EngineError(f"ovhip_dpb_create: {r} (no HIP device? the DPB has no CPU back-end outside the tests' own)")
        self.h = h

    def close(self):
        if self.h:
            self.lib.ovhip_dpb_destroy(self.h)
            self.h = None

    def stats(self) -> "capi.DpbStats":
        st = capi.DpbStats()
        self.lib.ovhip_dpb_get_stats(self.h, C.byref(st))
        return st

    def begin(self, key: int, dev: int, w: int, h: int, tag: int = 0) -> "capi.Pic":
        pic = capi.Pic()
        r = self.lib.ovhip_dpb_begin_tag(self.h, C.c_void_p(key), tag, dev, w, h, C.byref(pic))
        if r != 0:
            raise EngineError(f"ovhip_dpb_begin: {r}")
        return pic

    def lookup(self, key: int) -> "tuple[int, capi.Pic]":
        pic, dev = capi.Pic(), C.c_int()
        r = self.lib.ovhip_dpb_lookup(self.h, C.c_void_p(key), C.byref(dev), C.byref(pic))
        if r != 0:
            raise EngineError(f"ovhip_dpb_lookup: {r}")
        return dev.value, pic


class Frame:

    def __init__(self, dpb: Dpb, dev: int, w: int, h: int):
        self.lib, self.dpb, self.w, self.h = dpb.lib, dpb, w, h
        f = C.c_void_p()
        r = self.lib.ovhip_frame_create(dpb.h, dev, w, h, C.byref(f))
        if r != 0:
            raise EngineError(f"ovhip_frame_create: {r}")
        self.f = f

    def _chk(self, r, what):
        if r < 0:
            raise EngineError(f"{what}: {r}: {self.lib.ovhip_frame_last_error(self.f).decode()}")
        return r

    def close(self):
        if self.f:
            self.lib.ovhip_frame_destroy(self.f)
            self.f = None

    def begin(self, key: int, tag: int = 0):
        self._chk(self.lib.ovhip_frame_begin_tag(self.f, C.c_void_p(key), tag), "frame_begin")

    def ref(self, key: int, tag: int = 0) -> int:
        return self._chk(self.lib.ovhip_frame_ref_tag(self.f, C.c_void_p(key), tag), "frame_ref")

    def ref_at(self, slot: int, key: int) -> int:
        return self._chk(self.lib.ovhip_frame_ref_at(self.f, slot, C.c_void_p(key)), "frame_ref_at")

    def recorder(self) -> "capi.Recorder":
        r = capi.Recorder.__new__(capi.Recorder)
        r.lib, r.h, r._keep = self.lib, self.lib.ovhip_frame_recorder(self.f), []
        if not r.h:
            raise EngineError("ovhip_frame_recorder")
        r.close = lambda: None
        return r

    def dmvr_rows(self) -> int:
        return int(self._chk(self.lib.ovhip_frame_dmvr_rows(self.f), "frame_dmvr_rows"))

    def dmvr_rows_begin(self, log2_ctu: int = 7) -> int:
        return int(self._chk(self.lib.ovhip_frame_dmvr_rows_begin(self.f, log2_ctu), "frame_dmvr_rows_begin"))

    def dmvr_rows_collect(self) -> int:
        return int(self._chk(self.lib.ovhip_frame_dmvr_rows_collect(self.f), "frame_dmvr_rows_collect"))

    def submit(self, params: "capi.JobParams", job: "Job | None" = None, out: "capi.FrameOutput | None" = None, check: bool = True) -> int:
        r = self.lib.ovhip_frame_submit(self.f, job.j if job is not None else None, None, C.byref(params), C.byref(out) if out is not None else None)
        return self._chk(r, "frame_submit") if check else r

    def fail(self, status: int = -3):
        self.lib.ovhip_frame_fail(self.f, status)

    def set_output_scale(self, out_w: int, out_h: int, scale_window=(0, 0, 0, 0), col=(0, 0), check: bool = True) -> int:
        info = capi.ScaleInfo(*scale_window, *col)
        r = self.lib.ovhip_frame_set_output_scale(self.f, out_w, out_h, C.byref(info))
        if r < 0 and check:
            raise EngineError(f"frame_set_output_scale: {r}")
        return r

    def job(self) -> "Job":
        j = Job.__new__(Job)
        ctx = Context.__new__(Context)
        ctx.lib, ctx.h, ctx._bufs = self.lib, C.c_void_p(self.lib.ovhip_frame_ctx(self.f)), []
        j.ctx, j.lib, j.w, j.h, j.j, j._keep = ctx, self.lib, self.w, self.h, C.c_void_p(self.lib.ovhip_frame_job(self.f)), {}
# ... 119 lines not shown
```

Baseline: 3601.

## Fold LMCS inverse unmap and tag stripping into deblocking and SAO loads

Drops the separate full-picture unmap pass that applied the LMCS backward LUT and removed intra-flow tags before deblocking. Instead, deblocking and SAO decode samples as they load them (mask tag bits, apply the LUT to luma that lacks the linear tag). Deblocking marks its outputs with a linear tag so SAO does not map them a second time. The LUT is staged in LDS by default. This removes one full read-write pass over the picture, at the cost of extra per-sample work, LDS staging and a barrier in both kernels, and it relies on SAO being enabled to strip tags from every sample.

```diff
diff --git a/include/ovvc_hip.h b/include/ovvc_hip.h
--- a/include/ovvc_hip.h
+++ b/include/ovvc_hip.h
@@ -869,6 +869,7 @@
 int  ovhip_stream_set_output_scale(ovhip_stream *s, int32_t out_w, int32_t out_h, const ovhip_scale_info *info);
 const void *ovhip_stream_key(const ovhip_stream *s, uint32_t idx);
 int  ovhip_job_test_abort_next_flow(ovhip_job *job);
+int  ovhip_job_test_separate_unmap(ovhip_job *job, int on);
 
 #ifdef __cplusplus
 }
diff --git a/openvvc_amd/capi.py b/openvvc_amd/capi.py
--- a/openvvc_amd/capi.py
+++ b/openvvc_amd/capi.py
@@ -556,6 +556,7 @@
         "ovhip_host_alloc": (vp, [C.c_size_t]),
         "ovhip_host_free": (None, [vp]),
         "ovhip_job_test_abort_next_flow": (C.c_int, [vp]),
+        "ovhip_job_test_separate_unmap": (C.c_int, [vp, C.c_int]),
         "ovhip_dpb_create": (C.c_int, [P(vp), P(C.c_int), C.c_int]),
         "ovhip_dpb_create_ex": (C.c_int, [P(vp), C.c_int, P(DpbOps)]),
         "ovhip_dpb_destroy": (None, [vp]),
@@ -650,7 +651,7 @@
     "ovhip_job_flush", "ovhip_job_wait", "ovhip_job_refined_mvs", "ovhip_job_dmvr_rows", "ovhip_job_dmvr_rows_begin", "ovhip_job_dmvr_rows_collect", "ovhip_job_last_stats", "ovhip_job_time_stage", "ovhip_job_stage_time",
     "ovhip_output_bytes", "ovhip_output_rows", "ovhip_output_pack_launch", "ovhip_output_row_md5_launch", "ovhip_output_bands", "ovhip_output_tree_md5_launch", "ovhip_pic_output", "ovhip_pic_digest",
     "ovhip_md5_init", "ovhip_md5_update", "ovhip_md5_final", "ovhip_tmvp_cells_launch", "ovhip_job_tmvp_cells", "ovhip_intra_flow_untag_launch", "ovhip_lmcs_inverse_untag_launch", "ovhip_lmcs_scale_prepare_launch",
-    "ovhip_host_alloc", "ovhip_host_free", "ovhip_d2d", "ovhip_job_test_abort_next_flow",
+    "ovhip_host_alloc", "ovhip_host_free", "ovhip_d2d", "ovhip_job_test_abort_next_flow", "ovhip_job_test_separate_unmap",
     "ovhip_dpb_create", "ovhip_dpb_create_ex", "ovhip_dpb_destroy", "ovhip_dpb_n_devices", "ovhip_dpb_device", "ovhip_dpb_begin", "ovhip_dpb_want",
     "ovhip_dpb_publish", "ovhip_dpb_acquire", "ovhip_dpb_wait_copy", "ovhip_dpb_poll_tag", "ovhip_frame_refs_ready", "ovhip_dpb_set_unknown_key_timeout", "ovhip_dpb_unpin", "ovhip_dpb_release", "ovhip_dpb_lookup", "ovhip_dpb_shutdown",
     "ovhip_dpb_get_stats", "ovhip_dpb_begin_tag", "ovhip_dpb_want_tag", "ovhip_dpb_acquire_tag", "ovhip_frame_begin_tag", "ovhip_frame_ref_tag", "ovhip_frame_set_trace",
diff --git a/openvvc_amd/csrc/kernels_dbf.hip b/openvvc_amd/csrc/kernels_dbf.hip
--- a/openvvc_amd/csrc/kernels_dbf.hip
+++ b/openvvc_amd/csrc/kernels_dbf.hip
@@ -54,6 +54,7 @@
     return ((abs(P(3) - P(0)) + abs(Q(3) - Q(0))) < (beta >> 3)) && (abs(P(0) - Q(0)) < ((tc * 5 + 1) >> 1));
 }
 
+template <int TAG = 0>
 __device__ __forceinline__ void long_regs(const int *s, uint16_t *pix, int step, int tc, int lp, int lq)
 {
     const int f7[7] = { 59, 50, 41, 32, 23, 14, 5 }, f5[5] = { 58, 45, 32, 19, 6 }, f3[3] = { 53, 32, 11 };
@@ -77,12 +78,12 @@
         if (i < lp) {
             const int f = lp == 7 ? f7[i] : (lp == 5 ? f5[i < 5 ? i : 0] : f3[i < 3 ? i : 0]);
             const int cv = (tc * (lp == 3 ? t3[i < 3 ? i : 0] : t7[i])) >> 1;
-            pix[(-1 - i) * step] = (uint16_t)ov_clip3((mid * f + ref_p * (64 - f) + 32) >> 6, P(i) - cv, P(i) + cv);
+            pix[(-1 - i) * step] = (uint16_t)(ov_clip3((mid * f + ref_p * (64 - f) + 32) >> 6, P(i) - cv, P(i) + cv) | TAG);
         }
         if (i < lq) {
             const int f = lq == 7 ? f7[i] : (lq == 5 ? f5[i < 5 ? i : 0] : f3[i < 3 ? i : 0]);
             const int cv = (tc * (lq == 3 ? t3[i < 3 ? i : 0] : t7[i])) >> 1;
-            pix[i * step] = (uint16_t)ov_clip3((mid * f + ref_q * (64 - f) + 32) >> 6, Q(i) - cv, Q(i) + cv);
+            pix[i * step] = (uint16_t)(ov_clip3((mid * f + ref_q * (64 - f) + 32) >> 6, Q(i) - cv, Q(i) + cv) | TAG);
         }
     }
 }
@@ -94,15 +95,16 @@
     long_regs(s, pix, step, tc, lp, lq);
 }
 
+template <int TAG = 0>
 __device__ __forceinline__ void strong_regs(const int *s, uint16_t *pix, int step, int tc)
 {
     const int p3 = P(3), p2 = P(2), p1 = P(1), p0 = P(0), q0 = Q(0), q1 = Q(1), q2 = Q(2), q3 = Q(3);
-    pix[-3 * step] = (uint16_t)ov_clip3((2 * p3 + 3 * p2 + p1 + p0 + q0 + 4) >> 3, p2 - tc, p2 + tc);
-    pix[-2 * step] = (uint16_t)ov_clip3((p2 + p1 + p0 + q0 + 2) >> 2, p1 - 2 * tc, p1 + 2 * tc);
-    pix[-1 * step] = (uint16_t)ov_clip3((p2 + 2 * p1 + 2 * p0 + 2 * q0 + q1 + 4) >> 3, p0 - 3 * tc, p0 + 3 * tc);
-    pix[0]         = (uint16_t)ov_clip3((p1 + 2 * p0 + 2 * q0 + 2 * q1 + q2 + 4) >> 3, q0 - 3 * tc, q0 + 3 * tc);
-    pix[1 * step]  = (uint16_t)ov_clip3((p0 + q0 + q1 + q2 + 2) >> 2, q1 - 2 * tc, q1 + 2 * tc);
-    pix[2 * step]  = (uint16_t)ov_clip3((p0 + q0 + q1 + 3 * q2 + 2 * q3 + 4) >> 3, q2 - tc, q2 + tc);
+    pix[-3 * step] = (uint16_t)(ov_clip3((2 * p3 + 3 * p2 + p1 + p0 + q0 + 4) >> 3, p2 - tc, p2 + tc) | TAG);
+    pix[-2 * step] = (uint16_t)(ov_clip3((p2 + p1 + p0 + q0 + 2) >> 2, p1 - 2 * tc, p1 + 2 * tc) | TAG);
+    pix[-1 * step] = (uint16_t)(ov_clip3((p2 + 2 * p1 + 2 * p0 + 2 * q0 + q1 + 4) >> 3, p0 - 3 * tc, p0 + 3 * tc) | TAG);
+    pix[0]         = (uint16_t)(ov_clip3((p1 + 2 * p0 + 2 * q0 + 2 * q1 + q2 + 4) >> 3, q0 - 3 * tc, q0 + 3 * tc) | TAG);
+    pix[1 * step]  = (uint16_t)(ov_clip3((p0 + q0 + q1 + q2 + 2) >> 2, q1 - 2 * tc, q1 + 2 * tc) | TAG);
+    pix[2 * step]  = (uint16_t)(ov_clip3((p0 + q0 + q1 + 3 * q2 + 2 * q3 + 4) >> 3, q2 - tc, q2 + tc) | TAG);
 }
 
 __device__ __forceinline__ void strong_line(uint16_t *pix, int step, int tc)
@@ -112,6 +114,7 @@
     strong_regs(s, pix, step, tc);
 }
 
+template <int TAG = 0>
 __device__ __forceinline__ void weak_regs(const int *s, uint16_t *pix, int step, int tc, bool ext_p, bool ext_q)
 {
     const int p2 = P(2), p1 = P(1), p0 = P(0), q0 = Q(0), q1 = Q(1), q2 = Q(2);
@@ -121,10 +124,10 @@
         delta = ov_clip3(delta, -tc, tc);
         const int d1 = ov_clip3((((p2 + p0 + 1) >> 1) - p1 + delta) >> 1, -tc2p, tc2p);
         const int d2 = ov_clip3((((q2 + q0 + 1) >> 1) - q1 - delta) >> 1, -tc2q, tc2q);
-        pix[-2 * step] = (uint16_t)ov_clip_bd(p1 + d1);
-        pix[-1 * step] = (uint16_t)ov_clip_bd(p0 + delta);
-        pix[0]         = (uint16_t)ov_clip_bd(q0 - delta);
-        pix[1 * step]  = (uint16_t)ov_clip_bd(q1 + d2);
+        pix[-2 * step] = (uint16_t)(ov_clip_bd(p1 + d1) | TAG);
+        pix[-1 * step] = (uint16_t)(ov_clip_bd(p0 + delta) | TAG);
+        pix[0]         = (uint16_t)(ov_clip_bd(q0 - delta) | TAG);
+        pix[1 * step]  = (uint16_t)(ov_clip_bd(q1 + d2) | TAG);
     }
 }
 
@@ -157,14 +160,26 @@
     }
 }
 
-template <int DIR>
-__device__ __forceinline__ void luma_quad(uint16_t *pix, int step, Lim lim, int lp, int lq)
-{
+template <int UNMAP, bool LUMA, int NS>
+__device__ __forceinline__ void decode_line(int *s, const uint16_t *lut)
+{
+    if (UNMAP == 0) return;
+#pragma unroll
+    for (int i = 8 - NS; i < 8 + NS; ++i) {
+        const int raw = s[i], v = raw & OV_PIX_MAX;
+        s[i] = (UNMAP == 2 && LUMA && !(raw & LINEAR_TAG)) ? (int)lut[v] : v;
+    }
+}
+
+template <int DIR, int UNMAP>
+__device__ __forceinline__ void luma_quad(uint16_t *pix, int step, Lim lim, int lp, int lq, const uint16_t *lut)
+{
+    constexpr int TAG = UNMAP == 2 ? (int)LINEAR_TAG : 0;
     const int beta = lim.beta, tc = lim.tc;
     const bool big = lp > 3 || lq > 3;
     int s[16];
-    if (big) load_line_q<DIR, 8>(pix, step, s);
-    else     load_line_q<DIR, 4>(pix, step, s);
+    if (big) { load_line_q<DIR, 8>(pix, step, s); decode_line<UNMAP, true, 8>(s, lut); }
+    else     { load_line_q<DIR, 4>(pix, step, s); decode_line<UNMAP, true, 4>(s, lut); }
     const int dp = dp_of(s, 0), dq = dq_of(s, 0);
     const int dp0 = quad_bcast<0>(dp), dq0 = quad_bcast<0>(dq), dp3 = quad_bcast<3>(dp), dq3 = quad_bcast<3>(dq);
     const int d0 = dp0 + dq0, d3 = dp3 + dq3;
@@ -176,27 +191,28 @@
         const int dL = dpL + dqL;
         const int ok = (dL < ((beta + 0x10) >> 5)) && strong_large(s, beta, tc, lp, lq);
         const int d0L = quad_bcast<0>(dL), d3L = quad_bcast<3>(dL);
-        if ((d0L + d3L < beta) && quad_bcast<0>(ok) && quad_bcast<3>(ok)) { long_regs(s, pix, step, tc, lp, lq); return; }
+        if ((d0L + d3L < beta) && quad_bcast<0>(ok) && quad_bcast<3>(ok)) { long_regs<TAG>(s, pix, step, tc, lp, lq); return; }
     }
     const int oks = strong_small(s, beta, tc);
     const bool sw = lp > 2 && (d0 < ((beta + 4) >> 3)) && (d3 < ((beta + 4) >> 3)) && quad_bcast<0>(oks) && quad_bcast<3>(oks);
     if (sw) {
-        strong_regs(s, pix, step, tc);
+        strong_regs<TAG>(s, pix, step, tc);
     } else {
         const int side = (beta + (beta >> 1)) >> 3;
         const bool ext_p = (dp0 + dp3) < side && lp > 1;
         const bool ext_q = (dq0 + dq3) < side && lp > 1;
-        weak_regs(s, pix, step, tc, ext_p, ext_q);
-    }
-}
-
-template <int DIR>
+        weak_regs<TAG>(s, pix, step, tc, ext_p, ext_q);
+    }
+}
+
+template <int DIR, int UNMAP>
 __device__ __forceinline__ void chroma_quad(uint16_t *pix, int step, Lim lim, bool large, bool ctb_b, bool store)
 {
     const int tc = lim.tc, beta = lim.beta;
     if (tc == 0 || beta == 0) return;
     int s[16];
     load_line_q<DIR, 4>(pix, step, s);
+    decode_line<UNMAP, false, 4>(s, nullptr);
     bool strong = false;
     if (large) {
         const int p3 = ctb_b ? P(1) : P(3);
@@ -346,15 +362,26 @@
     }
 }
 
-template <int DIR>
+template <int DIR, int UNMAP>
 __global__ __launch_bounds__(256) OV_OCC_DBF void k_dbf_list(ovhip_pic pic, const ovhip_dbf_edge *__restrict__ edges, uint32_t n,
-                                                  uint64_t tc_pack, uint64_t beta_pack)
+                                                  uint64_t tc_pack, uint64_t beta_pack, const uint16_t *__restrict__ lut)
 {
     const uint32_t tid = ov_xcd_slot(blockIdx.x, gridDim.x) * 256 + threadIdx.x;
     const uint32_t ei = tid >> 2;
     const int l = tid & 3;
+    uint16_t *s_lut = nullptr;
+    ovhip_dbf_edge e0 = {};
+    constexpr bool STAGED = UNMAP == 2 && OV_UNMAP_STAGE;
+    if (UNMAP == 2 && !STAGED) s_lut = const_cast<uint16_t *>(lut);
+    if (STAGED) {
+        __shared__ uint16_t lds_lut[1024];
+        s_lut = lds_lut;
+        if (ei < n) e0 = edges[ei];
+        for (int i = threadIdx.x; i < 512; i += 256) reinterpret_cast<uint32_t *>(s_lut)[i] = reinterpret_cast<const uint32_t *>(lut)[i];
+        __syncthreads();
+    }
     if (ei >= n) return;
-    const ovhip_dbf_edge e = edges[ei];
+    const ovhip_dbf_edge e = STAGED ? e0 : edges[ei];
     const int v = e.word;
     const int osh = (e.pad & 7) * 8;
     const int tc_offset = (int8_t)(tc_pack >> osh), beta_offset = (int8_t)(beta_pack >> osh);
@@ -362,12 +389,29 @@
         const Lim lim = dbf_limits(v >> 8, v & 3, tc_offset, beta_offset);
         if (!(lim.tc || lim.beta)) return;
         uint16_t *p = pic.y + (e.uy * 4) * pic.stride_y + e.ux * 4 + l * (DIR ? 1 : pic.stride_y);
-        luma_quad<DIR>(p, DIR ? pic.stride_y : 1, lim, (v >> 2) & 7, (v >> 5) & 7);
+        luma_quad<DIR, UNMAP>(p, DIR ? pic.stride_y : 1, lim, (v >> 2) & 7, (v >> 5) & 7, s_lut);
     } else {
         const Lim lim = dbf_limits(v >> 8, 1 + !!(v & OVHIP_DBF_C_BS2), tc_offset, beta_offset);
         uint16_t *p = (e.comp == 1 ? pic.cb : pic.cr) + (e.uy * 2) * pic.stride_c + e.ux * 2 + (l & 1) * (DIR ? 1 : pic.stride_c);
-        chroma_quad<DIR>(p, DIR ? pic.stride_c : 1, lim, v & OVHIP_DBF_C_LARGE, v & OVHIP_DBF_C_CTB_B, l < 2);
-    }
+        chroma_quad<DIR, UNMAP>(p, DIR ? pic.stride_c : 1, lim, v & OVHIP_DBF_C_LARGE, v & OVHIP_DBF_C_CTB_B, l < 2);
+    }
+}
+
+template <int UNMAP>
+int dbf_list_launch(ovhip_ctx *ctx, const ovhip_pic *pic, const ovhip_dbf_edge *d_edges_v, uint32_t n_v, const ovhip_dbf_edge *d_edges_h, uint32_t n_h,
+                    const ovhip_dbf_offsets *offsets, const uint16_t *d_bwd_lut)
+{
+    uint64_t tc_pack, beta_pack;
+    memcpy(&tc_pack, offsets->tc, 8); memcpy(&beta_pack, offsets->beta, 8);
+    if (n_v) {
+        hipLaunchKernelGGL((k_dbf_list<0, UNMAP>), dim3((n_v + 63) / 64), dim3(256), 0, ctx->stream, *pic, d_edges_v, n_v, tc_pack, beta_pack, d_bwd_lut);
+        OV_LAUNCH_CHECK(ctx, "k_dbf_list<v>");
+    }
+    if (n_h) {
+        hipLaunchKernelGGL((k_dbf_list<1, UNMAP>), dim3((n_h + 63) / 64), dim3(256), 0, ctx->stream, *pic, d_edges_h, n_h, tc_pack, beta_pack, d_bwd_lut);
+        OV_LAUNCH_CHECK(ctx, "k_dbf_list<h>");
+    }
+    return OVHIP_OK;
 }
 
 }
@@ -379,17 +423,19 @@
     OV_DEVICE(ctx);
     if ((n_v && !d_edges_v) || (n_h && !d_edges_h))
         return ov_fail(ctx, OVHIP_EINVAL, "ovhip_dbf_launch_edges: null edge list", hipSuccess);
-    uint64_t tc_pack, beta_pack;
-    memcpy(&tc_pack, offsets->tc, 8); memcpy(&beta_pack, offsets->beta, 8);
-    if (n_v) {
-        hipLaunchKernelGGL(k_dbf_list<0>, dim3((n_v + 63) / 64), dim3(256), 0, ctx->stream, *pic, d_edges_v, n_v, tc_pack, beta_pack);
-        OV_LAUNCH_CHECK(ctx, "k_dbf_list<v>");
-    }
-    if (n_h) {
-        hipLaunchKernelGGL(k_dbf_list<1>, dim3((n_h + 63) / 64), dim3(256), 0, ctx->stream, *pic, d_edges_h, n_h, tc_pack, beta_pack);
-        OV_LAUNCH_CHECK(ctx, "k_dbf_list<h>");
-    }
-    return OVHIP_OK;
+    return dbf_list_launch<0>(ctx, pic, d_edges_v, n_v, d_edges_h, n_h, offsets, nullptr);
+}
+
+extern "C" int ovhip_dbf_launch_edges_unmap_(ovhip_ctx *ctx, const ovhip_pic *pic, const ovhip_dbf_edge *d_edges_v, uint32_t n_v,
+                                             const ovhip_dbf_edge *d_edges_h, uint32_t n_h, const ovhip_dbf_offsets *offsets, const uint16_t *d_bwd_lut)
+{
+    if (!ctx || !pic || !offsets) return OVHIP_EINVAL;
+    OV_DEVICE(ctx);
+    if ((n_v && !d_edges_v) || (n_h && !d_edges_h))
+        return ov_fail(ctx, OVHIP_EINVAL, "ovhip_dbf_launch_edges: null edge list", hipSuccess);
+    if (d_bwd_lut && ((uintptr_t)d_bwd_lut & 3)) return ov_fail(ctx, OVHIP_EINVAL, "ovhip_dbf_launch_edges_unmap_: table alignment", hipSuccess);
+    return d_bwd_lut ? dbf_list_launch<2>(ctx, pic, d_edges_v, n_v, d_edges_h, n_h, offsets, d_bwd_lut)
+                     : dbf_list_launch<1>(ctx, pic, d_edges_v, n_v, d_edges_h, n_h, offsets, nullptr);
 }
 
 extern "C" int ovhip_dbf_launch_edges(ovhip_ctx *ctx, const ovhip_pic *pic, const ovhip_dbf_edge *d_edges_v, uint32_t n_v,
diff --git a/openvvc_amd/csrc/kernels_sao.hip b/openvvc_amd/csrc/kernels_sao.hip
--- a/openvvc_amd/csrc/kernels_sao.hip
+++ b/openvvc_amd/csrc/kernels_sao.hip
@@ -20,9 +20,22 @@
     }
 }
 
+template <int UNMAP>
+__device__ __forceinline__ int sao_decode(int raw, bool luma, const uint16_t *lut)
+{
+    if (UNMAP == 0) return raw;
+    const int v = raw & OV_PIX_MAX;
+    return (UNMAP == 2 && luma && !(raw & LINEAR_TAG)) ? (int)lut[v] : v;
+}
+
+template <int UNMAP>
 __global__ __launch_bounds__(256) void k_sao(ovhip_pic dst, ovhip_pic src, const ovhip_sao_ctu *__restrict__ prm,
-                                              int log2_ctu, int nb_ctu_w, int tiles_y, int tiles_c, int ty0_y, int ty0_c, int row0, int row1)
+                                              int log2_ctu, int nb_ctu_w, int tiles_y, int tiles_c, int ty0_y, int ty0_c, int row0, int row1,
+                                              const uint16_t *__restrict__ lut)
 {
+    uint16_t *s_lut = nullptr;
+    if (UNMAP == 2 && OV_UNMAP_STAGE) { __shared__ uint16_t lds_lut[1024]; s_lut = lds_lut; }
+    if (UNMAP == 2 && !OV_UNMAP_STAGE) s_lut = const_cast<uint16_t *>(lut);
     const int tx = threadIdx.x & 7, ty = threadIdx.x >> 3;
     for (int t = blockIdx.x; t < tiles_y + 2 * tiles_c; t = tiles_y + 2 * tiles_c) {
         const int c = t < tiles_y ? 0 : (t < tiles_y + tiles_c ? 1 : 2);
@@ -31,16 +44,27 @@
         const int w = src.w >> sh, h = src.h >> sh, l2 = log2_ctu - sh;
         const int ntx = (w + SAO_TW - 1) / SAO_TW;
         const int x0 = (tt % ntx) * SAO_TW + tx * 8, y = (tt / ntx + (c ? ty0_c : ty0_y)) * SAO_TH + ty;
-        if (x0 >= w || y >= h || y < (row0 >> sh) || y >= (row1 >> sh)) continue;
+        const bool staged = UNMAP == 2 && OV_UNMAP_STAGE && c == 0;
+        const bool live = !(x0 >= w || y >= h || y < (row0 >> sh) || y >= (row1 >> sh));
+        if (!staged && !live) continue;
         int ss, ds;
         const uint16_t *s = ov_plane(src, c, ss) + y * ss;
         uint16_t *d = ov_plane(dst, c, ds) + y * ds;
+        int v[8], o[8];
+        if (staged) {
+            const int n_ = min(8, w - x0);
+            if (live) load8(s + x0, n_ == 8 && !((ss | ds) & 7) && !(((uintptr_t)s | (uintptr_t)d) & 15), n_, v);
+            for (int i = threadIdx.x; i < 512; i += 256) reinterpret_cast<uint32_t *>(s_lut)[i] = reinterpret_cast<const uint32_t *>(lut)[i];
+            __syncthreads();
+            if (!live) continue;
+        }
         const ovhip_sao_ctu *p = &prm[(y >> l2) * nb_ctu_w + (x0 >> l2)];
         const int type = p->type[c];
         const int n = min(8, w - x0);
         const bool vec = n == 8 && !((ss | ds) & 7) && !(((uintptr_t)s | (uintptr_t)d) & 15);
-        int v[8], o[8];
-        load8(s + x0, vec, n, v);
+        if (!staged) load8(s + x0, vec, n, v);
+#pragma unroll
+        for (int i = 0; i < 8; ++i) v[i] = sao_decode<UNMAP>(v[i], c == 0, s_lut);
 #pragma unroll
         for (int i = 0; i < 8; ++i) o[i] = v[i];
         if (type == OVHIP_SAO_BAND) {
@@ -72,6 +96,8 @@
                 ra[0] = x0 > 0 ? sa[x0 - 1] : 0; rb[0] = x0 > 0 ? sb[x0 - 1] : 0;
                 ra[9] = x0 + 8 < w ? sa[x0 + 8] : 0; rb[9] = x0 + 8 < w ? sb[x0 + 8] : 0;
 #pragma unroll
+                for (int i = 0; i < 10; ++i) { ra[i] = sao_decode<UNMAP>(ra[i], c == 0, s_lut); rb[i] = sao_decode<UNMAP>(rb[i], c == 0, s_lut); }
+#pragma unroll
                 for (int i = 0; i < 8; ++i) {
                     const int x = x0 + i;
                     if (i < n && !(eo != 1 && (x == 0 || x == w - 1 || x == skip_l || x == skip_r))) {
@@ -96,8 +122,9 @@
 
 }
 
-extern "C" int ovhip_sao_launch_rows(ovhip_ctx *ctx, const ovhip_pic *dst, const ovhip_pic *src,
-                                     const ovhip_sao_ctu *d_params, int32_t log2_ctu_s, int32_t row0, int32_t row1)
+template <int UNMAP>
+static int sao_launch_rows(ovhip_ctx *ctx, const ovhip_pic *dst, const ovhip_pic *src,
+                           const ovhip_sao_ctu *d_params, int32_t log2_ctu_s, int32_t row0, int32_t row1, const uint16_t *d_bwd_lut)
 {
     if (!ctx || !dst || !src || !d_params) return OVHIP_EINVAL;
     OV_DEVICE(ctx);
@@ -112,10 +139,24 @@
     const int tiles_y = ((src->w + SAO_TW - 1) / SAO_TW) * (ty1_y - ty0_y);
     const int tiles_c = ((src->w / 2 + SAO_TW - 1) / SAO_TW) * (ty1_c - ty0_c);
     const int total = tiles_y + 2 * tiles_c;
-    hipLaunchKernelGGL(k_sao, dim3(total), dim3(256), 0, ctx->stream, *dst, *src, d_params,
-                       log2_ctu_s, nb_ctu_w, tiles_y, tiles_c, ty0_y, ty0_c, row0, row1);
+    hipLaunchKernelGGL(k_sao<UNMAP>, dim3(total), dim3(256), 0, ctx->stream, *dst, *src, d_params,
+                       log2_ctu_s, nb_ctu_w, tiles_y, tiles_c, ty0_y, ty0_c, row0, row1, d_bwd_lut);
     OV_LAUNCH_CHECK(ctx, "k_sao");
     return OVHIP_OK;
+}
+
+extern "C" int ovhip_sao_launch_rows(ovhip_ctx *ctx, const ovhip_pic *dst, const ovhip_pic *src,
+                                     const ovhip_sao_ctu *d_params, int32_t log2_ctu_s, int32_t row0, int32_t row1)
+{
+    return sao_launch_rows<0>(ctx, dst, src, d_params, log2_ctu_s, row0, row1, nullptr);
+}
+
+extern "C" int ovhip_sao_launch_rows_unmap_(ovhip_ctx *ctx, const ovhip_pic *dst, const ovhip_pic *src, const ovhip_sao_ctu *d_params,
+                                            int32_t log2_ctu_s, int32_t row0, int32_t row1, const uint16_t *d_bwd_lut)
+{
+    if (d_bwd_lut && ((uintptr_t)d_bwd_lut & 3)) return OVHIP_EINVAL;
+    return d_bwd_lut ? sao_launch_rows<2>(ctx, dst, src, d_params, log2_ctu_s, row0, row1, d_bwd_lut)
+                     : sao_launch_rows<1>(ctx, dst, src, d_params, log2_ctu_s, row0, row1, nullptr);
 }
 
 extern "C" int ovhip_sao_launch(ovhip_ctx *ctx, const ovhip_pic *dst, const ovhip_pic *src,
diff --git a/openvvc_amd/csrc/ovvc_common.hip.h b/openvvc_amd/csrc/ovvc_common.hip.h
--- a/openvvc_amd/csrc/ovvc_common.hip.h
+++ b/openvvc_amd/csrc/ovvc_common.hip.h
@@ -8,6 +8,13 @@
 
 #define OV_BD 10
 #define OV_PIX_MAX ((1 << OV_BD) - 1)
+
+#define LINEAR_TAG 0x4000u
+#ifdef OV_UNMAP_LUT_L1
+#define OV_UNMAP_STAGE 0
+#else
+#define OV_UNMAP_STAGE 1
+#endif
 
 #define OV_MAX_LANES 4
 struct ovhip_ctx {
diff --git a/openvvc_amd/csrc/ovvc_picture.hip b/openvvc_amd/csrc/ovvc_picture.hip
--- a/openvvc_amd/csrc/ovvc_picture.hip
+++ b/openvvc_amd/csrc/ovvc_picture.hip
@@ -44,6 +44,7 @@
     uint32_t n_retries;
     int flow_launched;
     int test_abort, test_abort_seen;
+    int test_separate_unmap;
     ovhip_tmvp_cell *tmvp_host; size_t tmvp_cap, n_tmvp;
     size_t n_mv;
     size_t dmvr_first;
@@ -177,6 +178,10 @@
 
 extern "C" int ovhip_sao_launch_rows(ovhip_ctx *ctx, const ovhip_pic *dst, const ovhip_pic *src, const ovhip_sao_ctu *d_params, int32_t log2_ctu_s, int32_t row0, int32_t row1);
 extern "C" int ovhip_alf_launch_rows(ovhip_ctx *ctx, const ovhip_pic *dst, const ovhip_pic *src, const ovhip_alf_pic *alf, int32_t row0, int32_t row1);
+extern "C" int ovhip_dbf_launch_edges_unmap_(ovhip_ctx *ctx, const ovhip_pic *pic, const ovhip_dbf_edge *d_edges_v, uint32_t n_v,
+                                             const ovhip_dbf_edge *d_edges_h, uint32_t n_h, const ovhip_dbf_offsets *offsets, const uint16_t *d_bwd_lut);
+extern "C" int ovhip_sao_launch_rows_unmap_(ovhip_ctx *ctx, const ovhip_pic *dst, const ovhip_pic *src, const ovhip_sao_ctu *d_params,
+                                            int32_t log2_ctu_s, int32_t row0, int32_t row1, const uint16_t *d_bwd_lut);
 
 #define CHK(x) do { int r__ = (x); if (r__ != OVHIP_OK) return r__; } while (0)
 
@@ -313,6 +318,7 @@
     const uint32_t *lv_start; uint32_t n_lv;
     const uint32_t *d_items; uint32_t n_items;
     int prepared;
+    int unmap_on_load; const uint16_t *d_unmap;
 };
 
 int chain_predict(const Chain &c, const ovhip_pic *refs_same, const ovhip_pic *refs, uint32_t n_refs, const ovhip_pic *intra, int32_t *d_mv)
@@ -407,7 +413,8 @@
 int chain_deblock(const Chain &c, const ovhip_dbf_edge *d_ev, uint32_t n_ev, const ovhip_dbf_edge *d_eh, uint32_t n_eh, const ovhip_dbf_offsets *offs)
 {
     StageTimer t_(c.timer, OVHIP_TIME_DBF);
-    CHK(ovhip_dbf_launch_edges_ex(c.j->ctx, c.dst, d_ev, n_ev, d_eh, n_eh, offs));
+    if (c.unmap_on_load) CHK(ovhip_dbf_launch_edges_unmap_(c.j->ctx, c.dst, d_ev, n_ev, d_eh, n_eh, offs, c.d_unmap));
+    else CHK(ovhip_dbf_launch_edges_ex(c.j->ctx, c.dst, d_ev, n_ev, d_eh, n_eh, offs));
     c.j->st.n_launches += (n_ev != 0) + (n_eh != 0);
     return OVHIP_OK;
 }
@@ -418,7 +425,8 @@
     if (s1 > s0) {
         if (d_sao) {
             StageTimer t_(c.timer, OVHIP_TIME_SAO);
-            CHK(ovhip_sao_launch_rows(j->ctx, &j->tmp, c.dst, d_sao, c.log2_ctu, s0, s1));
+            if (c.unmap_on_load) CHK(ovhip_sao_launch_rows_unmap_(j->ctx, &j->tmp, c.dst, d_sao, c.log2_ctu, s0, s1, c.d_unmap));
+            else CHK(ovhip_sao_launch_rows(j->ctx, &j->tmp, c.dst, d_sao, c.log2_ctu, s0, s1));
             j->st.n_launches++;
         } else if (alf) CHK(copy_rows(j->ctx, &j->tmp, c.dst, s0, s1));
     }
@@ -712,6 +720,13 @@
 {
     if (!j) return OVHIP_EINVAL;
     j->test_abort = 1;
+    return OVHIP_OK;
+}
+
+int ovhip_job_test_separate_unmap(ovhip_job *j, int on)
+{
+    if (!j) return OVHIP_EINVAL;
+    j->test_separate_unmap = on != 0;
     return OVHIP_OK;
 }
 
@@ -931,7 +946,10 @@
             CHK(chain_ordered(c, n_workers));
             if (flow) { j->flow_launched = 1; j->st.flow_shift = (uint32_t)flow_shift_of(ctx->device); }
         }
-        CHK(chain_unmap(j, dst, 0, j->h, (pr->lmcs && (stages & OVHIP_STAGE_ITX)) ? d_bwd : nullptr, c.d_it, c.n_items ? c.n_it : 0u));
+        const uint16_t *d_unmap = (pr->lmcs && (stages & OVHIP_STAGE_ITX)) ? d_bwd : nullptr;
+        const uint32_t n_tagged = c.n_items ? c.n_it : 0u;
+        if (sao_on && !j->test_separate_unmap && (d_unmap || n_tagged)) { c.unmap_on_load = 1; c.d_unmap = d_unmap; }
+        else CHK(chain_unmap(j, dst, 0, j->h, d_unmap, c.d_it, n_tagged));
     }
     if (stages & OVHIP_STAGE_DBF)
         CHK(chain_deblock(c, (const ovhip_dbf_edge *)DEV(B_EV), (uint32_t)n_ev, (const ovhip_dbf_edge *)DEV(B_EH), (uint32_t)n_eh, &offs));
diff --git a/openvvc_amd/engine.py b/openvvc_amd/engine.py
--- a/openvvc_amd/engine.py
+++ b/openvvc_amd/engine.py
@@ -543,6 +543,9 @@
     def test_abort_next_flow(self):
         self.ctx._chk(self.lib.ovhip_job_test_abort_next_flow(self.j), "job_test_abort_next_flow")
 
+    def test_separate_unmap(self, on: bool = True):
+        self.ctx._chk(self.lib.ovhip_job_test_separate_unmap(self.j, int(on)), "job_test_separate_unmap")
+
     def stats(self) -> "capi.JobStats":
         s = capi.JobStats()
         self.lib.ovhip_job_last_stats(self.j, C.byref(s))
```

After: 3584. Within noise of the previous version (-0.5%).
